# Gregor-Mendel-Institute/SNPmatch

Hardware: NVIDIA B200
Metric: snp_accession_comparisons_per_sec (higher is better)
Workload: dtype f64

## Files before the change

snpmatch_b200/csrc/api.cu:

```cuda
#include "common.cuh"
#include <memory>
#include <new>
#include "pack.cuh"
#include "join.cuh"
#include "score.cuh"
#include "windows.cuh"
#include "f1.cuh"
#include "hardcall.cuh"
#include "gemm_onehot.cuh"
#include "grouped.cuh"
#include "group_sort.cuh"
#include "grouped2.cuh"
#include "pairs.cuh"
#include "cross_geno.cuh"
#include <unordered_map>

namespace snpm {
thread_local std::string g_last_error;

static int grid_for(int64_t items, int threads, int n_sm, int per_sm = 16) {
    int64_t g = ceil_div64(items, threads);
    const int64_t cap = int64_t(n_sm) * per_sm;
    if (g > cap) g = cap;
    if (g < 1) g = 1;
// ... 559 lines not shown
        for (int64_t i = 0; i < n; ++i) gid[size_t(i)] = rank[size_t(gid[size_t(i)])];
    }
    std::vector<int64_t> cnt(static_cast<size_t>(T) + 1);
    for (int64_t s = 0; s < n_samples; ++s) {
        const int64_t b0 = offsets[s], b1 = offsets[s + 1];
        std::fill(cnt.begin(), cnt.end(), 0);
        for (int64_t i = b0; i < b1; ++i) ++cnt[size_t(gid[size_t(i)]) + 1];
        for (int32_t t = 0; t < T; ++t) cnt[size_t(t) + 1] += cnt[size_t(t)];
        for (int64_t i = b0; i < b1; ++i) {
            const int32_t g = gid[size_t(i)];
            const int64_t o = b0 + cnt[size_t(g)]++;
            out_chrom[o] = s_chrom_id[i] < 0 ? uint8_t(255) : uint8_t(s_chrom_id[i]);
            out_pos[o] = s_pos[i];
            out_gid[o] = uint16_t(g);
            if (out_order) out_order[o] = i;
        }
    }
    return SNPM_OK;
}

static int upload_grouped(snpm_batch *b, int64_t n_samples, const int64_t *offsets, const uint8_t *chrom_u8, const int32_t *s_pos,
                          const uint32_t *packed_cp, const uint16_t *gid, const double *table, int32_t n_table,
                          const uint16_t *run_gid = nullptr, const uint32_t *run_end = nullptr, int64_t n_runs = 0) {
    if (!b) return fail(SNPM_E_ARG, "snpm_batch_upload_grouped: NULL batch");
    snpm_db *db = b->db;
    if (n_samples < 1 || !offsets || offsets[0] != 0) return fail(SNPM_E_ARG, "snpm_batch_upload_grouped: need samples and offsets starting at 0");
    for (int64_t s = 0; s < n_samples; ++s)
        if (offsets[s + 1] < offsets[s]) return fail(SNPM_E_ARG, "snpm_batch_upload_grouped: offsets must be non-decreasing");
    const int64_t n = offsets[n_samples];
    if (n >= (int64_t(1) << 31) - 2048) return fail(SNPM_E_ARG, "snpm_batch_upload_grouped: %lld markers exceed the 2^31 limit", (long long)n);
    if (n > 0 && ((!gid && !run_gid) || (!packed_cp && (!chrom_u8 || !s_pos)))) return fail(SNPM_E_ARG, "snpm_batch_upload_grouped: NULL marker arrays");
    if (run_gid && n > 0) {
        if (!run_end || n_runs < 1 || n_runs > n) return fail(SNPM_E_ARG, "snpm_batch_upload_grouped_runs: need 1..n runs");
        if (int64_t(run_end[n_runs - 1]) != n || run_end[0] == 0) return fail(SNPM_E_ARG, "snpm_batch_upload_grouped_runs: the runs must cover markers 0..n");
    }
    if (!table || n_table < 1 || n_table > 65536) return fail(SNPM_E_ARG, "snpm_batch_upload_grouped: weight table must hold 1..65536 triples");
    std::vector<double> t4(size_t(n_table) * 4);
    for (int32_t t = 0; t < n_table; ++t) {
        const double w0 = table[3 * size_t(t)], w1 = table[3 * size_t(t) + 1], w2 = table[3 * size_t(t) + 2];
        if (!(w0 >= 0.0 && w1 >= 0.0 && w2 >= 0.0) || std::isinf(w0) || std::isinf(w1) || std::isinf(w2))
            return fail(SNPM_E_ARG, "snpm_batch_upload_grouped: weights must be finite and non-negative (triple %d)", t);
        t4[4 * size_t(t)] = w0;
        t4[4 * size_t(t) + 1] = w2;
        t4[4 * size_t(t) + 2] = w1;
        t4[4 * size_t(t) + 3] = 0.0;
    }
    SNPM_CUDA(cudaSetDevice(db->device));
    b->S = n_samples;
    b->n = n;
    b->grouped = true;
    b->coded = false;
    b->pending_expand = 0;
    b->n_gtable = n_table;
    b->gchunk = b->gchunk_req;
    b->h_off.assign(offsets, offsets + n_samples + 1);
    int64_t nseg = 0;
    for (int64_t s = 0; s < n_samples; ++s) nseg += ceil_div64(offsets[s + 1] - offsets[s], b->gchunk);
    b->nseg_cap = nseg;
    SNPM_TRY(b->d_off.ensure(size_t(n_samples + 1) * 8));
    SNPM_TRY(b->d_chrom8.ensure(size_t(n)));
    SNPM_TRY(b->d_chrom.ensure(size_t(n) * 4));
    SNPM_TRY(b->d_pos.ensure(size_t(n) * 4));
    SNPM_TRY(b->d_gid.ensure(size_t(n) * 2));
    SNPM_TRY(b->d_gtable.ensure(size_t(n_table) * 32));
    cudaStream_t st = b->copy_stream;
    SNPM_CUDA(cudaStreamWaitEvent(st, b->ev_inputs_free, 0));
    SNPM_CUDA(cudaMemcpyAsync(b->d_off.p, offsets, size_t(n_samples + 1) * 8, cudaMemcpyHostToDevice, st));
    b->h_gtable.assign(t4.begin(), t4.end());
    SNPM_CUDA(cudaMemcpyAsync(b->d_gtable.p, b->h_gtable.data(), size_t(n_table) * 32, cudaMemcpyHostToDevice, st));
    if (n) {
        if (run_gid) {
            const size_t bad_off = (size_t(n_runs) * 6 + 15) & ~size_t(15);
            SNPM_TRY(b->d_runs.ensure(bad_off + 16));
            uint32_t *d_end = b->d_runs.as<uint32_t>();
            uint16_t *d_rg = reinterpret_cast<uint16_t *>(d_end + n_runs);
            b->d_runs_bad = reinterpret_cast<int *>(static_cast<char *>(b->d_runs.p) + bad_off);
            SNPM_CUDA(cudaMemsetAsync(b->d_runs_bad, 0, sizeof(int), st));
            SNPM_CUDA(cudaMemcpyAsync(d_end, run_end, size_t(n_runs) * 4, cudaMemcpyHostToDevice, st));
            SNPM_CUDA(cudaMemcpyAsync(d_rg, run_gid, size_t(n_runs) * 2, cudaMemcpyHostToDevice, st));
            b->pending_expand |= 1;
            b->pending_runs = n_runs;
        } else {
            b->d_runs_bad = nullptr;
            SNPM_CUDA(cudaMemcpyAsync(b->d_gid.p, gid, size_t(n) * 2, cudaMemcpyHostToDevice, st));
        }
        if (packed_cp) {
            SNPM_TRY(b->d_wei_idx.ensure(size_t(n) * 4));
            SNPM_CUDA(cudaMemcpyAsync(b->d_wei_idx.p, packed_cp, size_t(n) * 4, cudaMemcpyHostToDevice, st));
            b->pending_expand |= 2;
        } else {
            SNPM_CUDA(cudaMemcpyAsync(b->d_chrom8.p, chrom_u8, size_t(n), cudaMemcpyHostToDevice, st));
            SNPM_CUDA(cudaMemcpyAsync(b->d_pos.p, s_pos, size_t(n) * 4, cudaMemcpyHostToDevice, st));
            b->pending_expand |= 4;
        }
    }
    SNPM_CUDA(cudaEventRecord(b->ev_uploaded, st));
    b->ran = b->ran_windows = b->epilogue_done = false;
    return SNPM_OK;
}

int snpm_batch_upload_grouped(snpm_batch *b, int64_t n_samples, const int64_t *offsets, const uint8_t *chrom_u8, const int32_t *s_pos,
                              const uint16_t *gid, const double *table, int32_t n_table) {
    return upload_grouped(b, n_samples, offsets, chrom_u8, s_pos, nullptr, gid, table, n_table);
}

int snpm_batch_upload_grouped_packed(snpm_batch *b, int64_t n_samples, const int64_t *offsets, const uint32_t *chrom_pos, const uint16_t *gid,
                                     const double *table, int32_t n_table) {
    return upload_grouped(b, n_samples, offsets, nullptr, nullptr, chrom_pos, gid, table, n_table);
}

int snpm_batch_upload_grouped_runs(snpm_batch *b, int64_t n_samples, const int64_t *offsets, const uint32_t *chrom_pos, const uint16_t *run_gid,
                                   const uint32_t *run_end, int64_t n_runs, const double *table, int32_t n_table) {
    return upload_grouped(b, n_samples, offsets, nullptr, nullptr, chrom_pos, nullptr, table, n_table, run_gid, run_end, n_runs);
}

static int upload_coded(snpm_batch *b, int64_t n_samples, const int64_t *offsets, const uint32_t *chrom_pos, const uint16_t *codes,
                        const uint32_t *codes32, const double *wtable, int32_t n_wtable) {
    if (!b) return fail(SNPM_E_ARG, "snpm_batch_upload_coded: NULL batch");
    if (codes32 && n_wtable > 1024) return fail(SNPM_E_ARG, "snpm_batch_upload_coded32: three codes share one word only up to 1024 weight values (%d given)", n_wtable);
    snpm_db *db = b->db;
    if (n_samples < 1 || !offsets || offsets[0] != 0) return fail(SNPM_E_ARG, "snpm_batch_upload_coded: need samples and offsets starting at 0");
    for (int64_t s = 0; s < n_samples; ++s)
        if (offsets[s + 1] < offsets[s]) return fail(SNPM_E_ARG, "snpm_batch_upload_coded: offsets must be non-decreasing");
    const int64_t n = offsets[n_samples];
    if (n >= (int64_t(1) << 31) - 2048) return fail(SNPM_E_ARG, "snpm_batch_upload_coded: %lld markers exceed the 2^31 limit", (long long)n);
    if (n > 0 && (!chrom_pos || (!codes && !codes32))) return fail(SNPM_E_ARG, "snpm_batch_upload_coded: NULL marker arrays");
    if (!wtable || n_wtable < 1 || n_wtable > 65536) return fail(SNPM_E_ARG, "snpm_batch_upload_coded: the weight table must hold 1..65536 values");
    for (int32_t t = 0; t < n_wtable; ++t)
        if (!(wtable[t] >= 0.0) || std::isinf(wtable[t])) return fail(SNPM_E_ARG, "snpm_batch_upload_coded: weights must be finite and non-negative (entry %d)", t);
    if (!b->gchunk_set) b->gchunk_req = db->stride > G2_WX ? G2_MAX_CHUNK : 320;
    if (b->gchunk_req % GR_BLOCK || b->gchunk_req > G2_MAX_CHUNK)
        return fail(SNPM_E_ARG, "snpm_batch_upload_coded: the group chunk must be a multiple of %d and at most %d rows (it is %d)", GR_BLOCK, G2_MAX_CHUNK, b->gchunk_req);
    SNPM_CUDA(cudaSetDevice(db->device));
    b->S = n_samples;
    b->n = n;
    b->grouped = true;
    b->coded = true;
    b->codes_packed = codes32 != nullptr;
    b->pending_expand = 2;
    b->d_runs_bad = nullptr;
    b->n_wtable = n_wtable;
    int bits = 1;
    while ((1 << bits) < n_wtable) ++bits;
    b->code_bits = bits;
    b->key_bits = 3 * bits + 2;
    b->gchunk = b->gchunk_req;
    b->h_off.assign(offsets, offsets + n_samples + 1);
    int64_t nseg = 0;
    std::vector<int32_t> tile_first(size_t(n_samples) + 1), tile_sample;
    for (int64_t s = 0; s < n_samples; ++s) {
        const int64_t ns = offsets[s + 1] - offsets[s];
        nseg += ceil_div64(ns, b->gchunk);
        tile_first[size_t(s)] = int32_t(tile_sample.size());
        for (int64_t t = 0; t < ceil_div64(ns, RS_TILE); ++t) tile_sample.push_back(int32_t(s));
    }
    tile_first[size_t(n_samples)] = int32_t(tile_sample.size());
    b->nseg_cap = nseg;
    b->n_sort_tiles = int64_t(tile_sample.size());
    const size_t key_bytes = b->key_bits <= 32 ? 4 : 8;
    SNPM_TRY(b->d_off.ensure(size_t(n_samples + 1) * 8));
    SNPM_TRY(b->d_chrom.ensure(size_t(n) * 4));
    SNPM_TRY(b->d_pos.ensure(size_t(n) * 4));
    SNPM_TRY(b->d_wei_idx.ensure(size_t(n) * 4));
    SNPM_TRY(b->d_codes.ensure(size_t(n) * 6));
    SNPM_TRY(b->d_wtable.ensure(size_t(n_wtable) * 8));
    SNPM_TRY(b->d_key_a.ensure(size_t(n) * key_bytes));
    SNPM_TRY(b->d_pair_db_tmp.ensure(size_t(n) * 4));
    SNPM_TRY(b->d_pair_s_tmp.ensure(size_t(n) * 4));
    SNPM_TRY(b->d_tile_sample.ensure(std::max<size_t>(tile_sample.size(), 1) * 4));
    SNPM_TRY(b->d_tile_first.ensure(size_t(n_samples + 1) * 4));
    SNPM_TRY(b->d_tile_hist.ensure(std::max<size_t>(tile_sample.size(), 1) * (size_t(GH_MAX_GROUPS) * 4 + 8)));
    SNPM_TRY(b->d_blk_chg.ensure(size_t(std::max<int64_t>(nseg, 1)) * (size_t(b->gchunk / GR_BLOCK) * 8 + 12) + size_t(SO_BUCKETS) * 4 + 16));
    SNPM_TRY(b->d_seg_order.ensure(size_t(std::max<int64_t>(nseg, 1)) * 16));
    SNPM_TRY(b->d_work_counter.ensure(256));
    SNPM_TRY(b->d_hash.ensure(size_t(n_samples) * GH_SLOTS * 8));
    SNPM_TRY(b->d_slot_gid.ensure(size_t(n_samples) * GH_SLOTS * 2));
    SNPM_TRY(b->d_ngroups.ensure(size_t(n_samples) * 4));
    SNPM_TRY(b->d_group_overflow.ensure(size_t(n_samples) * 4));
    SNPM_TRY(b->d_gkeys.ensure(size_t(n_samples) * GH_MAX_GROUPS * key_bytes));
    SNPM_TRY(b->d_gw.ensure(size_t(n_samples) * GH_MAX_GROUPS * 32));
    SNPM_TRY(b->d_goff.ensure(size_t(n_samples) * (GH_MAX_GROUPS + 1) * 4));
    SNPM_TRY(b->d_gid.ensure(size_t(n) * 2));
    cudaStream_t st = b->copy_stream;
    SNPM_CUDA(cudaStreamWaitEvent(st, b->ev_inputs_free, 0));
    b->h_gtable.assign(wtable, wtable + n_wtable);
    b->h_tiles.assign(tile_first.begin(), tile_first.end());
    b->h_tiles.insert(b->h_tiles.end(), tile_sample.begin(), tile_sample.end());
    SNPM_CUDA(cudaMemcpyAsync(b->d_off.p, offsets, size_t(n_samples + 1) * 8, cudaMemcpyHostToDevice, st));
    SNPM_CUDA(cudaMemcpyAsync(b->d_wtable.p, b->h_gtable.data(), size_t(n_wtable) * 8, cudaMemcpyHostToDevice, st));
    SNPM_CUDA(cudaMemcpyAsync(b->d_tile_first.p, b->h_tiles.data(), size_t(n_samples + 1) * 4, cudaMemcpyHostToDevice, st));
    if (!tile_sample.empty())
        SNPM_CUDA(cudaMemcpyAsync(b->d_tile_sample.p, b->h_tiles.data() + n_samples + 1, tile_sample.size() * 4, cudaMemcpyHostToDevice, st));
    if (n) {
        SNPM_CUDA(cudaMemcpyAsync(b->d_wei_idx.p, chrom_pos, size_t(n) * 4, cudaMemcpyHostToDevice, st));
        if (codes32) SNPM_CUDA(cudaMemcpyAsync(b->d_codes.p, codes32, size_t(n) * 4, cudaMemcpyHostToDevice, st));
        else SNPM_CUDA(cudaMemcpyAsync(b->d_codes.p, codes, size_t(n) * 6, cudaMemcpyHostToDevice, st));
    }
    SNPM_CUDA(cudaEventRecord(b->ev_uploaded, st));
    b->ran = b->ran_windows = b->epilogue_done = false;
    return SNPM_OK;
}

int snpm_batch_upload_coded(snpm_batch *b, int64_t n_samples, const int64_t *offsets, const uint32_t *chrom_pos, const uint16_t *codes,
                            const double *wtable, int32_t n_wtable) {
    return upload_coded(b, n_samples, offsets, chrom_pos, codes, nullptr, wtable, n_wtable);
}

int snpm_batch_upload_coded32(snpm_batch *b, int64_t n_samples, const int64_t *offsets, const uint32_t *chrom_pos, const uint32_t *codes32,
                              const double *wtable, int32_t n_wtable) {
    return upload_coded(b, n_samples, offsets, chrom_pos, nullptr, codes32, wtable, n_wtable);
}

int snpm_batch_coded_timings(snpm_batch *b, float *ms, int n) {
    if (!b || !ms || n < 4) return fail(SNPM_E_ARG, "snpm_batch_coded_timings: need room for 4 floats");
    if (!b->coded || !b->ran) return fail(SNPM_E_STATE, "snpm_batch_coded_timings: run a coded batch first");
    SNPM_CUDA(cudaSetDevice(b->db->device));
    SNPM_CUDA(cudaStreamSynchronize(b->db->stream));
    for (int i = 0; i < n; ++i) ms[i] = 0.f;
    cudaEventElapsedTime(&ms[0], b->ev[SNPM_EV_START], b->ev_joined);
    cudaEventElapsedTime(&ms[1], b->ev_joined, b->ev[SNPM_EV_JOIN]);
    cudaEventElapsedTime(&ms[2], b->ev[SNPM_EV_JOIN], b->ev[SNPM_EV_SCORE]);
    cudaEventElapsedTime(&ms[3], b->ev[SNPM_EV_SCORE], b->ev[SNPM_EV_COMBINE]);
    return SNPM_OK;
}

int snpm_pack_markers(int64_t n, const uint8_t *chrom_u8, const int32_t *pos, uint32_t *out) {
    if (n < 0 || (n > 0 && (!chrom_u8 || !pos || !out))) return fail(SNPM_E_ARG, "snpm_pack_markers: bad arguments");
    for (int64_t i = 0; i < n; ++i) {
        const uint32_t c = chrom_u8[i] == 255 ? 31u : uint32_t(chrom_u8[i]);
        if ((chrom_u8[i] != 255 && c > 30u) || pos[i] < 0 || pos[i] >= (1 << 27))
            return fail(SNPM_E_RANGE, "snpm_pack_markers: marker %lld (chromosome id %u, position %d) does not fit 5 + 27 bits", (long long)i, c, pos[i]);
        out[i] = (c << 27) | uint32_t(pos[i]);
    }
    return SNPM_OK;
}

int snpm_pack_coded(int64_t n, const int32_t *chrom_id, const int32_t *pos, const uint16_t *codes, uint32_t *chrom_pos, uint32_t *codes32) {
    if (n < 0 || (n > 0 && (!chrom_id || !pos || !chrom_pos || (codes32 && !codes)))) return fail(SNPM_E_ARG, "snpm_pack_coded: bad arguments");
    uint32_t bad = 0u;
    for (int64_t i = 0; i < n; ++i) {
        const int32_t c = chrom_id[i], p = pos[i];
        bad |= uint32_t(c > 30) | uint32_t(p < 0) | uint32_t(p >= (1 << 27));
        chrom_pos[i] = ((c < 0 ? 31u : uint32_t(c)) << 27) | (uint32_t(p) & ((1u << 27) - 1u));
    }
    if (codes32)
        for (int64_t i = 0; i < n; ++i) {
            const uint32_t a = codes[3 * i], h = codes[3 * i + 1], t = codes[3 * i + 2];
            bad |= uint32_t((a | h | t) > 1023u);
            codes32[i] = a | (h << 10) | (t << 20);
        }
    if (bad) return fail(SNPM_E_RANGE, "snpm_pack_coded: a chromosome id above 30, a position outside 27 bits or a code above 1023");
    return SNPM_OK;
}

int snpm_batch_guard_counts(snpm_batch *b, int32_t *counts) {
    if (!b || !counts) return fail(SNPM_E_ARG, "snpm_batch_guard_counts: NULL argument");
    if (!b->grouped) { for (int64_t s = 0; s < b->rangen(); ++s) counts[s] = 0; return SNPM_OK; }
    if (!b->epilogue_done) return fail(SNPM_E_STATE, "snpm_batch_guard_counts: run the epilogue first");
    if (b->rangen() == 0) return SNPM_OK;
    SNPM_CUDA(cudaSetDevice(b->db->device));
    SNPM_CUDA(cudaMemcpyAsync(counts, b->d_guard.as<int32_t>() + b->range0(), size_t(b->rangen()) * 4, cudaMemcpyDeviceToHost, b->db->stream));
    SNPM_CUDA(cudaStreamSynchronize(b->db->stream));
    return SNPM_OK;
}

int snpm_batch_set_result_range(snpm_batch *b, int64_t first_sample, int64_t n_samples) {
    if (!b || first_sample < 0 || n_samples < -1) return fail(SNPM_E_ARG, "snpm_batch_set_result_range: bad range");
    b->res0 = first_sample;
    b->resn = n_samples;
    return SNPM_OK;
}

int snpm_batch_set_track_pairs(snpm_batch *b, int on) {
    if (!b) return fail(SNPM_E_ARG, "snpm_batch_set_track_pairs: NULL batch");
    b->track_pairs = on != 0;
    return SNPM_OK;
}

int snpm_batch_set_chunk_rows(snpm_batch *b, int32_t rows) {
    if (!b || rows < 1 || rows > 1000000) return fail(SNPM_E_ARG, "snpm_batch_set_chunk_rows: 1..1000000 rows");
    b->chunk_rows_req = rows;
    return SNPM_OK;
}

int snpm_batch_set_group_chunk(snpm_batch *b, int32_t rows) {
    if (!b || rows < 16 || rows > GR_MAX_CHUNK || rows % 8) return fail(SNPM_E_ARG, "snpm_batch_set_group_chunk: 16..%d rows, a multiple of 8", GR_MAX_CHUNK);
    b->gchunk_req = rows;
    b->gchunk_set = true;
    return SNPM_OK;
}

static void ipc_close_peers(snpm_batch *b);

int snpm_batch_destroy(snpm_batch *b) {
    if (!b) return SNPM_OK;
    cudaSetDevice(b->db->device);
    cudaStreamSynchronize(b->db->stream);
    if (b->copy_stream) { cudaStreamSynchronize(b->copy_stream); cudaStreamDestroy(b->copy_stream); }
    if (b->ev_uploaded) cudaEventDestroy(b->ev_uploaded);
    if (b->ev_inputs_free) cudaEventDestroy(b->ev_inputs_free);
    if (b->ev_joined) cudaEventDestroy(b->ev_joined);
    if (b->ev_fork) cudaEventDestroy(b->ev_fork);
    if (b->ev_join) cudaEventDestroy(b->ev_join);
    DevBuf *bufs[] = {&b->d_off, &b->d_chrom, &b->d_pos, &b->d_wei, &b->d_filter, &b->d_match_row, &b->d_tile_cnt, &b->d_tile_off,
                      &b->d_prefix, &b->d_pair_db, &b->d_pair_s, &b->d_pair_w, &b->d_mstart, &b->d_seg_off, &b->d_part_score,
                      &b->d_part_ninfo, &b->d_red, &b->d_matches, &b->d_ninfo64, &b->d_prob, &b->d_L, &b->d_LR, &b->d_status,
                      &b->d_win_count, &b->d_win_off, &b->d_win_begin, &b->d_win_end, &b->d_kmax, &b->d_win_L, &b->d_win_LR,
                      &b->d_win_ident, &b->d_win_amb, &b->d_win_row_off, &b->d_row_acc, &b->d_row_score, &b->d_row_ninfo, &b->d_row_L, &b->d_row_ident, &b->d_f1_acc, &b->d_f1_part, &b->d_f1_out, &b->d_pair_code, &b->d_wei_idx, &b->d_wei_table,
                      &b->d_chrom8, &b->d_gid, &b->d_gtable, &b->d_pair_gid, &b->d_part_int, &b->d_guard, &b->d_runs,
                      &b->d_codes, &b->d_wtable, &b->d_key_a, &b->d_key_b, &b->d_idx_a, &b->d_idx_b, &b->d_pair_db_tmp, &b->d_pair_s_tmp,
                      &b->d_tile_sample, &b->d_tile_first, &b->d_tile_hist, &b->d_blk_chg, &b->d_seg_order, &b->d_work_counter, &b->d_hash, &b->d_slot_gid, &b->d_ngroups,
                      &b->d_group_overflow, &b->d_gkeys, &b->d_gw, &b->d_goff, &b->d_segsel, &b->d_segsel_off, &b->d_flags, &b->d_flag_counts};
    for (DevBuf *d : bufs) d->release();
    for (int i = 0; i < SNPM_N_EVENTS; ++i)
        if (b->ev[i]) cudaEventDestroy(b->ev[i]);
    if (b->h_status) cudaFreeHost(b->h_status);
    if (b->h_tail) cudaFreeHost(b->h_tail);
    if (b->ev_fetched) cudaEventDestroy(b->ev_fetched);
    if (b->ev_results) cudaEventDestroy(b->ev_results);
    ipc_close_peers(b);
    delete b;
    return SNPM_OK;
}

int snpm_batch_set_row_filter(snpm_batch *b, const int64_t *sorted_rows, int64_t n) {
    if (!b || n < 0) return fail(SNPM_E_ARG, "snpm_batch_set_row_filter: bad arguments");
    for (int64_t i = 1; i < n; ++i)
        if (sorted_rows[i] <= sorted_rows[i - 1]) return fail(SNPM_E_ARG, "snpm_batch_set_row_filter: rows must be strictly ascending");
    SNPM_CUDA(cudaSetDevice(b->db->device));
    b->has_filter = sorted_rows != nullptr;
    b->n_filter = b->has_filter ? n : 0;
    SNPM_TRY(b->d_filter.ensure(size_t(std::max<int64_t>(n, 1)) * 8));
    if (b->has_filter && n) {
        SNPM_CUDA(cudaMemcpyAsync(b->d_filter.p, sorted_rows, size_t(n) * 8, cudaMemcpyHostToDevice, b->db->stream));
        SNPM_CUDA(cudaStreamSynchronize(b->db->stream));
    }
    return SNPM_OK;
}

int snpm_batch_set_segregation_filter(snpm_batch *b, const uint32_t *sel, int64_t S, int32_t words) {
    if (!b) return fail(SNPM_E_ARG, "snpm_batch_set_segregation_filter: NULL batch");
    if (!sel) {
        b->has_seg = false;
        b->seg_S = 0;
        return SNPM_OK;
    }
    snpm_db *db = b->db;
    if (S < 1 || words != db->stride)
        return fail(SNPM_E_ARG, "snpm_batch_set_segregation_filter: need S >= 1 selections of snpm_db_row_words() = %d words (got S = %lld, %d words)",
                    db->stride, (long long)S, words);
    std::vector<int32_t> off(size_t(S) + 1, 0);
    std::vector<uint32_t> pairs;
    for (int64_t s = 0; s < S; ++s) {
        for (int32_t w = 0; w < words; ++w) {
            const uint32_t m = sel[size_t(s) * words + w];
            const int64_t first = int64_t(w) * 32;
            const uint32_t valid = first >= db->n_acc ? 0u : (db->n_acc - first >= 32 ? 0xffffffffu : (1u << (db->n_acc - first)) - 1u);
            if (m & ~valid) return fail(SNPM_E_ARG, "snpm_batch_set_segregation_filter: sample %lld selects accessions beyond the panel's %d", (long long)s, db->n_acc);
            if (m) {
                pairs.push_back(uint32_t(w));
                pairs.push_back(m);
            }
        }
        if (pairs.size() / 2 > size_t(INT32_MAX)) return fail(SNPM_E_ARG, "snpm_batch_set_segregation_filter: selections too large");
        off[size_t(s) + 1] = int32_t(pairs.size() / 2);
    }
    SNPM_CUDA(cudaSetDevice(db->device));
    SNPM_TRY(b->d_segsel.ensure(std::max<size_t>(pairs.size(), 2) * 4));
    SNPM_TRY(b->d_segsel_off.ensure(off.size() * 4));
    if (!pairs.empty()) SNPM_CUDA(cudaMemcpyAsync(b->d_segsel.p, pairs.data(), pairs.size() * 4, cudaMemcpyHostToDevice, db->stream));
    SNPM_CUDA(cudaMemcpyAsync(b->d_segsel_off.p, off.data(), off.size() * 4, cudaMemcpyHostToDevice, db->stream));
    SNPM_CUDA(cudaStreamSynchronize(db->stream));
    b->has_seg = true;
    b->seg_S = S;
    return SNPM_OK;
}

int snpm_batch_count_flagged_pairs(snpm_batch *b, const uint8_t *flags, int64_t *counts) {
    if (!b || !counts || (b->n > 0 && !flags)) return fail(SNPM_E_ARG, "snpm_batch_count_flagged_pairs: bad arguments");
    if (!b->ran) return fail(SNPM_E_STATE, "snpm_batch_count_flagged_pairs: run the batch first");
    snpm_db *db = b->db;
    SNPM_CUDA(cudaSetDevice(db->device));
    cudaStream_t st = db->stream;
    SNPM_TRY(b->d_flag_counts.ensure(size_t(b->S) * 8));
    SNPM_CUDA(cudaMemsetAsync(b->d_flag_counts.p, 0, size_t(b->S) * 8, st));
    if (b->n > 0) {
        SNPM_TRY(b->d_flags.ensure(size_t(b->n)));
        SNPM_CUDA(cudaMemcpyAsync(b->d_flags.p, flags, size_t(b->n), cudaMemcpyHostToDevice, st));
        k_count_flagged_pairs<<<int(ceil_div64(b->n, 256)), 256, 0, st>>>(b->d_match_row.as<int32_t>(), b->d_flags.as<uint8_t>(), b->n,
                                                                          b->d_off.as<int64_t>(), b->S, b->d_flag_counts.as<unsigned long long>());
        SNPM_KERNEL_CHECK();
    }
    SNPM_CUDA(cudaMemcpyAsync(counts, b->d_flag_counts.p, size_t(b->S) * 8, cudaMemcpyDeviceToHost, st));
    SNPM_CUDA(cudaStreamSynchronize(st));
    return SNPM_OK;
}

static int batch_join(snpm_batch *b, int algo) {
    snpm_db *db = b->db;
    cudaStream_t st = db->stream;
    const int64_t n = b->n, S = b->S;
    const int64_t n_tiles = ceil_div64(n, JOIN_TILE);
    SNPM_TRY(b->d_match_row.ensure(size_t(n) * 4));
    SNPM_TRY(b->d_tile_cnt.ensure(size_t(n_tiles) * 4));
    SNPM_TRY(b->d_tile_off.ensure(size_t(n_tiles) * 4));
    SNPM_TRY(b->d_prefix.ensure(size_t(n + 1) * 4));
    SNPM_TRY(b->d_pair_db.ensure(size_t(n) * 4));
    SNPM_TRY(b->d_pair_s.ensure(size_t(n) * 4));
    if (b->coded) {  }
    else if (b->grouped) SNPM_TRY(b->d_pair_gid.ensure(size_t(n) * 2 + 16));
    else SNPM_TRY(b->d_pair_w.ensure(size_t(n) * 32));
    SNPM_TRY(b->d_mstart.ensure(size_t(S + 1) * 4));
    SNPM_TRY(b->d_seg_off.ensure(size_t(S + 1) * 4));
    SNPM_TRY(b->d_status.ensure(8 * sizeof(int)));
    SNPM_CUDA(cudaStreamWaitEvent(st, b->ev_uploaded, 0));
    SNPM_CUDA(cudaMemsetAsync(b->d_status.p, 0, 8 * sizeof(int), st));
    if (b->grouped && b->pending_expand && n > 0) {
        if (b->pending_expand & 1) {
            const uint32_t *d_end = b->d_runs.as<uint32_t>();
            k_expand_runs<<<int(ceil_div64(b->pending_runs * 32, 256)), 256, 0, st>>>(d_end, reinterpret_cast<const uint16_t *>(d_end + b->pending_runs),
                                                                                 int32_t(b->pending_runs), n, b->d_gid.as<uint16_t>(), b->d_runs_bad);
        }
        if (b->pending_expand & 4) k_expand_chrom<<<int(ceil_div64(n, 256)), 256, 0, st>>>(b->d_chrom8.as<uint8_t>(), n, b->d_chrom.as<int32_t>());
        SNPM_KERNEL_CHECK();
        b->pending_expand &= 2;
    }
    if (b->grouped && b->d_runs_bad) SNPM_CUDA(cudaMemcpyAsync(b->d_status.as<int>() + 4, b->d_runs_bad, sizeof(int), cudaMemcpyDeviceToDevice, st));
    if (!b->peer_red.empty() && b->ipc_step > 0 && b->d_red.p == b->ipc_ptr) {
        k_wait_peers_done<<<1, 32, 0, st>>>(reinterpret_cast<const uint32_t *>(static_cast<const char *>(b->d_red.p) + b->ipc_flags_off),
                                            int32_t(b->peer_red.size()), b->ipc_step, b->d_status.as<int>());
        SNPM_KERNEL_CHECK();
    }
    if (algo == 0) algo = (n / S) * 8 >= db->n_rows ? 2 : 1;
    if (b->grouped) algo = 1;
    const int64_t *filter = b->has_filter ? b->d_filter.as<int64_t>() : nullptr;
    if (n_tiles > 0) {
        if (algo == 2)
            k_join_mergepath<<<int(n_tiles), 256, 0, st>>>(b->d_chrom.as<int32_t>(), b->d_pos.as<int32_t>(), n, b->d_off.as<int64_t>(), S,
                                                         db->d_pos, db->d_chr_regions, db->n_chr, filter, b->n_filter, db->row0_global,
                                                         b->d_match_row.as<int32_t>(), b->d_tile_cnt.as<int32_t>(), b->d_status.as<int>());
        else
            k_join_search<<<int(n_tiles), JOIN_TILE, 0, st>>>(b->d_chrom.as<int32_t>(), b->d_pos.as<int32_t>(), n, b->d_off.as<int64_t>(), S,
                                                            db->d_pos, db->d_chr_regions, db->n_chr, db->d_bucket, db->d_bucket_off, db->bucket_shift,
                                                            filter, b->n_filter, db->row0_global,
                                                            b->d_match_row.as<int32_t>(), b->d_tile_cnt.as<int32_t>(), b->d_status.as<int>(), (b->grouped && !b->coded) ? 0 : 1,
                                                            db->d_bitmap, db->d_bm_first_row, db->d_bm_off,
                                                            (b->grouped && (b->pending_expand & 2)) ? b->d_wei_idx.as<uint32_t>() : nullptr);
        SNPM_KERNEL_CHECK();
        if (b->has_seg) {
            static_assert(SEGP_THREADS == JOIN_TILE, "the segregation filter recounts the join's tiles");
            k_segregating_pairs<<<int(n_tiles), SEGP_THREADS, 0, st>>>(db->d_packed, db->stride, b->d_off.as<int64_t>(), S, n, b->d_segsel.as<uint2>(),
                                                                      b->d_segsel_off.as<int32_t>(), b->d_match_row.as<int32_t>(), b->d_tile_cnt.as<int32_t>());
            SNPM_KERNEL_CHECK();
            b->launches += 1;
        }
        k_scan_tiles<<<1, 1024, 0, st>>>(b->d_tile_cnt.as<int32_t>(), n_tiles, b->d_tile_off.as<int32_t>(), b->d_prefix.as<int32_t>() + n);
        SNPM_KERNEL_CHECK();
        if (b->coded) {
            unsigned long long *hash = b->d_hash.as<unsigned long long>();
            SNPM_CUDA(cudaMemsetAsync(b->d_group_overflow.p, 0, size_t(S) * 4, st));
            SNPM_CUDA(cudaMemsetAsync(hash, 0, size_t(S) * GH_SLOTS * 8, st));
            if (b->key_bits <= 32)
                k_scatter_pairs_coded<uint32_t><<<int(n_tiles), SC_THREADS, 0, st>>>(b->d_match_row.as<int32_t>(), n, b->d_tile_off.as<int32_t>(), b->d_codes.as<uint16_t>(),
                        b->d_wtable.as<double>(), b->n_wtable, b->code_bits, b->d_prefix.as<int32_t>(), b->d_pair_db_tmp.as<int32_t>(), b->d_pair_s_tmp.as<int32_t>(),
                        b->d_key_a.as<uint32_t>(), b->d_status.as<int>(), b->d_off.as<int64_t>(), S, hash, b->d_group_overflow.as<int>(),
                        b->codes_packed ? b->d_codes.as<uint32_t>() : nullptr);
            else
                k_scatter_pairs_coded<uint64_t><<<int(n_tiles), SC_THREADS, 0, st>>>(b->d_match_row.as<int32_t>(), n, b->d_tile_off.as<int32_t>(), b->d_codes.as<uint16_t>(),
                        b->d_wtable.as<double>(), b->n_wtable, b->code_bits, b->d_prefix.as<int32_t>(), b->d_pair_db_tmp.as<int32_t>(), b->d_pair_s_tmp.as<int32_t>(),
                        b->d_key_a.as<uint64_t>(), b->d_status.as<int>(), b->d_off.as<int64_t>(), S, hash, b->d_group_overflow.as<int>(),
                        b->codes_packed ? b->d_codes.as<uint32_t>() : nullptr);
        } else if (b->grouped)
            k_scatter_pairs_grouped<<<int(n_tiles), JOIN_TILE, 0, st>>>(b->d_match_row.as<int32_t>(), n, b->d_tile_off.as<int32_t>(),
                                                                      b->d_gid.as<uint16_t>(), b->n_gtable, b->d_prefix.as<int32_t>(), b->d_pair_db.as<int32_t>(),
                                                                      b->d_pair_s.as<int32_t>(), b->d_pair_gid.as<uint16_t>(), b->d_status.as<int>());
        else
            k_scatter_pairs<<<int(n_tiles), JOIN_TILE, 0, st>>>(b->d_match_row.as<int32_t>(), n, b->d_tile_off.as<int32_t>(), b->d_wei.as<double>(),
                                                              b->d_prefix.as<int32_t>(), b->d_pair_db.as<int32_t>(), b->d_pair_s.as<int32_t>(),
                                                              b->d_pair_w.as<double>());
        SNPM_KERNEL_CHECK();
        b->launches += 3;
    } else {
        SNPM_CUDA(cudaMemsetAsync(b->d_prefix.p, 0, 4, st));
    }
    k_sample_ranges<<<1, 1024, 0, st>>>(b->d_prefix.as<int32_t>(), b->d_off.as<int64_t>(), S, b->grouped ? b->gchunk : b->chunk_rows, b->d_mstart.as<int32_t>(),
                                        b->d_seg_off.as<int32_t>());
    SNPM_KERNEL_CHECK();
    b->launches += 1;
    return SNPM_OK;
}

}

template <typename KeyT>
static int batch_group_sort_t(snpm_batch *b) {
    snpm_db *db = b->db;
    cudaStream_t st = db->stream;
    const int tiles = int(b->n_sort_tiles);
    if (tiles == 0 || b->n == 0) return SNPM_OK;
    const int32_t *mstart = b->d_mstart.as<int32_t>(), *tsample = b->d_tile_sample.as<int32_t>(), *tfirst = b->d_tile_first.as<int32_t>();
    uint32_t *hist = b->d_tile_hist.as<uint32_t>();
    int2 *range = reinterpret_cast<int2 *>(hist + (size_t(tiles) << 11));
    static bool gattr = false;
    if (!gattr) {
        SNPM_CUDA(cudaFuncSetAttribute(k_group_place, cudaFuncAttributeMaxDynamicSharedMemorySize, 64 * 1024));
        gattr = true;
    }
    KeyT *gkeys = b->d_gkeys.as<KeyT>();
    k_group_rank<KeyT><<<int(b->S), 1024, 0, st>>>(b->d_hash.as<unsigned long long>(), b->d_wtable.as<double>(), b->code_bits, b->d_slot_gid.as<uint16_t>(),
                                                   b->d_ngroups.as<int32_t>(), gkeys, b->d_gw.as<double4>(), b->d_group_overflow.as<int>());
    int64_t n_max = 0, jcap1 = 1;
    for (int64_t s = 0; s < b->S; ++s) {
        n_max = std::max(n_max, b->h_off[size_t(s) + 1] - b->h_off[size_t(s)]);
        jcap1 = std::max(jcap1, ceil_div64(b->h_off[size_t(s) + 1] - b->h_off[size_t(s)], b->gchunk));
    }
    const char *force = getenv("SNPM_GROUP_KERNEL");
    const bool fits = n_max <= GP_MAX_PAIRS;
    const bool want = force ? !strcmp(force, "sample") : (n_max <= 32768 || b->S >= 128);
    if (fits && want) {
        static bool sattr = false;
        if (!sattr) {
            SNPM_CUDA(cudaFuncSetAttribute(k_group_sample<uint32_t>, cudaFuncAttributeMaxDynamicSharedMemorySize, int(GP_SMEM)));
            SNPM_CUDA(cudaFuncSetAttribute(k_group_sample<uint64_t>, cudaFuncAttributeMaxDynamicSharedMemorySize, int(GP_SMEM)));
            sattr = true;
        }
        const size_t ncap = size_t(std::max<int64_t>(b->nseg_cap, 1));
        int32_t *cost = reinterpret_cast<int32_t *>(b->d_blk_chg.as<unsigned long long>() + ncap * size_t(b->gchunk / GR_BLOCK));
        int32_t *buckets = cost + ncap;
        const size_t zbytes = ncap * (size_t(b->gchunk / GR_BLOCK) * 8 + 4) + size_t(SO_BUCKETS) * 4;
        int2 *br = reinterpret_cast<int2 *>(reinterpret_cast<unsigned char *>(b->d_blk_chg.p) + ((zbytes + 7) & ~size_t(7)));
        SNPM_CUDA(cudaMemsetAsync(b->d_blk_chg.p, 0, zbytes, st));
        k_group_sample<KeyT><<<int(b->S), 32 * GP_WARPS, GP_SMEM, st>>>(
            b->d_key_a.as<KeyT>(), b->d_hash.as<unsigned long long>(), b->d_slot_gid.as<uint16_t>(), b->d_ngroups.as<int32_t>(), b->d_gid.as<uint16_t>(),
            b->d_pair_db_tmp.as<int32_t>(), b->d_pair_s_tmp.as<int32_t>(), b->d_pair_db.as<int32_t>(), b->track_pairs ? b->d_pair_s.as<int32_t>() : nullptr,
            b->d_goff.as<int32_t>(), gkeys, mstart, b->d_seg_off.as<int32_t>(), b->gchunk, b->code_bits, b->d_blk_chg.as<unsigned long long>(), cost,
            int32_t(jcap1), buckets, br, b->d_work_counter.as<unsigned int>());
        k_order_place<<<int(b->S), 256, 0, st>>>(buckets, br, b->d_seg_off.as<int32_t>(), mstart, b->gchunk, b->d_seg_order.as<int4>());
        SNPM_KERNEL_CHECK();
        b->launches += 3;
        return SNPM_OK;
    }
    k_tile_ranges<<<(tiles + 255) / 256, 256, 0, st>>>(mstart, tsample, tfirst, tiles, range);
    k_group_ids<KeyT><<<tiles, RS_THREADS, 0, st>>>(b->d_key_a.as<KeyT>(), range, tsample, b->d_hash.as<unsigned long long>(), b->d_slot_gid.as<uint16_t>(),
                                                    b->d_ngroups.as<int32_t>(), b->d_gid.as<uint16_t>(), hist);
    k_group_scan<<<int(b->S), 1024, 0, st>>>(hist, tfirst, b->d_ngroups.as<int32_t>(), b->d_goff.as<int32_t>());
    const size_t nseg_cap = size_t(std::max<int64_t>(b->nseg_cap, 1));
    int32_t *seg_cost = reinterpret_cast<int32_t *>(b->d_blk_chg.as<unsigned long long>() + nseg_cap * size_t(b->gchunk / GR_BLOCK));
    int32_t *bucket_cnt = seg_cost + nseg_cap;
    const size_t zero_bytes = nseg_cap * (size_t(b->gchunk / GR_BLOCK) * 8 + 4) + size_t(SO_BUCKETS) * 4;
    int2 *seg_br = reinterpret_cast<int2 *>(reinterpret_cast<unsigned char *>(b->d_blk_chg.p) + ((zero_bytes + 7) & ~size_t(7)));
    int64_t jcap = 1;
    for (int64_t s = 0; s < b->S; ++s) jcap = std::max(jcap, ceil_div64(b->h_off[size_t(s) + 1] - b->h_off[size_t(s)], b->gchunk));
    cudaStream_t aux = b->copy_stream;
    if (!b->ev_fork) SNPM_CUDA(cudaEventCreateWithFlags(&b->ev_fork, cudaEventDisableTiming));
    if (!b->ev_join) SNPM_CUDA(cudaEventCreateWithFlags(&b->ev_join, cudaEventDisableTiming));
    SNPM_CUDA(cudaEventRecord(b->ev_fork, st));
    SNPM_CUDA(cudaStreamWaitEvent(aux, b->ev_fork, 0));
    SNPM_CUDA(cudaMemsetAsync(b->d_blk_chg.p, 0, zero_bytes, aux));
    k_group_marks<KeyT><<<int(b->S), 1024, 0, aux>>>(b->d_goff.as<int32_t>(), gkeys, b->d_ngroups.as<int32_t>(), mstart, b->d_seg_off.as<int32_t>(), b->gchunk,
                                                     b->code_bits, b->d_blk_chg.as<unsigned long long>(), seg_cost, int32_t(jcap), bucket_cnt, seg_br);
    k_order_place<<<int(b->S), 256, 0, aux>>>(bucket_cnt, seg_br, b->d_seg_off.as<int32_t>(), mstart, b->gchunk, b->d_seg_order.as<int4>());
    SNPM_CUDA(cudaEventRecord(b->ev_join, aux));
    k_group_place<<<tiles, RS_THREADS, size_t(GH_MAX_GROUPS) * 20, st>>>(b->d_gid.as<uint16_t>(), b->d_pair_db_tmp.as<int32_t>(), b->d_pair_s_tmp.as<int32_t>(),
                                                                        b->d_pair_db.as<int32_t>(), b->track_pairs ? b->d_pair_s.as<int32_t>() : nullptr, mstart, tsample,
                                                                        tfirst, range, hist, b->d_ngroups.as<int32_t>(), b->d_goff.as<int32_t>(), b->d_work_counter.as<unsigned int>());
    SNPM_CUDA(cudaStreamWaitEvent(st, b->ev_join, 0));
    SNPM_KERNEL_CHECK();
    b->launches += 7;
    return SNPM_OK;
}

static int launch_grouped2(snpm_batch *b, bool skip_db_hets) {
    snpm_db *db = b->db;
    cudaStream_t st = db->stream;
    Group2Args g = {};
    g.packed = db->d_packed; g.stride = db->stride; g.pair_db = b->d_pair_db.as<int32_t>();
    g.blk_chg = b->d_blk_chg.as<unsigned long long>(); g.gw = b->d_gw.as<double>();
    g.seg_off = b->d_seg_off.as<int32_t>(); g.mstart = b->d_mstart.as<int32_t>(); g.S = int32_t(b->S); g.chunk = b->gchunk;
    g.part_score = b->d_part_score.as<double>(); g.part_int = b->d_part_int.as<int32_t>(); g.a_pad = db->stride * 32;
    if (db->stride <= G2_WX) { g.n_slices = 1; g.wx = (db->stride + 1) & ~1; }
    else { g.wx = 32; g.n_slices = (db->stride + 31) / 32; }
    g.teams = std::min(G2_THREADS / g.wx, G2_MAX_TEAMS);
    g.order = b->d_seg_order.as<int4>();
    g.work_counter = b->d_work_counter.as<unsigned int>();
    const int64_t n_items = std::max<int64_t>(b->nseg_cap, 1) * g.n_slices;
    if (n_items >= (int64_t(1) << 31) - (int64_t(1) << 20)) return fail(SNPM_E_ARG, "snpm_batch_run: %lld work items exceed the 2^31 limit", (long long)n_items);
    constexpr int ring = 64;
    const size_t smem = size_t(g.teams) * g2_team_smem(g.wx, g.chunk, ring);
    if (smem > 226 * 1024) return fail(SNPM_E_ARG, "snpm_batch_run: group chunk %d needs %zu bytes of shared memory", g.chunk, smem);
    const int grid = int(std::min<int64_t>(db->n_sm, ceil_div64(n_items, g.teams)));
#define G2_LAUNCH(SK, WXV)                                                                                                        \
    do {                                                                                                                          \
        static bool attr_ = false;                                                                                                \
        if (!attr_) {                                                                                                             \
            SNPM_CUDA(cudaFuncSetAttribute(k_score_grouped2<SK, WXV, ring>, cudaFuncAttributeMaxDynamicSharedMemorySize, 226 * 1024)); \
            attr_ = true;                                                                                                         \
        }                                                                                                                         \
        k_score_grouped2<SK, WXV, ring><<<grid, G2_THREADS, smem, st>>>(g);                                                       \
    } while (0)
    if (g.wx == G2_WX) {
        if (skip_db_hets) G2_LAUNCH(true, G2_WX); else G2_LAUNCH(false, G2_WX);
    } else if (g.wx == 32) {
        if (skip_db_hets) G2_LAUNCH(true, 32); else G2_LAUNCH(false, 32);
    } else {
        if (skip_db_hets) G2_LAUNCH(true, 0); else G2_LAUNCH(false, 0);
    }
#undef G2_LAUNCH
    SNPM_KERNEL_CHECK();
    b->launches += 1;
    return SNPM_OK;
}

extern "C" {

static int batch_alloc_outputs(snpm_batch *b, int64_t nseg) {
    snpm_db *db = b->db;
    const int64_t a_pad = int64_t(db->stride) * 32;
    const int64_t SA = b->S * int64_t(db->n_acc);
    SNPM_TRY(b->d_part_score.ensure(size_t(std::max<int64_t>(nseg, 1)) * a_pad * 8));
    SNPM_TRY(b->d_part_ninfo.ensure(size_t(std::max<int64_t>(nseg, 1)) * a_pad * 4));
    SNPM_TRY(b->d_red.ensure(size_t(b->S) * size_t(b->red_pitch()) * 8));
    if (b->grouped) SNPM_TRY(b->d_part_int.ensure(size_t(std::max<int64_t>(nseg, 1)) * a_pad * 4));
    SNPM_TRY(b->d_matches.ensure(size_t(SA) * 8));
    SNPM_TRY(b->d_ninfo64.ensure(size_t(SA) * 8));
    SNPM_TRY(b->d_prob.ensure(size_t(SA) * 8));
    SNPM_TRY(b->d_L.ensure(size_t(SA) * 8));
    SNPM_TRY(b->d_LR.ensure(size_t(SA) * 8));
    return SNPM_OK;
}

static void rec(snpm_batch *b, int which) {
    cudaEventRecord(b->ev[which], b->db->stream);
    b->ev_rec[which] = true;
}

int snpm_batch_run(snpm_batch *b, int skip_db_hets, int mode) {
    if (!b) return fail(SNPM_E_ARG, "snpm_batch_run: NULL batch");
    snpm_db *db = b->db;
    SNPM_CUDA(cudaSetDevice(db->device));
    cudaStream_t st = db->stream;
    const int kernel_mode = mode & 0xff, algo = (mode >> 8) & 0xff;
    if (kernel_mode < 0 || kernel_mode > 2) return fail(SNPM_E_ARG, "snpm_batch_run: unknown kernel mode %d", kernel_mode);
    if ((kernel_mode == 2) != b->grouped)
        return fail(SNPM_E_STATE, "snpm_batch_run: kernel mode 2 scores batches uploaded with snpm_batch_upload_grouped, and only those");
    if (algo > 2) return fail(SNPM_E_ARG, "snpm_batch_run: unknown join algorithm %d", algo);
    if (b->has_seg && kernel_mode == 2)
        return fail(SNPM_E_STATE, "snpm_batch_run: the segregation filter is honoured by kernel modes 0 and 1 only; clear it first");
    if (b->has_seg && b->seg_S != b->S)
        return fail(SNPM_E_ARG, "snpm_batch_run: the segregation filter holds %lld selections for %lld samples", (long long)b->seg_S, (long long)b->S);
    b->launches = 0;
    for (int i = 0; i < SNPM_N_EVENTS; ++i) b->ev_rec[i] = false;
    SNPM_TRY(batch_alloc_outputs(b, b->nseg_cap));
    rec(b, SNPM_EV_START);
    SNPM_TRY(batch_join(b, algo));
    rec(b, SNPM_EV_JOIN);
    ScoreArgs a = {};
    a.packed = db->d_packed;
    a.stride = db->stride;
    a.pair_db = b->d_pair_db.as<int32_t>();
    a.pair_w = b->d_pair_w.as<double>();
    a.seg_off = b->d_seg_off.as<int32_t>();
    a.mstart = b->d_mstart.as<int32_t>();
    a.S = int32_t(b->S);
    a.chunk = b->chunk_rows;
    a.table = 0;
    a.part_score = b->d_part_score.as<double>();
    a.part_ninfo = b->d_part_ninfo.as<int32_t>();
    a.a_pad = db->stride * 32;
    if (kernel_mode == 2 && b->coded) {
        cudaEventRecord(b->ev_joined, st);
        if (b->key_bits <= 32) SNPM_TRY(batch_group_sort_t<uint32_t>(b)); else SNPM_TRY(batch_group_sort_t<uint64_t>(b));
        rec(b, SNPM_EV_JOIN);
        if (b->nseg_cap > 0 && b->n > 0) {
            SNPM_TRY(launch_grouped2(b, skip_db_hets != 0));
        }
        rec(b, SNPM_EV_SCORE);
        dim3 cgrid((a.a_pad + 31) / 32, unsigned(b->S));
        k_combine_grouped<<<cgrid, 32 * CG_PARTS, 0, st>>>(a.part_score, b->d_part_int.as<int32_t>(), a.a_pad, db->stride, db->n_acc, a.seg_off, a.mstart,
                                                 b->d_red.as<double>());
        SNPM_KERNEL_CHECK();
        b->launches += 1;
        rec(b, SNPM_EV_COMBINE);
        SNPM_CUDA(cudaEventRecord(b->ev_inputs_free, st));
        b->ran = true;
        b->ran_windows = false;
        b->epilogue_done = false;
        return SNPM_OK;
    }
    if (kernel_mode == 2) {
        if (b->nseg_cap > 0) {
            GroupArgs g = {};
            g.packed = db->d_packed; g.stride = db->stride; g.pair_db = a.pair_db; g.pair_gid = b->d_pair_gid.as<uint16_t>();
            g.table = b->d_gtable.as<double>(); g.seg_off = a.seg_off; g.mstart = a.mstart; g.S = a.S; g.chunk = b->gchunk;
            g.part_score = a.part_score; g.part_int = b->d_part_int.as<int32_t>(); g.a_pad = a.a_pad;
            const int nsl = (db->stride + GR_MAX_WX - 1) / GR_MAX_WX;
            g.wx = ((db->stride + nsl - 1) / nsl + 1) & ~1;
            g.spc = std::min(GR_THREADS / g.wx, GR_MAX_TEAMS);
            const size_t gsmem = size_t(g.spc) * grouped_team_smem(g.wx, g.chunk);
            static bool gr_attr = false;
            if (!gr_attr) {
                SNPM_CUDA(cudaFuncSetAttribute(k_score_grouped<true, 0>, cudaFuncAttributeMaxDynamicSharedMemorySize, 220 * 1024));
                SNPM_CUDA(cudaFuncSetAttribute(k_score_grouped<false, 0>, cudaFuncAttributeMaxDynamicSharedMemorySize, 220 * 1024));
                SNPM_CUDA(cudaFuncSetAttribute(k_score_grouped<true, GR_MAX_WX>, cudaFuncAttributeMaxDynamicSharedMemorySize, 220 * 1024));
                SNPM_CUDA(cudaFuncSetAttribute(k_score_grouped<false, GR_MAX_WX>, cudaFuncAttributeMaxDynamicSharedMemorySize, 220 * 1024));
                gr_attr = true;
            }
            int64_t jmax = 0;
            for (int64_t smp = 0; smp < b->S; ++smp)
                jmax = std::max(jmax, ceil_div64(b->h_off[size_t(smp) + 1] - b->h_off[size_t(smp)], b->gchunk));
            g.jmax = int32_t(jmax);
            dim3 ggrid(unsigned(ceil_div64(b->S * jmax, g.spc)), unsigned((db->stride + g.wx - 1) / g.wx));
            if (g.wx == GR_MAX_WX) {
                if (skip_db_hets) k_score_grouped<true, GR_MAX_WX><<<ggrid, GR_THREADS, gsmem, st>>>(g);
                else k_score_grouped<false, GR_MAX_WX><<<ggrid, GR_THREADS, gsmem, st>>>(g);
            } else {
                if (skip_db_hets) k_score_grouped<true, 0><<<ggrid, GR_THREADS, gsmem, st>>>(g);
                else k_score_grouped<false, 0><<<ggrid, GR_THREADS, gsmem, st>>>(g);
            }
            SNPM_KERNEL_CHECK();
            b->launches += 1;
        }
        rec(b, SNPM_EV_SCORE);
        dim3 cgrid((a.a_pad + 31) / 32, unsigned(b->S));
        k_combine_grouped<<<cgrid, 32 * CG_PARTS, 0, st>>>(a.part_score, b->d_part_int.as<int32_t>(), a.a_pad, db->stride, db->n_acc, a.seg_off, a.mstart,
                                                 b->d_red.as<double>());
        SNPM_KERNEL_CHECK();
        b->launches += 1;
        rec(b, SNPM_EV_COMBINE);
        SNPM_CUDA(cudaEventRecord(b->ev_inputs_free, st));
        b->ran = true;
        b->ran_windows = false;
        b->epilogue_done = false;
        return SNPM_OK;
    }
    if (kernel_mode == 1 && b->chunk_rows != SNPM_CHUNK_ROWS)
        return fail(SNPM_E_STATE, "snpm_batch_run: the popcount kernel works in %d-row chunks (its sums are exact in any chunking); set the chunk back", SNPM_CHUNK_ROWS);
    if (kernel_mode == 1 && b->nseg_cap > 0) {
        SNPM_TRY(b->d_pair_code.ensure(size_t(std::max<int64_t>(b->n, 1))));
        k_pair_codes<<<int(ceil_div64(b->n, 256)), 256, 0, st>>>(a.pair_w, b->d_prefix.as<int32_t>() + b->n, b->d_pair_code.as<uint8_t>());
        SNPM_KERNEL_CHECK();
        HardArgs h = {};
        h.packed = a.packed; h.stride = a.stride; h.pair_db = a.pair_db; h.pair_code = b->d_pair_code.as<uint8_t>();
        h.seg_off = a.seg_off; h.mstart = a.mstart; h.S = a.S; h.chunk = a.chunk;
        h.part_score = a.part_score; h.part_ninfo = a.part_ninfo; h.a_pad = a.a_pad; h.status = b->d_status.as<int>();
        const int wx = std::min<int>(db->stride, HC_THREADS), spc = std::min(HC_THREADS / wx, HC_MAX_SEGS);
        h.wx = wx;
        h.spc = spc;
        dim3 hgrid(unsigned(ceil_div64(b->nseg_cap, spc)), unsigned((db->stride + wx - 1) / wx));
        const size_t hsmem = size_t(spc) * SNPM_CHUNK_ROWS * 5;
        static bool hc_attr = false;
        if (!hc_attr) {
            SNPM_CUDA(cudaFuncSetAttribute(k_score_hard<true>, cudaFuncAttributeMaxDynamicSharedMemorySize, 64 * 1024));
            SNPM_CUDA(cudaFuncSetAttribute(k_score_hard<false>, cudaFuncAttributeMaxDynamicSharedMemorySize, 64 * 1024));
            hc_attr = true;
        }
        if (skip_db_hets) k_score_hard<true><<<hgrid, HC_THREADS, hsmem, st>>>(h);
        else k_score_hard<false><<<hgrid, HC_THREADS, hsmem, st>>>(h);
        SNPM_KERNEL_CHECK();
        b->launches += 2;
    } else {
        SNPM_TRY(launch_score(st, a, int(b->nseg_cap), skip_db_hets != 0));
        if (b->nseg_cap > 0) b->launches += 1;
    }
    rec(b, SNPM_EV_SCORE);
    dim3 cgrid((db->n_acc + 31) / 32, unsigned(b->S));
    k_combine<<<cgrid, 32, 0, st>>>(a.part_score, a.part_ninfo, a.a_pad, db->n_acc, a.seg_off, a.mstart, 0, nullptr, nullptr, b->d_red.as<double>());
    SNPM_KERNEL_CHECK();
    b->launches += 1;
    rec(b, SNPM_EV_COMBINE);
    SNPM_CUDA(cudaEventRecord(b->ev_inputs_free, st));
    b->ran = true;
    b->ran_windows = false;
    b->epilogue_done = false;
    return SNPM_OK;
}

int snpm_batch_epilogue(snpm_batch *b) {
    if (!b) return fail(SNPM_E_ARG, "snpm_batch_epilogue: NULL batch");
    if (!b->ran) return fail(SNPM_E_STATE, "snpm_batch_epilogue: run the batch first");
    snpm_db *db = b->db;
    SNPM_CUDA(cudaSetDevice(db->device));
    const int64_t r0 = b->range0(), rn = b->rangen();
    if (r0 < 0 || rn < 0 || r0 + rn > b->S) return fail(SNPM_E_ARG, "snpm_batch_epilogue: result range [%lld, %lld) outside the %lld samples", (long long)r0, (long long)(r0 + rn), (long long)b->S);
    rec(b, SNPM_EV_EPI_START);
    const int64_t pitch = b->red_pitch(), A = db->n_acc;
    if (rn > 0) {
        if (b->grouped) {
            SNPM_TRY(b->d_guard.ensure(size_t(b->S) * 4));
            SNPM_CUDA(cudaMemsetAsync(b->d_guard.as<int32_t>() + r0, 0, size_t(rn) * 4, db->stream));
            dim3 fgrid((db->n_acc + 255) / 256, unsigned(rn));
            k_grouped_finalize<<<fgrid, 256, 0, db->stream>>>(b->d_red.as<double>() + r0 * pitch, db->n_acc, b->d_guard.as<int32_t>() + r0,
                                                              b->coded ? b->d_group_overflow.as<int>() + r0 : nullptr);
            SNPM_KERNEL_CHECK();
            b->launches += 1;
        }
        SNPM_CUDA(launch_epilogue(db->stream, rn, b->d_red.as<double>() + r0 * pitch, pitch, db->n_acc, 1, 0, 0.0,
                                  b->d_matches.as<int64_t>() + r0 * A, b->d_ninfo64.as<int64_t>() + r0 * A,
                                  b->d_prob.as<double>() + r0 * A, b->d_L.as<double>() + r0 * A, b->d_LR.as<double>() + r0 * A));
    }
    SNPM_KERNEL_CHECK();
    b->launches += 1;
    rec(b, SNPM_EV_EPI_END);
    b->epilogue_done = true;
    return SNPM_OK;
}

int snpm_batch_wait(snpm_batch *b, float *ms_device) {
    if (!b) return fail(SNPM_E_ARG, "snpm_batch_wait: NULL batch");
    snpm_db *db = b->db;
    SNPM_CUDA(cudaSetDevice(db->device));
    if (b->d_status.p) SNPM_CUDA(cudaMemcpyAsync(b->h_status, b->d_status.p, 8 * sizeof(int), cudaMemcpyDeviceToHost, db->stream));
    else memset(b->h_status, 0, 8 * sizeof(int));
    SNPM_CUDA(cudaStreamSynchronize(db->stream));
    if (ms_device) {
        *ms_device = 0.f;
        if (b->ev_rec[SNPM_EV_START] && b->ev_rec[SNPM_EV_COMBINE]) {
            float t = 0.f;
            cudaEventElapsedTime(&t, b->ev[SNPM_EV_START], b->ev[SNPM_EV_COMBINE]);
            *ms_device += t;
        }
        if (b->ev_rec[SNPM_EV_EPI_START] && b->ev_rec[SNPM_EV_EPI_END]) {
            float t = 0.f;
            cudaEventElapsedTime(&t, b->ev[SNPM_EV_EPI_START], b->ev[SNPM_EV_EPI_END]);
            *ms_device += t;
        }
    }
    if (b->h_status[0] > 0)
        return fail(SNPM_E_ARG, "sample markers are not sorted by (database chromosome order, position) or repeat a position (%d places)", b->h_status[0]);
    if (b->h_status[1] > 0)
        return fail(SNPM_E_ASSERT, "provided y is greater than n (%d window cells; likeliTest, snpmatch.py:43)", b->h_status[1]);
    if (b->h_status[2] > 0)
        return fail(SNPM_E_ARG, "identity table too short for %d window cells", b->h_status[2]);
    if (b->h_status[3] > 0)
        return fail(SNPM_E_ARG, "kernel mode 1 needs one-hot weights (called genotypes); %d matched markers are not", b->h_status[3]);
    if (b->h_status[4] > 0)
        return fail(SNPM_E_ARG, "%d matched markers carry a weight-triple id outside the table (or run-length coded ids do not ascend)", b->h_status[4]);
    if (b->h_status[5] > 0)
        return fail(SNPM_E_STATE, "peer reduce: a rank did not arrive within thirty seconds (every rank must run and reduce the same batches in the same order)");
    return SNPM_OK;
}

int snpm_batch_timings(snpm_batch *b, float *ms, int n) {
    if (!b || !ms || n < 6) return fail(SNPM_E_ARG, "snpm_batch_timings: need room for 6 floats");
    SNPM_CUDA(cudaSetDevice(b->db->device));
    SNPM_CUDA(cudaStreamSynchronize(b->db->stream));
    for (int i = 0; i < n; ++i) ms[i] = 0.f;
    auto el = [&](int a, int c) {
        float t = 0.f;
        if (b->ev_rec[a] && b->ev_rec[c]) cudaEventElapsedTime(&t, b->ev[a], b->ev[c]);
        return t;
    };
    ms[0] = el(SNPM_EV_START, SNPM_EV_JOIN);
    ms[1] = el(SNPM_EV_JOIN, SNPM_EV_SCORE);
    ms[2] = el(SNPM_EV_SCORE, SNPM_EV_COMBINE);
    ms[3] = el(SNPM_EV_EPI_START, SNPM_EV_EPI_END);
    ms[4] = el(SNPM_EV_START, SNPM_EV_COMBINE) + ms[3];
    ms[5] = float(b->launches);
    if (n >= 8) {
        ms[6] = el(SNPM_EV_RED_START, SNPM_EV_RED_END);
        int wait_ns = 0;
        if (b->ev_rec[SNPM_EV_RED_END] && b->d_status.p) cudaMemcpy(&wait_ns, b->d_status.as<int>() + 7, sizeof(int), cudaMemcpyDeviceToHost);
        ms[7] = float(wait_ns) * 1e-6f;
    }
    return SNPM_OK;
}

int snpm_batch_reduce_buffer(snpm_batch *b, void **dev_ptr, int64_t *n_doubles) {
    if (!b || !dev_ptr) return fail(SNPM_E_ARG, "snpm_batch_reduce_buffer: NULL argument");
    SNPM_CUDA(cudaSetDevice(b->db->device));
    SNPM_TRY(b->d_red.ensure(size_t(b->S) * size_t(b->red_pitch()) * 8));
    *dev_ptr = b->d_red.p;
    if (n_doubles) *n_doubles = b->S * b->red_pitch();
    return SNPM_OK;
}

static void ipc_close_peers(snpm_batch *b) {
    for (size_t r = 0; r < b->peer_red.size(); ++r)
        if (int32_t(r) != b->ipc_rank && b->peer_red[r]) cudaIpcCloseMemHandle(b->peer_red[r]);
    b->peer_red.clear();
    b->ipc_rank = -1;
}

int snpm_batch_ipc_export(snpm_batch *b, void *handle64, int64_t *n_doubles) {
    static_assert(sizeof(cudaIpcMemHandle_t) == 64, "CUDA IPC handles are 64 bytes");
    if (!b || !handle64) return fail(SNPM_E_ARG, "snpm_batch_ipc_export: NULL argument");
    SNPM_CUDA(cudaSetDevice(b->db->device));
    const size_t bytes = size_t(b->S) * size_t(b->red_pitch()) * 8;
    const size_t cap = std::max<size_t>(((bytes + 255) & ~size_t(255)) + PR_FLAG_BYTES, size_t(4) << 20);
    SNPM_CUDA(cudaStreamSynchronize(b->db->stream));
    if (b->d_red.cap != cap) {
        b->d_red.release();
        SNPM_TRY(b->d_red.ensure(cap));
    }
    b->ipc_flags_off = cap - PR_FLAG_BYTES;
    b->ipc_step = 0;
    SNPM_CUDA(cudaMemset(static_cast<char *>(b->d_red.p) + b->ipc_flags_off, 0, PR_FLAG_BYTES));
    SNPM_CUDA(cudaIpcGetMemHandle(reinterpret_cast<cudaIpcMemHandle_t *>(handle64), b->d_red.p));
    b->ipc_ptr = b->d_red.p;
    if (n_doubles) *n_doubles = b->S * b->red_pitch();
    return SNPM_OK;
}

int snpm_batch_ipc_open(snpm_batch *b, const void *handles, int32_t world, int32_t rank) {
    if (!b || !handles || world < 1 || world > PR_MAX_WORLD || rank < 0 || rank >= world) return fail(SNPM_E_ARG, "snpm_batch_ipc_open: bad arguments (at most %d ranks)", PR_MAX_WORLD);
    if (!b->ipc_ptr || b->ipc_ptr != b->d_red.p) return fail(SNPM_E_STATE, "snpm_batch_ipc_open: export this batch's buffer first (snpm_batch_ipc_export)");
    SNPM_CUDA(cudaSetDevice(b->db->device));
    ipc_close_peers(b);
    b->peer_red.assign(size_t(world), nullptr);
    b->ipc_rank = rank;
    const cudaIpcMemHandle_t *h = reinterpret_cast<const cudaIpcMemHandle_t *>(handles);
    for (int32_t r = 0; r < world; ++r) {
        if (r == rank) { b->peer_red[size_t(r)] = b->d_red.p; continue; }
        cudaError_t e = cudaIpcOpenMemHandle(&b->peer_red[size_t(r)], h[r], cudaIpcMemLazyEnablePeerAccess);
        if (e != cudaSuccess) {
            b->peer_red[size_t(r)] = nullptr;
            ipc_close_peers(b);
            return fail(SNPM_E_CUDA, "snpm_batch_ipc_open: rank %d's buffer: %s", r, cudaGetErrorString(e));
        }
    }
    return SNPM_OK;
}

int snpm_batch_ipc_close(snpm_batch *b) {
    if (!b) return SNPM_OK;
    cudaSetDevice(b->db->device);
    cudaStreamSynchronize(b->db->stream);
    ipc_close_peers(b);
    b->ipc_ptr = nullptr;
    return SNPM_OK;
}

int snpm_batch_reduce_peers(snpm_batch *b) {
    if (!b) return fail(SNPM_E_ARG, "snpm_batch_reduce_peers: NULL batch");
    if (!b->ran) return fail(SNPM_E_STATE, "snpm_batch_reduce_peers: run the batch first");
    const int32_t world = int32_t(b->peer_red.size());
    if (world < 1 || b->ipc_rank < 0) return fail(SNPM_E_STATE, "snpm_batch_reduce_peers: open the peers' buffers first (snpm_batch_ipc_open)");
    if (b->d_red.p != b->ipc_ptr) return fail(SNPM_E_STATE, "snpm_batch_reduce_peers: the reduce buffer moved since it was exported (batch grew): export and open again");
    const int64_t r0 = b->res0, rn = b->resn < 0 ? b->S - b->res0 : b->resn;
    if (r0 + rn > b->S) return fail(SNPM_E_ARG, "snpm_batch_reduce_peers: result range outside the batch");
    const int64_t pitch = b->red_pitch();
    int64_t first = r0 * pitch, count = rn * pitch;
    SNPM_CUDA(cudaSetDevice(b->db->device));
    PeerPtrs pp;
    for (int32_t r = 0; r < PR_MAX_WORLD; ++r) {
        pp.p[r] = r < world ? static_cast<const double *>(b->peer_red[size_t(r)]) : nullptr;
        pp.flags[r] = r < world ? reinterpret_cast<uint32_t *>(static_cast<char *>(b->peer_red[size_t(r)]) + b->ipc_flags_off) : nullptr;
    }
    b->ipc_step += 1;
    rec(b, SNPM_EV_RED_START);
    const bool vec = ((first | count) & 1) == 0;
    const int grid = int(std::max<int64_t>(1, std::min<int64_t>(ceil_div64(vec ? count / 2 : count, 256), int64_t(b->db->n_sm) * 4)));
    if (vec) k_reduce_peers<double2><<<grid, 256, 0, b->db->stream>>>(pp, world, b->ipc_rank, b->ipc_step, first, count, b->d_red.as<double>(), b->d_status.as<int>());
    else k_reduce_peers<double><<<grid, 256, 0, b->db->stream>>>(pp, world, b->ipc_rank, b->ipc_step, first, count, b->d_red.as<double>(), b->d_status.as<int>());
    rec(b, SNPM_EV_RED_END);
    SNPM_KERNEL_CHECK();
    b->launches += 1;
    return SNPM_OK;
}

int snpm_batch_fetch(snpm_batch *b, double *score, int64_t *matches, int64_t *ninfo, int64_t *m, double *prob, double *L, double *LR) {
    if (!b) return fail(SNPM_E_ARG, "snpm_batch_fetch: NULL batch");
    if (!b->ran) return fail(SNPM_E_STATE, "snpm_batch_fetch: run the batch first");
    if ((matches || ninfo || prob || L || LR) && !b->epilogue_done) return fail(SNPM_E_STATE, "snpm_batch_fetch: run the epilogue first");
    snpm_db *db = b->db;
    SNPM_CUDA(cudaSetDevice(db->device));
    cudaStream_t st = db->stream;
    const size_t A = size_t(db->n_acc), S = size_t(b->rangen()), R0 = size_t(b->range0()), pitch = size_t(b->red_pitch()) * 8;
    if (R0 + S > size_t(b->S)) return fail(SNPM_E_ARG, "snpm_batch_fetch: result range outside the batch");
    if (b->grouped && score && !b->epilogue_done) return fail(SNPM_E_STATE, "snpm_batch_fetch: grouped batches finalise their scores in the epilogue; run it first");
    const double *red = b->d_red.as<double>() + R0 * size_t(b->red_pitch());
    std::vector<double> tail(2 * S + 2);
    if (S > 0) {
        if (score) SNPM_CUDA(cudaMemcpy2DAsync(score, A * 8, red, pitch, A * 8, S, cudaMemcpyDeviceToHost, st));
        SNPM_CUDA(cudaMemcpy2DAsync(tail.data(), 16, red + 2 * A, pitch, 16, S, cudaMemcpyDeviceToHost, st));
        if (matches) SNPM_CUDA(cudaMemcpyAsync(matches, b->d_matches.as<int64_t>() + R0 * A, S * A * 8, cudaMemcpyDeviceToHost, st));
        if (ninfo) SNPM_CUDA(cudaMemcpyAsync(ninfo, b->d_ninfo64.as<int64_t>() + R0 * A, S * A * 8, cudaMemcpyDeviceToHost, st));
        if (prob) SNPM_CUDA(cudaMemcpyAsync(prob, b->d_prob.as<double>() + R0 * A, S * A * 8, cudaMemcpyDeviceToHost, st));
        if (L) SNPM_CUDA(cudaMemcpyAsync(L, b->d_L.as<double>() + R0 * A, S * A * 8, cudaMemcpyDeviceToHost, st));
        if (LR) SNPM_CUDA(cudaMemcpyAsync(LR, b->d_LR.as<double>() + R0 * A, S * A * 8, cudaMemcpyDeviceToHost, st));
    }
    SNPM_TRY(snpm_batch_wait(b, nullptr));
    long long viol = 0;
// ... 766 lines not shown
```

snpmatch_b200/csrc/common.cuh:

```cuda
#pragma once
#include <cuda_runtime.h>
#include <stdint.h>
#include <stdarg.h>
#include <stdio.h>
#include <stdlib.h>
#include <string.h>
#include <string>
#include <vector>
#include <algorithm>
#include <cmath>

#include "../../include/snpmatch_b200.h"

namespace snpm {

extern thread_local std::string g_last_error;

inline int fail(int code, const char *fmt, ...) __attribute__((format(printf, 2, 3)));
inline int fail(int code, const char *fmt, ...) {
    char buf[512];
    va_list ap;
    va_start(ap, fmt);
    vsnprintf(buf, sizeof(buf), fmt, ap);
    va_end(ap);
    g_last_error = buf;
    return code;
}

#define SNPM_CUDA(call)                                                                          \
    do {                                                                                         \
        cudaError_t e__ = (call);                                                                \
        if (e__ != cudaSuccess)                                                                  \
            return snpm::fail(SNPM_E_CUDA, "%s:%d %s -> %s", __FILE__, __LINE__, #call,          \
                              cudaGetErrorString(e__));                                          \
    } while (0)

#define SNPM_TRY(call)                 \
    do {                               \
        int rc__ = (call);             \
        if (rc__ != SNPM_OK) return rc__; \
    } while (0)

static inline bool snpm_sync_debug() {
    static int v = -1;
    if (v < 0) v = getenv("SNPM_SYNC_DEBUG") ? 1 : 0;
    return v == 1;
}
#define SNPM_KERNEL_CHECK()                                              \
    do {                                                                 \
        SNPM_CUDA(cudaGetLastError());                                   \
        if (snpm_sync_debug()) SNPM_CUDA(cudaDeviceSynchronize());       \
    } while (0)

struct DevBuf {
    void *p = nullptr;
    size_t cap = 0;
    int ensure(size_t bytes) {
        if (bytes <= cap && p) return SNPM_OK;
        if (p) { cudaFree(p); p = nullptr; cap = 0; }
        size_t want = bytes < 256 ? 256 : bytes;
        cudaError_t e = cudaMalloc(&p, want);
        if (e != cudaSuccess) {
            p = nullptr;
            return fail(SNPM_E_NOMEM, "cudaMalloc(%zu bytes) failed: %s", want, cudaGetErrorString(e));
        }
        cap = want;
        return SNPM_OK;
    }
    void release() {
        if (p) cudaFree(p);
        p = nullptr;
        cap = 0;
    }
    template <typename T> T *as() const { return reinterpret_cast<T *>(p); }
};

static inline int64_t ceil_div64(int64_t a, int64_t b) { return (a + b - 1) / b; }

}

struct snpm_db {
    int device = 0;
    int64_t n_rows = 0;
    int32_t n_acc = 0;
    int32_t n_words = 0;
    int32_t stride = 0;
    int64_t row0_global = 0;
    int32_t n_chr = 0;
    int n_sm = 148;
    uint64_t *d_packed = nullptr;
    int32_t *d_pos = nullptr;
    int64_t *d_chr_regions = nullptr;
    int32_t *d_bucket = nullptr;
    int32_t *d_bucket_off = nullptr;
    int bucket_shift = 0;
    unsigned long long *d_bitmap = nullptr;
    int32_t *d_bm_first_row = nullptr;
    int64_t *d_bm_off = nullptr;
    std::vector<int64_t> h_chr_regions;
    cudaStream_t stream = nullptr;
    bool own_stream = false;
    snpm::DevBuf scratch;
    struct snpm_batch *scratch_batch_ = nullptr;
};

enum { SNPM_EV_START = 0, SNPM_EV_JOIN, SNPM_EV_SCORE, SNPM_EV_COMBINE, SNPM_EV_EPI_START, SNPM_EV_EPI_END, SNPM_EV_RED_START, SNPM_EV_RED_END, SNPM_N_EVENTS };

struct snpm_batch {
    snpm_db *db = nullptr;
    int64_t S = 0;
    int64_t n = 0;
    int64_t nseg_cap = 0;
    std::vector<int64_t> h_off;
    snpm::DevBuf d_off, d_chrom, d_pos, d_wei, d_filter;
    int64_t n_filter = 0;
    bool has_filter = false;
    snpm::DevBuf d_segsel, d_segsel_off;
    int64_t seg_S = 0;
    bool has_seg = false;
    snpm::DevBuf d_flags, d_flag_counts;
    snpm::DevBuf d_match_row, d_tile_cnt, d_tile_off, d_prefix, d_pair_db, d_pair_s, d_pair_w;
    snpm::DevBuf d_mstart, d_seg_off;
    snpm::DevBuf d_part_score, d_part_ninfo, d_red, d_matches, d_ninfo64, d_prob, d_L, d_LR, d_status;
    int32_t n_windows = 0;
    int64_t bin_len = 0;
    double lr_thres = 3.841;
    snpm::DevBuf d_win_count, d_win_off, d_win_begin, d_win_end, d_kmax, d_win_L, d_win_LR, d_win_ident, d_win_amb;
    snpm::DevBuf d_win_nrows, d_win_zero, d_win_red;
    int64_t kmax_len = 0;
    bool win_pending = false;
    bool win_reduced = false;
    snpm::DevBuf d_win_row_off, d_row_acc, d_row_score, d_row_ninfo, d_row_L, d_row_ident;
    snpm::DevBuf d_f1_acc, d_f1_part, d_f1_out;
    snpm::DevBuf d_pair_code;
    snpm::DevBuf d_wei_idx, d_wei_table;
    bool grouped = false;
    int32_t n_gtable = 0;
    int32_t chunk_rows = SNPM_CHUNK_ROWS, chunk_rows_req = SNPM_CHUNK_ROWS;
    int32_t gchunk = 320;
    int32_t gchunk_req = 320;
    bool gchunk_set = false;
    bool coded = false;
    bool codes_packed = false;
    int32_t n_wtable = 0, code_bits = 0, key_bits = 0;
    int64_t n_sort_tiles = 0;
    snpm::DevBuf d_codes, d_wtable, d_key_a, d_key_b, d_idx_a, d_idx_b, d_pair_db_tmp, d_pair_s_tmp, d_tile_sample, d_tile_first,
                 d_tile_hist, d_blk_chg, d_seg_order, d_work_counter, d_hash, d_slot_gid, d_ngroups, d_group_overflow, d_gkeys, d_gw, d_goff;
    bool track_pairs = true;
    cudaEvent_t ev_fork = nullptr, ev_join = nullptr;
    cudaEvent_t ev_joined = nullptr;
    snpm::DevBuf d_chrom8, d_gid, d_gtable, d_pair_gid, d_part_int, d_guard, d_runs;
    std::vector<double> h_gtable;
    std::vector<int32_t> h_tiles;
    int pending_expand = 0;
    int64_t pending_runs = 0;
    int *d_runs_bad = nullptr;
    int64_t red_pitch() const { return (grouped ? 3 : 2) * int64_t(db->n_acc) + 2; }
    bool ran = false, ran_windows = false, epilogue_done = false;
    int launches = 0;
    cudaStream_t copy_stream = nullptr;
    cudaEvent_t ev_uploaded = nullptr, ev_inputs_free = nullptr;
    cudaEvent_t ev[SNPM_N_EVENTS] = {};
    bool ev_rec[SNPM_N_EVENTS] = {};
    int *h_status = nullptr;
    cudaEvent_t ev_fetched = nullptr, ev_results = nullptr;
    double *h_tail = nullptr;
    int64_t h_tail_cap = 0;
    int64_t *pend_m = nullptr;
    bool fetch_pending = false;
    int64_t res0 = 0, resn = -1;
    void *ipc_ptr = nullptr;
    std::vector<void *> peer_red;
    int32_t ipc_rank = -1;
    size_t ipc_flags_off = 0;
    uint32_t ipc_step = 0;
    int64_t range0() const { return resn < 0 ? 0 : res0; }
    int64_t rangen() const { return resn < 0 ? S : resn; }
};
```

snpmatch_b200/csrc/group_sort.cuh:

```cuda
#pragma once
#include "common.cuh"
#include "join.cuh"

namespace snpm {

constexpr int RS_THREADS = 256;
constexpr int RS_PER_THREAD = 8;
constexpr int RS_TILE = RS_THREADS * RS_PER_THREAD;

__host__ __device__ __forceinline__ int gs_slow_class(int c) { return c == 2 ? 0 : 2; }
__host__ __device__ __forceinline__ int gs_fast_class(int c) { return c == 1 ? 0 : 1; }
__host__ __device__ __forceinline__ int gs_field_shift(int c, int which, int b) {
    return which == c ? 2 * b : (which == gs_slow_class(c) ? b : 0);
}
template <typename KeyT>
__host__ __device__ __forceinline__ uint32_t gs_code(KeyT key, int which, int b) {
    const int c = int(key >> (3 * b)) & 3;
    return uint32_t(key >> gs_field_shift(c, which, b)) & ((1u << b) - 1u);
}

constexpr int GH_SLOTS = 4096;
constexpr int GH_MAX_GROUPS = 2048;

__device__ __forceinline__ uint32_t gh_hash(unsigned long long key) { return uint32_t((key * 0x9E3779B97F4A7C15ull) >> 52); }
__device__ __forceinline__ void gh_insert(unsigned long long *__restrict__ table, unsigned long long key, int *overflow) {
    const unsigned long long want = key + 1ull;
    uint32_t h = gh_hash(key);
    for (int probe = 0; probe < GH_SLOTS; ++probe) {
        unsigned long long cur = __ldcg(table + h);
        if (cur == 0ull) cur = atomicCAS(table + h, 0ull, want);
        if (cur == 0ull || cur == want) return;
        h = (h + 1u) & uint32_t(GH_SLOTS - 1);
    }
    atomicExch(overflow, 1);
}
__device__ __forceinline__ uint32_t gh_find(const unsigned long long *__restrict__ table, unsigned long long key) {
    const unsigned long long want = key + 1ull;
    uint32_t h = gh_hash(key);
    for (int probe = 0; probe < GH_SLOTS; ++probe) {
        const unsigned long long cur = __ldg(table + h);
        if (cur == want || cur == 0ull) break;
        h = (h + 1u) & uint32_t(GH_SLOTS - 1);
    }
    return h;
}

constexpr int SC_THREADS = 256;
constexpr int SC_PER = JOIN_TILE / SC_THREADS;
constexpr int SC_SLOTS = 1024;
template <typename KeyT>
__global__ void __launch_bounds__(SC_THREADS) k_scatter_pairs_coded(
        const int32_t *__restrict__ match_row, int64_t n, const int32_t *__restrict__ tile_off, const uint16_t *__restrict__ codes,
        const double *__restrict__ wtable, int32_t n_table, int32_t code_bits, int32_t *__restrict__ prefix,
        int32_t *__restrict__ pair_db, int32_t *__restrict__ pair_s, KeyT *__restrict__ key, int *status,
        const int64_t *__restrict__ off, int64_t S, unsigned long long *__restrict__ hash, int *__restrict__ overflow,
        const uint32_t *__restrict__ codes32) {
    constexpr int NW = SC_THREADS / 32;
    __shared__ int s_cnt[SC_PER][NW];
    __shared__ int64_t s_first_sm, s_first_end;
    __shared__ unsigned long long s_seen[SC_SLOTS];
    const int lane = threadIdx.x & 31, warp = threadIdx.x >> 5;
    const int64_t i0 = int64_t(blockIdx.x) * JOIN_TILE;
    int32_t row[SC_PER];
    uint32_t cw[SC_PER];
#pragma unroll
    for (int j = 0; j < SC_PER; ++j) {
        const int64_t i = i0 + j * SC_THREADS + threadIdx.x;
        row[j] = i < n ? match_row[i] : -1;
    }
#pragma unroll
    for (int j = 0; j < SC_PER; ++j) {
        const int64_t i = i0 + j * SC_THREADS + threadIdx.x;
        cw[j] = (codes32 != nullptr && i < n) ? codes32[i] : 0u;
    }
    const int32_t base0 = tile_off[blockIdx.x];
#pragma unroll
    for (int j = 0; j < SC_SLOTS / SC_THREADS; ++j) s_seen[j * SC_THREADS + threadIdx.x] = 0ull;
    uint32_t bal[SC_PER];
#pragma unroll
    for (int j = 0; j < SC_PER; ++j) {
        bal[j] = __ballot_sync(0xffffffffu, row[j] >= 0);
        if (lane == 0) s_cnt[j][warp] = __popc(bal[j]);
    }
    if (threadIdx.x == 0) {
        int64_t lo = 0, hi = S;
        while (hi - lo > 1) {
            const int64_t mid = (lo + hi) >> 1;
            if (off[mid] <= i0) lo = mid; else hi = mid;
        }
        s_first_sm = lo;
        s_first_end = off[lo + 1];
    }
    __syncthreads();
    const int64_t s_first = s_first_sm, first_end = s_first_end;
    int32_t base = base0;
#pragma unroll
    for (int j = 0; j < SC_PER; ++j) {
        const int64_t i = i0 + j * SC_THREADS + threadIdx.x;
        int before = 0, total = 0;
#pragma unroll
        for (int w = 0; w < NW; ++w) {
            const int c = s_cnt[j][w];
            before += w < warp ? c : 0;
            total += c;
        }
        const int32_t p = base + before + __popc(bal[j] & ((1u << lane) - 1u));
        base += total;
        unsigned long long ins = ~0ull, fold = 0ull;
        bool solo = false;
        int64_t smp = 0;
        if (i < n) {
            prefix[i] = p;
            if (row[j] >= 0) {
                pair_db[p] = row[j];
                pair_s[p] = int32_t(i);
                uint32_t cd[3];
                if (codes32 != nullptr) {
                    const uint32_t v = cw[j];
                    cd[0] = v & 1023u; cd[2] = (v >> 10) & 1023u; cd[1] = (v >> 20) & 1023u;
                } else {
                    cd[0] = codes[3 * i]; cd[2] = codes[3 * i + 1]; cd[1] = codes[3 * i + 2];
                }
                bool bad = false;
#pragma unroll
                for (int k = 0; k < 3; ++k)
                    if (int32_t(cd[k]) >= n_table) { bad = true; cd[k] = 0; }
                if (bad) atomicAdd(status + 4, 1);
                const double w0 = __ldg(wtable + cd[0]), w1 = __ldg(wtable + cd[1]), w2 = __ldg(wtable + cd[2]);
                int c;
                if (w0 == 1.0) c = 0; else if (w1 == 1.0) c = 1; else if (w2 == 1.0) c = 2;
                else { c = 0; if (w1 > w0) c = 1; if (w2 > (c ? w1 : w0)) c = 2; }
                const int b = code_bits;
                const KeyT kk = (KeyT(c) << (3 * b)) | (KeyT(cd[c]) << (2 * b)) | (KeyT(cd[gs_slow_class(c)]) << b) | KeyT(cd[gs_fast_class(c)]);
                key[p] = kk;
                int64_t lo = s_first;
                if (i >= first_end) {
                    ++lo;
                    while (lo + 1 < S && off[lo + 1] <= i) ++lo;
                }
                smp = lo;
                ins = (unsigned long long)(kk);
                if (lo - s_first < 8192) fold = (unsigned long long)(lo - s_first) << 50;
                else solo = true;
            }
        }
        const uint32_t peers = __match_any_sync(0xffffffffu, solo ? (0xffffull << 48 | (unsigned long long)(threadIdx.x)) : (ins | fold));
        if (ins != ~0ull && (solo || lane == __ffs(peers) - 1)) {
            bool fresh = true;
            if (!solo) {
                const unsigned long long want = (ins | fold) + 1ull;
                uint32_t h = uint32_t((want * 0x9E3779B97F4A7C15ull) >> 54);
                for (int probe = 0; probe < 16; ++probe) {
                    const unsigned long long cur = atomicCAS(s_seen + h, 0ull, want);
                    if (cur == 0ull) break;
                    if (cur == want) { fresh = false; break; }
                    h = (h + 1u) & uint32_t(SC_SLOTS - 1);
                }
            }
            if (fresh) gh_insert(hash + size_t(smp) * GH_SLOTS, ins, overflow + smp);
        }
    }
}

__global__ void __launch_bounds__(256) k_tile_ranges(const int32_t *__restrict__ mstart, const int32_t *__restrict__ tile_sample,
                                                     const int32_t *__restrict__ tile_first, int32_t n_tiles, int2 *__restrict__ range) {
    const int t = blockIdx.x * blockDim.x + threadIdx.x;
    if (t >= n_tiles) return;
    const int s = tile_sample[t];
    const int lt = t - tile_first[s];
    const int b0 = mstart[s], b1 = mstart[s + 1];
    const int begin = min(b1, b0 + lt * RS_TILE);
    range[t] = make_int2(begin, min(b1, begin + RS_TILE));
}


template <typename KeyT>
__global__ void __launch_bounds__(1024) k_group_rank(const unsigned long long *__restrict__ hash, const double *__restrict__ wtable, int32_t code_bits,
                                                     uint16_t *__restrict__ slot_gid, int32_t *__restrict__ ngroups, KeyT *__restrict__ gkeys,
                                                     double4 *__restrict__ gw, int *__restrict__ overflow) {
    __shared__ unsigned long long sm[GH_SLOTS];
    __shared__ int s_warp[33];
    const int s = blockIdx.x;
    const unsigned long long *tab = hash + size_t(s) * GH_SLOTS;
    unsigned long long v[4];
    int cnt = 0;
#pragma unroll
    for (int j = 0; j < 4; ++j) {
        v[j] = tab[4 * threadIdx.x + j];
        cnt += v[j] != 0ull;
    }
    int n;
    int at = block_excl_scan(cnt, &n, s_warp);
    int P = 1;
    while (P < n) P <<= 1;
    for (int j = threadIdx.x; j < P; j += blockDim.x) sm[j] = ~0ull;
    __syncthreads();
#pragma unroll
    for (int j = 0; j < 4; ++j)
        if (v[j] != 0ull) sm[at++] = ((v[j] - 1ull) << 12) | (unsigned long long)(4 * threadIdx.x + j);
    __syncthreads();
    for (int k = 2; k <= P; k <<= 1) {
        for (int j = k >> 1; j > 0; j >>= 1) {
            for (int i = threadIdx.x; i < P; i += blockDim.x) {
                const int x = i ^ j;
                if (x > i) {
                    const unsigned long long a = sm[i], c = sm[x];
                    const bool up = (i & k) == 0;
                    if ((a > c) == up) { sm[i] = c; sm[x] = a; }
                }
            }
            __syncthreads();
        }
    }
    const int ng = min(n, GH_MAX_GROUPS);
    uint16_t *out = slot_gid + size_t(s) * GH_SLOTS;
    for (int p = threadIdx.x; p < n; p += blockDim.x) {
        const unsigned long long e = sm[p];
        out[e & 4095ull] = uint16_t(min(p, GH_MAX_GROUPS - 1));
        if (p < ng) {
            const KeyT key = KeyT(e >> 12);
            gkeys[size_t(s) * GH_MAX_GROUPS + p] = key;
            double4 w;
            w.x = __ldg(wtable + gs_code(key, 0, code_bits));
            w.y = __ldg(wtable + gs_code(key, 1, code_bits));
            w.z = __ldg(wtable + gs_code(key, 2, code_bits));
            w.w = 0.0;
            gw[size_t(s) * GH_MAX_GROUPS + p] = w;
        }
    }
    if (threadIdx.x == 0) {
        ngroups[s] = ng;
        if (n > GH_MAX_GROUPS) overflow[s] = 1;
    }
}

template <typename KeyT>
__global__ void __launch_bounds__(RS_THREADS) k_group_ids(const KeyT *__restrict__ key, const int2 *__restrict__ range,
                                                         const int32_t *__restrict__ tile_sample, const unsigned long long *__restrict__ hash,
                                                         const uint16_t *__restrict__ slot_gid, const int32_t *__restrict__ ngroups,
                                                         uint16_t *__restrict__ gid, uint32_t *__restrict__ tile_hist) {
    __shared__ uint32_t h[GH_MAX_GROUPS];
    const int t = blockIdx.x;
    const int2 rg = range[t];
    const int begin = rg.x, end = rg.y;
    const int s = tile_sample[t];
    const int ng = ngroups[s];
    if (begin >= end) {
        for (int d = threadIdx.x; d < ng; d += RS_THREADS) tile_hist[size_t(t) * GH_MAX_GROUPS + d] = 0u;
        return;
    }
    for (int d = threadIdx.x; d < ng; d += RS_THREADS) h[d] = 0u;
    const int lane = threadIdx.x & 31, warp = threadIdx.x >> 5;
    const unsigned long long *tab = hash + size_t(s) * GH_SLOTS;
    const uint16_t *sg = slot_gid + size_t(s) * GH_SLOTS;
    KeyT k[RS_PER_THREAD];
#pragma unroll
    for (int e = 0; e < RS_PER_THREAD; ++e) {
        const int i = begin + warp * (32 * RS_PER_THREAD) + e * 32 + lane;
        k[e] = i < end ? key[i] : KeyT(0);
    }
    __syncthreads();
#pragma unroll
    for (int e = 0; e < RS_PER_THREAD; ++e) {
        const int i = begin + warp * (32 * RS_PER_THREAD) + e * 32 + lane;
        if (i < end) {
            const uint32_t g = min(uint32_t(__ldg(sg + gh_find(tab, (unsigned long long)(k[e])))), uint32_t(max(ng, 1) - 1));
            gid[i] = uint16_t(g);
            atomicAdd(h + g, 1u);
        }
    }
    __syncthreads();
    uint32_t *out = tile_hist + size_t(t) * GH_MAX_GROUPS;
    for (int d = threadIdx.x; d < ng; d += RS_THREADS) out[d] = h[d];
}

__global__ void __launch_bounds__(1024) k_group_scan(uint32_t *__restrict__ tile_hist, const int32_t *__restrict__ tile_first,
                                                     const int32_t *__restrict__ ngroups, int32_t *__restrict__ goff) {
    __shared__ int s_warp[33];
    const int s = blockIdx.x;
    const int ng = ngroups[s];
    const int t0 = tile_first[s], t1 = tile_first[s + 1];
    constexpr int PITCH = GH_MAX_GROUPS, U = 8;
    uint32_t tot[2] = {0u, 0u};
    const int d0 = 2 * threadIdx.x;
#pragma unroll
    for (int j = 0; j < 2; ++j) {
        if (d0 + j < ng) {
            uint32_t run = 0u;
            for (int t = t0; t < t1; t += U) {
                uint32_t c[U];
#pragma unroll
                for (int u = 0; u < U; ++u) c[u] = t + u < t1 ? tile_hist[size_t(t + u) * PITCH + d0 + j] : 0u;
#pragma unroll
                for (int u = 0; u < U; ++u) {
                    if (t + u < t1) tile_hist[size_t(t + u) * PITCH + d0 + j] = run;
                    run += c[u];
                }
            }
            tot[j] = run;
        }
    }
    int all;
    const int ex = block_excl_scan(int(tot[0] + tot[1]), &all, s_warp);
    int32_t *out = goff + size_t(s) * (GH_MAX_GROUPS + 1);
    if (d0 < ng) out[d0] = ex;
    if (d0 + 1 < ng) out[d0 + 1] = ex + int(tot[0]);
    if (threadIdx.x == 0) out[ng] = all;
}

__global__ void __launch_bounds__(RS_THREADS, 3) k_group_place(const uint16_t *__restrict__ gid_in,
                                                              const int32_t *__restrict__ pair_db_in, const int32_t *__restrict__ pair_s_in,
                                                              int32_t *__restrict__ pair_db_out, int32_t *__restrict__ pair_s_out,
                                                              const int32_t *__restrict__ mstart, const int32_t *__restrict__ tile_sample,
                                                              const int32_t *__restrict__ tile_first, const int2 *__restrict__ range,
                                                              const uint32_t *__restrict__ tile_hist, const int32_t *__restrict__ ngroups,
                                                              const int32_t *__restrict__ goff, unsigned int *__restrict__ work_counter) {
    extern __shared__ uint32_t rs_sm[];
    if (blockIdx.x == 0 && threadIdx.x == 0) *work_counter = 0u;
    constexpr int NW = RS_THREADS / 32;
    constexpr int PITCH = GH_MAX_GROUPS;
    uint16_t *whist = reinterpret_cast<uint16_t *>(rs_sm);
    uint32_t *off = rs_sm + NW * PITCH / 2;
    const int t = blockIdx.x;
    const int2 rg = range[t];
    const int begin = rg.x, end = rg.y;
    const int s = tile_sample[t];
    if (begin >= end) return;
    const int lane = threadIdx.x & 31, warp = threadIdx.x >> 5;
    uint32_t d[RS_PER_THREAD];
    int32_t pdb[RS_PER_THREAD], ps[RS_PER_THREAD];
#pragma unroll
    for (int e = 0; e < RS_PER_THREAD; ++e) {
        const int i = begin + warp * (32 * RS_PER_THREAD) + e * 32 + lane;
        const bool on = i < end;
        d[e] = on ? uint32_t(gid_in[i]) : 0xffffffffu;
        pdb[e] = on ? pair_db_in[i] : 0;
        ps[e] = on && pair_s_out ? pair_s_in[i] : 0;
    }
    const int ng = ngroups[s];
    const int base = mstart[s];
    for (int j = threadIdx.x; j < NW * PITCH / 2; j += RS_THREADS) rs_sm[j] = 0u;
    for (int g = threadIdx.x; g < ng; g += RS_THREADS)
        off[g] = uint32_t(__ldg(goff + size_t(s) * (GH_MAX_GROUPS + 1) + g)) + __ldg(tile_hist + size_t(t) * PITCH + g);
    __syncthreads();
    const uint32_t lt_mask = (1u << lane) - 1u;
    uint16_t *mine_h = whist + size_t(warp) * PITCH;
    uint32_t rank[RS_PER_THREAD];
#pragma unroll
    for (int e = 0; e < RS_PER_THREAD; ++e) {
        const bool on = d[e] != 0xffffffffu;
        const uint32_t peers = __match_any_sync(0xffffffffu, d[e]);
        uint32_t prior = 0u;
        if (on) prior = mine_h[d[e]];
        __syncwarp();
        if (on && lane == __ffs(peers) - 1) mine_h[d[e]] = uint16_t(prior + __popc(peers));
        __syncwarp();
        rank[e] = prior + uint32_t(__popc(peers & lt_mask));
    }
    __syncthreads();
    for (int g = threadIdx.x; g < ng; g += RS_THREADS) {
        uint32_t run = 0u;
#pragma unroll
        for (int w = 0; w < NW; ++w) {
            const uint32_t c = whist[size_t(w) * PITCH + g];
            whist[size_t(w) * PITCH + g] = uint16_t(run);
            run += c;
        }
    }
    __syncthreads();
#pragma unroll
    for (int e = 0; e < RS_PER_THREAD; ++e) {
        if (d[e] != 0xffffffffu) {
            const int o = base + int(off[d[e]]) + int(mine_h[d[e]]) + int(rank[e]);
            pair_db_out[o] = pdb[e];
            if (pair_s_out) pair_s_out[o] = ps[e];
        }
    }
}

constexpr int SEG_CLASSES = 16;
constexpr int SO_LEVELS = 128;
constexpr int SO_BUCKETS = SEG_CLASSES * SO_LEVELS;
__device__ __forceinline__ int seg_cost_class(int cost, int base) {
    const int r = (cost * 16) / max(base, 1);
    const int lim[SEG_CLASSES - 1] = {384, 256, 192, 160, 128, 96, 80, 64, 48, 40, 32, 28, 24, 20, 18};
    int c = 0;
#pragma unroll
    for (int k = 0; k < SEG_CLASSES - 1; ++k) c += r < lim[k] ? 1 : 0;
    return c;
}

constexpr int SEG_COST_BLOCK = 8;
constexpr int SEG_COST_CHANGE = 8;
template <typename KeyT>
__device__ __forceinline__ void group_marks_body(int s, const int32_t *s_off, int ng, const KeyT *__restrict__ gkeys,
                                                 const int32_t *__restrict__ mstart, const int32_t *__restrict__ seg_off, int32_t chunk,
                                                 int32_t code_bits, unsigned long long *__restrict__ blk_chg, int32_t *__restrict__ seg_cost,
                                                 int32_t jcap, int32_t *__restrict__ bucket_cnt, int2 *__restrict__ seg_br) {
    const int m = mstart[s + 1] - mstart[s];
    const int seg0 = seg_off[s];
    const int nseg_s = seg_off[s + 1] - seg0;
    for (int j = threadIdx.x; j < nseg_s; j += blockDim.x) {
        const int rows = min(chunk, m - j * chunk);
        atomicAdd(seg_cost + seg0 + j, SEG_COST_BLOCK * ((rows + 15) / 16));
    }
    if (m > 0 && ng > 0) {
        unsigned long long *out = blk_chg + size_t(seg0) * size_t(chunk / 16);
        const KeyT *gk = gkeys + size_t(s) * GH_MAX_GROUPS;
        const int b = code_bits;
        for (int g = 1 + threadIdx.x; g < ng; g += blockDim.x) {
            const int r = s_off[g];
            if (r >= m || s_off[g + 1] == r) continue;
            const KeyT k1 = gk[g], k0 = gk[g - 1];
            const int c1 = int(k1 >> (3 * b)) & 3, c0 = int(k0 >> (3 * b)) & 3;
            unsigned long long bits = 0ull;
            if (c1 != c0) {
                bits = 1ull | (1ull << 16) | (1ull << 32);
            } else {
                const KeyT dd = k1 ^ k0;
                const uint32_t fm = (1u << b) - 1u;
#pragma unroll
                for (int w = 0; w < 3; ++w)
                    if ((uint32_t(dd >> gs_field_shift(c1, w, b)) & fm) != 0u) bits |= 1ull << (16 * w);
            }
            atomicOr(out + (r >> 4), bits << (r & 15));
            atomicAdd(seg_cost + seg0 + r / chunk, SEG_COST_CHANGE * __popcll(bits));
        }
        const int nb = (m + 15) / 16;
        for (int blk = threadIdx.x; blk < nb; blk += blockDim.x) {
            int lo = 0, hi = ng;
            const int r = 16 * blk;
            while (hi - lo > 1) {
                const int mid = (lo + hi) >> 1;
                if (s_off[mid] <= r) lo = mid; else hi = mid;
            }
            atomicOr(out + blk, (unsigned long long)(lo) << 48);
        }
    }
    __threadfence();
    __syncthreads();
    const int base = SEG_COST_BLOCK * (chunk / 16);
    const int jdiv = (jcap + SO_LEVELS - 1) / SO_LEVELS;
    for (int j = threadIdx.x; j < nseg_s; j += blockDim.x) {
        const int bkt = seg_cost_class(__ldcg(seg_cost + seg0 + j), base) * SO_LEVELS + min(SO_LEVELS - 1, j / jdiv);
        seg_br[seg0 + j] = make_int2(bkt, atomicAdd(bucket_cnt + bkt, 1));
    }
}

template <typename KeyT>
__global__ void __launch_bounds__(1024) k_group_marks(const int32_t *__restrict__ goff, const KeyT *__restrict__ gkeys, const int32_t *__restrict__ ngroups,
                                                      const int32_t *__restrict__ mstart, const int32_t *__restrict__ seg_off, int32_t chunk,
                                                      int32_t code_bits, unsigned long long *__restrict__ blk_chg, int32_t *__restrict__ seg_cost,
                                                      int32_t jcap, int32_t *__restrict__ bucket_cnt, int2 *__restrict__ seg_br) {
    __shared__ int32_t s_off[GH_MAX_GROUPS + 1];
    const int s = blockIdx.x;
    const int ng = ngroups[s];
    for (int g = threadIdx.x; g <= ng; g += blockDim.x) s_off[g] = goff[size_t(s) * (GH_MAX_GROUPS + 1) + g];
    __syncthreads();
    group_marks_body<KeyT>(s, s_off, ng, gkeys, mstart, seg_off, chunk, code_bits, blk_chg, seg_cost, jcap, bucket_cnt, seg_br);
}

constexpr int GP_WARPS = 32;
constexpr int GP_MAX_PAIRS = 65535;
constexpr size_t GP_SMEM = size_t(GP_WARPS) * GH_MAX_GROUPS * 2 + size_t(GH_MAX_GROUPS + 4) * 4;
template <typename KeyT>
__global__ void __launch_bounds__(32 * GP_WARPS) k_group_sample(
        const KeyT *__restrict__ key, const unsigned long long *__restrict__ hash, const uint16_t *__restrict__ slot_gid,
        const int32_t *__restrict__ ngroups, uint16_t *__restrict__ gid, const int32_t *__restrict__ pair_db_in,
        const int32_t *__restrict__ pair_s_in, int32_t *__restrict__ pair_db_out, int32_t *__restrict__ pair_s_out,
        int32_t *__restrict__ goff, const KeyT *__restrict__ gkeys, const int32_t *__restrict__ mstart,
        const int32_t *__restrict__ seg_off, int32_t chunk, int32_t code_bits, unsigned long long *__restrict__ blk_chg,
        int32_t *__restrict__ seg_cost, int32_t jcap, int32_t *__restrict__ bucket_cnt, int2 *__restrict__ seg_br,
        unsigned int *__restrict__ work_counter) {
    extern __shared__ __align__(16) unsigned char gp_smem[];
    __shared__ int s_warp[33];
    uint16_t *whist = reinterpret_cast<uint16_t *>(gp_smem);
    uint32_t *whist32 = reinterpret_cast<uint32_t *>(gp_smem);
    int32_t *s_off = reinterpret_cast<int32_t *>(gp_smem + size_t(GP_WARPS) * GH_MAX_GROUPS * 2);
    if (blockIdx.x == 0 && threadIdx.x == 0) *work_counter = 0u;
    const int s = blockIdx.x;
    const int ng = ngroups[s];
    const int b0 = mstart[s], m = min(mstart[s + 1] - b0, GP_MAX_PAIRS);
    const int lane = threadIdx.x & 31, warp = threadIdx.x >> 5;
    const int used_words = (ng + 1) / 2;
    for (int j = threadIdx.x; j < GP_WARPS * used_words; j += blockDim.x) whist32[size_t(j / used_words) * (GH_MAX_GROUPS / 2) + j % used_words] = 0u;
    __syncthreads();
    const int per = ((m + GP_WARPS - 1) / GP_WARPS + 31) & ~31;
    const int r0 = min(m, warp * per), r1 = min(m, r0 + per);
    uint16_t *mine = whist + size_t(warp) * GH_MAX_GROUPS;
    const unsigned long long *tab = hash + size_t(s) * GH_SLOTS;
    const uint16_t *sg = slot_gid + size_t(s) * GH_SLOTS;
    const uint32_t last_id = uint32_t(max(ng, 1) - 1);
    constexpr int U = 8;
    for (int base = r0; base < r1; base += 32 * U) {
        unsigned long long want[U], cur[U];
        uint32_t h[U];
#pragma unroll
        for (int u = 0; u < U; ++u) {
            const int i = base + 32 * u + lane;
            want[u] = i < r1 ? (unsigned long long)(key[b0 + i]) + 1ull : 0ull;
            h[u] = gh_hash(want[u] - 1ull);
        }
#pragma unroll
        for (int u = 0; u < U; ++u) cur[u] = want[u] ? __ldg(tab + h[u]) : 0ull;
#pragma unroll
        for (int u = 0; u < U; ++u) {
            for (int probe = 1; probe < GH_SLOTS && cur[u] != want[u] && cur[u] != 0ull; ++probe) {
                h[u] = (h[u] + 1u) & uint32_t(GH_SLOTS - 1);
                cur[u] = __ldg(tab + h[u]);
            }
        }
        uint32_t g[U];
#pragma unroll
        for (int u = 0; u < U; ++u) g[u] = want[u] ? min(uint32_t(__ldg(sg + h[u])), last_id) : 0xffffffffu;
#pragma unroll
        for (int u = 0; u < U; ++u) {
            if (base + 32 * u >= r1) break;
            const int i = base + 32 * u + lane;
            const bool on = i < r1;
            if (on) gid[b0 + i] = uint16_t(g[u]);
            const uint32_t peers = __match_any_sync(0xffffffffu, g[u]);
            if (on && lane == __ffs(peers) - 1) mine[g[u]] = uint16_t(mine[g[u]] + __popc(peers));
            __syncwarp();
        }
    }
    __syncthreads();
    uint32_t tot0 = 0u, tot1 = 0u;
    if (2 * int(threadIdx.x) < ng) {
#pragma unroll 8
        for (int w = 0; w < GP_WARPS; ++w) {
            const uint32_t c = whist32[size_t(w) * (GH_MAX_GROUPS / 2) + threadIdx.x];
            whist32[size_t(w) * (GH_MAX_GROUPS / 2) + threadIdx.x] = tot0 | (tot1 << 16);
            tot0 += c & 0xffffu;
            tot1 += c >> 16;
        }
    }
    int all;
    const int ex = block_excl_scan(int(tot0 + tot1), &all, s_warp);
    int32_t *out = goff + size_t(s) * (GH_MAX_GROUPS + 1);
    const int d0 = 2 * int(threadIdx.x);
    if (d0 < ng) { s_off[d0] = ex; out[d0] = ex; }
    if (d0 + 1 < ng) { s_off[d0 + 1] = ex + int(tot0); out[d0 + 1] = ex + int(tot0); }
    if (threadIdx.x == 0) { s_off[ng] = all; out[ng] = all; }
    __syncthreads();
    const uint32_t lt_mask = (1u << lane) - 1u;
    for (int base = r0; base < r1; base += 32 * U) {
        uint32_t g[U];
        int32_t pdb[U], ps[U];
#pragma unroll
        for (int u = 0; u < U; ++u) {
            const int i = base + 32 * u + lane;
            const bool on = i < r1;
            g[u] = on ? uint32_t(gid[b0 + i]) : 0xffffffffu;
            pdb[u] = on ? pair_db_in[b0 + i] : 0;
            ps[u] = on && pair_s_out ? pair_s_in[b0 + i] : 0;
        }
#pragma unroll
        for (int u = 0; u < U; ++u) {
            if (base + 32 * u >= r1) break;
            const bool on = g[u] != 0xffffffffu;
            const uint32_t peers = __match_any_sync(0xffffffffu, g[u]);
            uint32_t prior = 0u;
            if (on) prior = mine[g[u]];
            __syncwarp();
            if (on && lane == __ffs(peers) - 1) mine[g[u]] = uint16_t(prior + __popc(peers));
            __syncwarp();
            if (on) {
                const int o = b0 + s_off[g[u]] + int(prior) + __popc(peers & lt_mask);
                pair_db_out[o] = pdb[u];
                if (pair_s_out) pair_s_out[o] = ps[u];
            }
        }
    }
    __syncthreads();
    group_marks_body<KeyT>(s, s_off, ng, gkeys, mstart, seg_off, chunk, code_bits, blk_chg, seg_cost, jcap, bucket_cnt, seg_br);
}

__global__ void __launch_bounds__(256) k_order_place(const int32_t *__restrict__ bucket_cnt, const int2 *__restrict__ seg_br, const int32_t *__restrict__ seg_off,
                                                    const int32_t *__restrict__ mstart, int32_t chunk, int4 *__restrict__ order) {
    __shared__ int scan[SO_BUCKETS];
    __shared__ int warp_sum[8];
    const int s = blockIdx.x, t = threadIdx.x;
    const int seg0 = seg_off[s], nseg_s = seg_off[s + 1] - seg0;
    if (nseg_s <= 0) return;
    constexpr int PT = SO_BUCKETS / 256;
    int v[PT], sum = 0;
#pragma unroll
    for (int k = 0; k < PT; ++k) { v[k] = __ldcg(bucket_cnt + PT * t + k); sum += v[k]; }
    int incl = sum;
#pragma unroll
    for (int d = 1; d < 32; d <<= 1) {
        const int u = __shfl_up_sync(0xffffffffu, incl, d);
        if ((t & 31) >= d) incl += u;
    }
    if ((t & 31) == 31) warp_sum[t >> 5] = incl;
    __syncthreads();
    int run = incl - sum;
    for (int w = 0; w < (t >> 5); ++w) run += warp_sum[w];
#pragma unroll
    for (int k = 0; k < PT; ++k) { scan[PT * t + k] = run; run += v[k]; }
    __syncthreads();
    const int m0 = mstart[s], m1 = mstart[s + 1];
    for (int j = t; j < nseg_s; j += blockDim.x) {
        const int2 br = seg_br[seg0 + j];
        const int begin = m0 + j * chunk;
        order[scan[br.x] + br.y] = make_int4(seg0 + j, begin, min(m1, begin + chunk) - begin, s);
    }
}

}
```

snpmatch_b200/csrc/grouped.cuh:

```cuda
#pragma once
#include "common.cuh"
#include "hardcall.cuh"

namespace snpm {

constexpr int GR_THREADS = 128;
constexpr int GR_MAX_WX = 36;
constexpr int GR_MAX_TEAMS = 3;
constexpr int GR_BLOCK = 16;
constexpr int GR_RING = 64;
constexpr int GR_INFLIGHT = GR_RING / GR_BLOCK;
constexpr int GR_LP = 10;
constexpr int GR_MAX_CHUNK = 1008;

struct GroupArgs {
    const uint64_t *packed;
    int32_t stride;
    const int32_t *pair_db;
    const uint16_t *pair_gid;
    const double *table;
    const int32_t *seg_off;
    const int32_t *mstart;
    int32_t S;
    int32_t chunk;
// ... 94 lines not shown

__device__ __forceinline__ void fold_counts(const BitCounter<GR_LP> &c, double w, double (&F)[32]) {
    uint32_t t[8];
#pragma unroll
    for (int k = 0; k < 8; ++k) t[k] = c.p[k];
    transpose_planes8(t);
    if ((c.p[8] | c.p[9]) == 0u) {
#pragma unroll
        for (int i = 0; i < 8; ++i) {
#pragma unroll
            for (int j = 0; j < 4; ++j) {
                const int cnt = int((t[i] >> (8 * j)) & 0xffu);
                F[8 * j + i] = fma(w, double(cnt), F[8 * j + i]);
            }
        }
    } else {
#pragma unroll
        for (int i = 0; i < 8; ++i) {
#pragma unroll
            for (int j = 0; j < 4; ++j) {
                const int b = 8 * j + i;
                const int cnt = int((t[i] >> (8 * j)) & 0xffu) | int(((c.p[8] >> b) & 1u) << 8) | int(((c.p[9] >> b) & 1u) << 9);
                F[b] = fma(w, double(cnt), F[b]);
            }
        }
    }
}

__device__ __forceinline__ void counter_values(const BitCounter<GR_LP> &c, int32_t (&v)[32]) {
    uint32_t t[8];
#pragma unroll
    for (int k = 0; k < 8; ++k) t[k] = c.p[k];
    transpose_planes8(t);
#pragma unroll
    for (int i = 0; i < 8; ++i) {
#pragma unroll
        for (int j = 0; j < 4; ++j) {
            const int b = 8 * j + i;
            v[b] = int32_t((t[i] >> (8 * j)) & 0xffu) | int32_t(((c.p[8] >> b) & 1u) << 8) | int32_t(((c.p[9] >> b) & 1u) << 9);
        }
    }
}

__host__ __device__ __forceinline__ size_t grouped_team_smem(int wx, int chunk) {
    const size_t n_blocks = size_t(chunk + GR_BLOCK - 1) / GR_BLOCK;
    return size_t(GR_RING) * wx * 8 + size_t(chunk) * 4 + ((size_t(chunk) * 2 + 15) & ~size_t(15)) + ((n_blocks * 8 + 15) & ~size_t(15));
}

template <bool SKIP_HETS, int WX>
__global__ void __launch_bounds__(GR_THREADS, 2) k_score_grouped(const GroupArgs a) {
    extern __shared__ __align__(16) unsigned char gr_smem[];
    const int wx = WX ? WX : a.wx;
    const int spc = a.spc;
    const int q = threadIdx.x / wx, w = threadIdx.x - q * wx;
    const int slot = blockIdx.x * spc + q;
    const int word = blockIdx.y * wx + w;
    int seg = 0, begin = 0, end = 0;
    bool team_ok = false;
    if (q < spc) {
        const int j = a.jmax - 1 - slot / a.S, smp = slot % a.S;
        if (j >= 0 && j < a.seg_off[smp + 1] - a.seg_off[smp]) {
            team_ok = true;
            seg = a.seg_off[smp] + j;
            begin = a.mstart[smp] + j * a.chunk;
            end = min(a.mstart[smp + 1], begin + a.chunk);
        }
    }
    const int n_rows = end - begin;
    const int n_blocks = (n_rows + GR_BLOCK - 1) / GR_BLOCK;
    unsigned char *team = gr_smem + size_t(q < spc ? q : 0) * grouped_team_smem(wx, a.chunk);
    uint64_t *ring = reinterpret_cast<uint64_t *>(team);
    int32_t *s_row = reinterpret_cast<int32_t *>(team + size_t(GR_RING) * wx * 8);
    uint16_t *s_gid = reinterpret_cast<uint16_t *>(team + size_t(GR_RING) * wx * 8 + size_t(a.chunk) * 4);
    unsigned long long *s_chg = reinterpret_cast<unsigned long long *>(team + size_t(GR_RING) * wx * 8 + size_t(a.chunk) * 4 +
                                                                       ((size_t(a.chunk) * 2 + 15) & ~size_t(15)));
    if (team_ok) {
        for (int b = w; b < n_blocks; b += wx) s_chg[b] = 0ull;
#pragma unroll 4
        for (int r = w; r < n_rows; r += wx) {
            s_row[r] = __ldg(a.pair_db + begin + r);
            s_gid[r] = __ldg(a.pair_gid + begin + r);
        }
    }
    __syncthreads();
    if (team_ok) {
        for (int r = w + 1; r < n_rows; r += wx) {
            const int g1 = s_gid[r], g0 = s_gid[r - 1];
            if (g1 != g0) {
                const double4 t1 = reinterpret_cast<const double4 *>(a.table)[g1];
                const double4 t0 = reinterpret_cast<const double4 *>(a.table)[g0];
                unsigned long long f = 0ull;
                if (t1.x != t0.x) f |= 1ull << (r & 15);
                if (t1.y != t0.y) f |= 1ull << (16 + (r & 15));
                if (t1.z != t0.z) f |= 1ull << (32 + (r & 15));
                if (f) atomicOr(s_chg + (r >> 4), f);
            }
        }
    }
    __syncthreads();
    if (!team_ok || word >= a.stride) return;

    const uint32_t my_ring = smem_u32(ring + w);
    const uint32_t ring_pitch = uint32_t(wx) * 8u;
    const int64_t stride = a.stride;
    const int n_full = n_rows / GR_BLOCK;
    const int odd = w & 1;
    const uint32_t pair_ring = smem_u32(ring + (w & ~1));
    const unsigned char *pair_col = reinterpret_cast<const unsigned char *>(a.packed + (word & ~1));
    const uint32_t stride_b = uint32_t(a.stride) * 8u;
    constexpr unsigned pair_mask = 0xffffffffu;
    auto issue = [&](int b) {
        const int r0 = b * GR_BLOCK + 8 * odd;
        const uint32_t slot0 = pair_ring + uint32_t(r0 % GR_RING) * ring_pitch;
        if (b < n_full) {
#pragma unroll
            for (int k4 = 0; k4 < GR_BLOCK / 2; k4 += 4) {
                const int4 rr = *reinterpret_cast<const int4 *>(s_row + r0 + k4);
                cp_async16(slot0 + uint32_t(k4 + 0) * ring_pitch, pair_col + (unsigned long long)(uint32_t(rr.x)) * stride_b);
                cp_async16(slot0 + uint32_t(k4 + 1) * ring_pitch, pair_col + (unsigned long long)(uint32_t(rr.y)) * stride_b);
                cp_async16(slot0 + uint32_t(k4 + 2) * ring_pitch, pair_col + (unsigned long long)(uint32_t(rr.z)) * stride_b);
                cp_async16(slot0 + uint32_t(k4 + 3) * ring_pitch, pair_col + (unsigned long long)(uint32_t(rr.w)) * stride_b);
            }
        } else if (b < n_blocks) {
            for (int k = 0; k < GR_BLOCK / 2 && r0 + k < n_rows; ++k) cp_async16(slot0 + uint32_t(k) * ring_pitch, pair_col + (unsigned long long)(uint32_t(s_row[r0 + k])) * stride_b);
        }
        cp_async_commit();
    };
#pragma unroll
    for (int b = 0; b < GR_INFLIGHT; ++b) issue(b);

    double F[32];
#pragma unroll
    for (int b = 0; b < 32; ++b) F[b] = 0.0;
    BitCounter<GR_LP> c_int, c_ninfo, c_ref, c_alt, c_het;
    c_int.clear();
    c_ninfo.clear();
    c_ref.clear();
    c_alt.clear();
    c_het.clear();
    double w_ref, w_alt, w_het;
    {
        const double4 t = *reinterpret_cast<const double4 *>(a.table + 4 * size_t(s_gid[0]));
        w_ref = t.x;
        w_alt = t.y;
        w_het = t.z;
    }
    auto flush_class = [&](BitCounter<GR_LP> &c, double wt) {
        if (c.any()) {
            c_ninfo.add_counter(c);
            if (wt == 1.0) c_int.add_counter(c);
            else if (wt != 0.0) fold_counts(c, wt, F);
            c.clear();
        }
    };
    auto add_class = [&](BitCounter<GR_LP> &c, double &wt, const uint32_t (&pl)[GR_BLOCK], uint32_t mask, int which, int r0) {
        if (mask == 0u) {
            c.add16(pl);
            return;
        }
        int k0 = 0;
        while (true) {
            const int k1 = mask ? __ffs(mask) - 1 : GR_BLOCK;
            if (k1 > k0) {
                const uint32_t rm = ((1u << k1) - 1u) & ~((1u << k0) - 1u);
                uint32_t m[GR_BLOCK];
#pragma unroll
                for (int k = 0; k < GR_BLOCK; ++k) m[k] = pl[k] & uint32_t(int32_t(rm << (31 - k)) >> 31);
                c.add16(m);
            }
            if (k1 >= GR_BLOCK) break;
            flush_class(c, wt);
            wt = a.table[4 * size_t(s_gid[r0 + k1]) + which];
            mask &= mask - 1u;
            k0 = k1;
        }
    };
    auto score_block = [&](const uint32_t (&lo)[GR_BLOCK], const uint32_t (&hi)[GR_BLOCK], int b) {
        const unsigned long long chg = s_chg[b];
        uint32_t pl[GR_BLOCK];
#pragma unroll
        for (int k = 0; k < GR_BLOCK; ++k) pl[k] = ~(lo[k] | hi[k]);
        add_class(c_ref, w_ref, pl, uint32_t(chg) & 0xffffu, 0, b * GR_BLOCK);
#pragma unroll
        for (int k = 0; k < GR_BLOCK; ++k) pl[k] = lo[k] & ~hi[k];
        add_class(c_alt, w_alt, pl, uint32_t(chg >> 16) & 0xffffu, 1, b * GR_BLOCK);
        if (!SKIP_HETS) {
#pragma unroll
            for (int k = 0; k < GR_BLOCK; ++k) pl[k] = hi[k] & ~lo[k];
            add_class(c_het, w_het, pl, uint32_t(chg >> 32) & 0xffffu, 2, b * GR_BLOCK);
        }
    };

    for (int b = 0; b < n_full; ++b) {
        cp_async_wait<GR_INFLIGHT - 1>();
        __syncwarp(pair_mask);
        const uint64_t *slot = ring + size_t((b * GR_BLOCK) % GR_RING) * wx + w;
        uint32_t lo[GR_BLOCK], hi[GR_BLOCK];
#pragma unroll
        for (int k = 0; k < GR_BLOCK; ++k) {
            const uint64_t v = slot[size_t(k) * wx];
            lo[k] = uint32_t(v);
            hi[k] = uint32_t(v >> 32);
        }
        score_block(lo, hi, b);
        __syncwarp(pair_mask);
        issue(b + GR_INFLIGHT);
    }
    if (n_full < n_blocks) {
        cp_async_wait<0>();
        __syncwarp(pair_mask);
        const int r0 = n_full * GR_BLOCK;
        const uint64_t *slot = ring + size_t(r0 % GR_RING) * wx + w;
        uint32_t lo[GR_BLOCK], hi[GR_BLOCK];
#pragma unroll
        for (int k = 0; k < GR_BLOCK; ++k) {
            uint64_t v = ~0ull;
            if (r0 + k < n_rows) v = slot[size_t(k) * wx];
            lo[k] = uint32_t(v);
            hi[k] = uint32_t(v >> 32);
        }
        score_block(lo, hi, n_full);
    }
    flush_class(c_ref, w_ref);
    flush_class(c_alt, w_alt);
    if (!SKIP_HETS) flush_class(c_het, w_het);

    int32_t vi[32], vn[32];
    counter_values(c_int, vi);
    counter_values(c_ninfo, vn);
    const int64_t o = int64_t(seg) * a.a_pad + word;
    const int64_t lane_pitch = a.stride;
#pragma unroll
    for (int b = 0; b < 32; ++b) {
        a.part_score[o + b * lane_pitch] = F[b];
        a.part_int[o + b * lane_pitch] = vi[b] | (vn[b] << 16);
    }
}

__global__ void __launch_bounds__(JOIN_TILE) k_scatter_pairs_grouped(
        const int32_t *__restrict__ match_row, int64_t n, const int32_t *__restrict__ tile_off, const uint16_t *__restrict__ gid,
        int32_t n_table, int32_t *__restrict__ prefix, int32_t *__restrict__ pair_db, int32_t *__restrict__ pair_s,
        uint16_t *__restrict__ pair_gid, int *status) {
    __shared__ int s_warp[33];
    const int64_t i = int64_t(blockIdx.x) * JOIN_TILE + threadIdx.x;
    const int32_t row = i < n ? match_row[i] : -1;
    const int flag = row >= 0;
    int total;
    const int ex = block_excl_scan(flag, &total, s_warp);
    if (i < n) {
        const int32_t p = tile_off[blockIdx.x] + ex;
        prefix[i] = p;
        if (flag) {
            pair_db[p] = row;
            pair_s[p] = int32_t(i);
            uint16_t g = gid[i];
            if (int32_t(g) >= n_table) {
                atomicAdd(status + 4, 1);
                g = 0;
            }
            pair_gid[p] = g;
        }
    }
}

__global__ void __launch_bounds__(256) k_expand_chrom(const uint8_t *__restrict__ c8, int64_t n, int32_t *__restrict__ c32) {
    const int64_t i = int64_t(blockIdx.x) * blockDim.x + threadIdx.x;
    if (i < n) c32[i] = c8[i] == 255 ? -1 : int32_t(c8[i]);
}

__global__ void __launch_bounds__(256) k_expand_packed(const uint32_t *__restrict__ cp, int64_t n, int32_t *__restrict__ c32, int32_t *__restrict__ pos) {
    const int64_t i = int64_t(blockIdx.x) * blockDim.x + threadIdx.x;
    if (i < n) {
        const uint32_t v = cp[i];
        const uint32_t c = v >> 27;
        c32[i] = c == 31u ? -1 : int32_t(c);
        pos[i] = int32_t(v & 0x7ffffffu);
    }
}

__global__ void __launch_bounds__(256) k_expand_runs(const uint32_t *__restrict__ run_end, const uint16_t *__restrict__ run_gid, int32_t n_runs,
                                                     int64_t n, uint16_t *__restrict__ gid, int *__restrict__ status_bad) {
    const int lane = threadIdx.x & 31;
    const int64_t r = (int64_t(blockIdx.x) * blockDim.x + threadIdx.x) >> 5;
    if (r >= n_runs) return;
    const int64_t begin = r ? int64_t(__ldg(run_end + r - 1)) : 0, end = int64_t(__ldg(run_end + r));
    if (end <= begin || end > n) {
        if (lane == 0) atomicAdd(status_bad, 1);
        return;
    }
    const uint16_t g = __ldg(run_gid + r);
    for (int64_t i = begin + lane; i < end; i += 32) gid[i] = g;
}

constexpr int CG_PARTS = 8;
__global__ void __launch_bounds__(32 * CG_PARTS) k_combine_grouped(const double *__restrict__ part_score, const int32_t *__restrict__ part_int,
                                                                   int32_t a_pad, int32_t stride, int32_t n_acc,
                                                                   const int32_t *__restrict__ seg_off, const int32_t *__restrict__ mstart,
                                                                   double *__restrict__ red) {
    __shared__ double s_f[CG_PARTS][32];
    __shared__ long long s_i[CG_PARTS][32], s_n[CG_PARTS][32];
    const int s = blockIdx.y;
    const int x = threadIdx.x & 31, y = threadIdx.x >> 5;
    const int p = blockIdx.x * 32 + x;
    const int j0 = seg_off[s], j1 = seg_off[s + 1];
    const int per = (j1 - j0 + CG_PARTS - 1) / CG_PARTS;
    const int ja = min(j1, j0 + y * per), jb = min(j1, ja + per);
    double f = 0.0;
    long long ii = 0, ni = 0;
    if (p < a_pad) {
        constexpr int CB = 8;
        int j = ja;
        for (; j + CB <= jb; j += CB) {
            double v[CB];
            int32_t ci[CB];
#pragma unroll
            for (int k = 0; k < CB; ++k) {
                v[k] = __ldg(part_score + int64_t(j + k) * a_pad + p);
                ci[k] = __ldg(part_int + int64_t(j + k) * a_pad + p);
            }
#pragma unroll
            for (int k = 0; k < CB; ++k) {
                f += v[k];
                ii += ci[k] & 0xffff;
                ni += ci[k] >> 16;
            }
        }
        for (; j < jb; ++j) {
            f += part_score[int64_t(j) * a_pad + p];
            const int32_t c = part_int[int64_t(j) * a_pad + p];
            ii += c & 0xffff;
            ni += c >> 16;
        }
    }
    s_f[y][x] = f;
    s_i[y][x] = ii;
    s_n[y][x] = ni;
    __syncthreads();
    double *row = red + int64_t(s) * (3 * int64_t(n_acc) + 2);
    if (y == 0) {
        const int b = p / stride, w = p - b * stride;
        const int acc = 32 * w + b;
        if (p < a_pad && acc < n_acc) {
#pragma unroll
            for (int k = 1; k < CG_PARTS; ++k) {
                f += s_f[k][x];
                ii += s_i[k][x];
                ni += s_n[k][x];
            }
            row[acc] = f;
            row[n_acc + acc] = double(ni);
            row[2 * n_acc + 2 + acc] = double(ii);
        }
        if (p == 0) {
            row[2 * n_acc] = double(mstart[s + 1] - mstart[s]);
            row[2 * n_acc + 1] = 0.0;
        }
    }
}

constexpr int PR_MAX_WORLD = 16;
constexpr int PR_FLAG_BYTES = 4096;
constexpr int PR_DONE_OFF = 64;
struct PeerPtrs {
    const double *p[PR_MAX_WORLD];
    uint32_t *flags[PR_MAX_WORLD];
};
__device__ __forceinline__ uint32_t ld_acquire_sys_u32(const uint32_t *p) {
    uint32_t v;
    asm volatile("ld.acquire.sys.global.u32 %0, [%1];" : "=r"(v) : "l"(p) : "memory");
    return v;
}
__device__ __forceinline__ void st_release_sys_u32(uint32_t *p, uint32_t v) {
    asm volatile("st.release.sys.global.u32 [%0], %1;" ::"l"(p), "r"(v) : "memory");
}
__device__ __forceinline__ unsigned long long global_timer_ns() {
    unsigned long long t;
    asm volatile("mov.u64 %0, %%globaltimer;" : "=l"(t));
    return t;
}
__device__ __forceinline__ bool spin_until(const uint32_t *f, uint32_t want) {
    const unsigned long long t0 = global_timer_ns();
    while (int32_t(ld_acquire_sys_u32(f) - want) < 0) {
        __nanosleep(40);
        if (global_timer_ns() - t0 > 30000000000ull) return false;
    }
    return true;
}
template <typename V>
__device__ __forceinline__ V ld_peer(const double *p);
template <>
__device__ __forceinline__ double ld_peer<double>(const double *p) {
    double v;
    asm volatile("ld.volatile.global.f64 %0, [%1];" : "=d"(v) : "l"(p) : "memory");
    return v;
}
template <>
__device__ __forceinline__ double2 ld_peer<double2>(const double *p) {
    double2 v;
    asm volatile("ld.volatile.global.v2.f64 {%0, %1}, [%2];" : "=d"(v.x), "=d"(v.y) : "l"(p) : "memory");
    return v;
}

template <typename V>
__global__ void __launch_bounds__(256) k_reduce_peers(const PeerPtrs peers, int32_t world, int32_t rank, uint32_t step, int64_t first, int64_t count,
                                                      double *__restrict__ own, int *status) {
    constexpr int W = int(sizeof(V) / sizeof(double));
    __shared__ int s_last;
    if (blockIdx.x == 0 && threadIdx.x < world) {
        __threadfence_system();
        st_release_sys_u32(peers.flags[threadIdx.x] + rank, step);
    }
    const unsigned long long t_wait = global_timer_ns();
    if (threadIdx.x < world && !spin_until(peers.flags[rank] + threadIdx.x, step)) atomicExch(status + 5, 1);
    __syncthreads();
    if (blockIdx.x == 0 && threadIdx.x == 0) status[7] = int(global_timer_ns() - t_wait);
    const int64_t nv = count / W;
    for (int64_t i = int64_t(blockIdx.x) * blockDim.x + threadIdx.x; i < nv; i += int64_t(gridDim.x) * blockDim.x) {
        const int64_t o = first + W * i;
        double acc[W];
#pragma unroll
        for (int k = 0; k < W; ++k) acc[k] = 0.0;
#pragma unroll 4
        for (int r = 0; r < world; ++r) {
            const V v = ld_peer<V>(peers.p[r] + o);
            const double *e = reinterpret_cast<const double *>(&v);
#pragma unroll
            for (int k = 0; k < W; ++k) acc[k] += e[k];
        }
#pragma unroll
        for (int k = 0; k < W; ++k) own[o + k] = acc[k];
    }
    __syncthreads();
    if (threadIdx.x == 0) {
        __threadfence();
        const int prev = atomicAdd(status + 6, 1);
        s_last = prev == int(gridDim.x) - 1;
        if (s_last) status[6] = 0;
    }
    __syncthreads();
    if (s_last && threadIdx.x < world) st_release_sys_u32(peers.flags[threadIdx.x] + PR_DONE_OFF + rank, step);
}

__global__ void __launch_bounds__(32) k_wait_peers_done(const uint32_t *own_flags, int32_t world, uint32_t want, int *status) {
    if (threadIdx.x < world && !spin_until(own_flags + PR_DONE_OFF + threadIdx.x, want)) atomicExch(status + 5, 1);
}

__global__ void __launch_bounds__(256) k_grouped_finalize(double *__restrict__ red, int32_t n_acc, int32_t *__restrict__ guard,
                                                          const int *__restrict__ overflow = nullptr) {
    const int s = blockIdx.y;
    const int acc = blockIdx.x * blockDim.x + threadIdx.x;
    if (acc >= n_acc) return;
    if (acc == 0 && overflow != nullptr && overflow[s]) atomicAdd(guard + s, 1);
    double *row = red + int64_t(s) * (3 * int64_t(n_acc) + 2);
    const double f = row[acc], ii = row[2 * n_acc + 2 + acc], m = row[2 * n_acc];
    const double depth = 1010.0 + m * (1.0 / 500.0);
    const double g = 4.0 * depth * 1.1102230246251565e-16 * (ii + f + 1.0);
    const double k = rint(f);
    if (k >= 1.0 && fabs(f - k) <= g) atomicAdd(guard + s, 1);
    const double want = ii + floor(f);
    double v = ii + f;
    if (floor(v) != want) v = __longlong_as_double(__double_as_longlong(want + 1.0) - 1);
    row[acc] = v;
}

}
```

snpmatch_b200/csrc/grouped2.cuh:

```cuda
#pragma once
#include "common.cuh"
#include "grouped.cuh"
#include "group_sort.cuh"

namespace snpm {

constexpr int G2_WX = 36;
constexpr int G2_MAX_TEAMS = 8;
constexpr int G2_THREADS = 256;
constexpr int G2_MAX_CHUNK = 496;
constexpr int G2_CP = 9;
constexpr int G2_TP = 9;

struct Group2Args {
    const uint64_t *packed;
    int32_t stride;
    const int32_t *pair_db;
    const unsigned long long *blk_chg;
    const double *gw;
    const int32_t *seg_off;
    const int32_t *mstart;
    int32_t S;
    int32_t chunk;
    double *part_score;
    int32_t *part_int;
    int32_t a_pad;
    int32_t wx;
    int32_t teams;
    int32_t n_slices;
    const int4 *order;
    unsigned int *work_counter;
};

__device__ __forceinline__ void cp_async4(uint32_t dst_smem, const void *src_gmem) {
    asm volatile("cp.async.ca.shared.global [%0], [%1], 4;" ::"r"(dst_smem), "l"(src_gmem) : "memory");
}

struct G2Item {
    int32_t seg;
    int32_t begin;
    int32_t n_rows;
    int32_t slice;
    int32_t smp;
};

__host__ __device__ __forceinline__ size_t g2_stage_bytes(int chunk) {
    return (size_t(chunk) * 4 + size_t(chunk / 16 + 1) * 8 + 15) & ~size_t(15);
}
__host__ __device__ __forceinline__ size_t g2_team_smem(int wx, int chunk, int ring) {
    return size_t(ring) * wx * 8 + 2 * g2_stage_bytes(chunk);
}

__device__ __forceinline__ void bytes_to_f64(uint32_t t, double &d0, double &d1, double &d2, double &d3) {
    asm("{\n\t.reg .b8 b0, b1, b2, b3;\n\tmov.b32 {b0, b1, b2, b3}, %4;\n\tcvt.rn.f64.u8 %0, b0;\n\tcvt.rn.f64.u8 %1, b1;\n\t"
        "cvt.rn.f64.u8 %2, b2;\n\tcvt.rn.f64.u8 %3, b3;\n\t}"
        : "=d"(d0), "=d"(d1), "=d"(d2), "=d"(d3)
        : "r"(t));
}

template <int K>
__device__ __forceinline__ uint32_t row_if_bit(uint32_t pl, uint32_t rm) {
    uint32_t r;
    asm("{\n\t.reg .pred p;\n\t.reg .b32 t;\n\tand.b32 t, %2, %3;\n\tsetp.ne.u32 p, t, 0;\n\tselp.b32 %0, %1, 0, p;\n\t}"
        : "=r"(r)
        : "r"(pl), "r"(rm), "n"(1u << K));
    return r;
}
template <int K>
struct MaskRows {
    static __device__ __forceinline__ void go(uint32_t (&m)[GR_BLOCK], const uint32_t (&pl)[GR_BLOCK], uint32_t rm) {
        m[K] = row_if_bit<K>(pl[K], rm);
        MaskRows<K - 1>::go(m, pl, rm);
    }
};
template <>
struct MaskRows<-1> {
    static __device__ __forceinline__ void go(uint32_t (&)[GR_BLOCK], const uint32_t (&)[GR_BLOCK], uint32_t) {}
};

__device__ __forceinline__ void fold_counts9(const BitCounter<G2_CP> &c, double w, double (&F)[32]) {
    uint32_t t[8];
#pragma unroll
    for (int k = 0; k < 8; ++k) t[k] = c.p[k];
    transpose_planes8(t);
    if (c.p[8] == 0u) {
#pragma unroll
        for (int i = 0; i < 8; ++i) {
            double d0, d1, d2, d3;
            bytes_to_f64(t[i], d0, d1, d2, d3);
            F[i] = fma(w, d0, F[i]);
            F[8 + i] = fma(w, d1, F[8 + i]);
            F[16 + i] = fma(w, d2, F[16 + i]);
            F[24 + i] = fma(w, d3, F[24 + i]);
        }
    } else {
#pragma unroll
        for (int i = 0; i < 8; ++i) {
#pragma unroll
            for (int j = 0; j < 4; ++j) {
                const int b = 8 * j + i;
                const int cnt = int((t[i] >> (8 * j)) & 0xffu) | int(((c.p[8] >> b) & 1u) << 8);
                F[b] = fma(w, double(cnt), F[b]);
            }
        }
    }
}

__device__ __forceinline__ void counter_values9(const BitCounter<G2_TP> &c, int32_t (&v)[32]) {
    uint32_t t[8];
#pragma unroll
    for (int k = 0; k < 8; ++k) t[k] = c.p[k];
    transpose_planes8(t);
#pragma unroll
    for (int i = 0; i < 8; ++i) {
#pragma unroll
        for (int j = 0; j < 4; ++j) {
            const int b = 8 * j + i;
            v[b] = int32_t((t[i] >> (8 * j)) & 0xffu) | int32_t(((c.p[8] >> b) & 1u) << 8);
        }
    }
}

template <bool SKIP_HETS, int WX, int RING>
__global__ void __launch_bounds__(G2_THREADS, 1) k_score_grouped2(const Group2Args a) {
    constexpr int INFLIGHT = RING / GR_BLOCK;
    extern __shared__ __align__(16) unsigned char g2_smem[];
    __shared__ int s_base[2];
    const int wx = WX ? WX : a.wx;
    const int q = threadIdx.x / wx, w = threadIdx.x - q * wx;
    const bool in_team = q < a.teams;
    const size_t team_bytes = g2_team_smem(wx, a.chunk, RING);
    const size_t stage_bytes = g2_stage_bytes(a.chunk);
    unsigned char *team = g2_smem + size_t(in_team ? q : 0) * team_bytes;
    uint64_t *ring = reinterpret_cast<uint64_t *>(team);
    unsigned char *stage0 = team + size_t(RING) * wx * 8;
    const int n_items = __ldg(a.seg_off + a.S) * a.n_slices;
    auto decode = [&](int i) {
        G2Item it;
        it.seg = -1; it.begin = 0; it.n_rows = 0; it.slice = 0; it.smp = 0;
        if (in_team && i < n_items) {
            const int rank = i / a.n_slices;
            const int4 o = __ldg(a.order + rank);
            it.seg = o.x;
            it.begin = o.y;
            it.n_rows = o.z;
            it.slice = i - rank * a.n_slices;
            it.smp = o.w;
        }
        return it;
    };
    auto prefetch = [&](const G2Item &it, int buf) {
        if (it.seg >= 0) {
            unsigned char *st = stage0 + size_t(buf) * stage_bytes;
            const uint32_t s_row = smem_u32(st), s_chg = s_row + uint32_t(a.chunk) * 4u;
            for (int r = w; r < it.n_rows; r += wx) cp_async4(s_row + uint32_t(r) * 4u, a.pair_db + it.begin + r);
            const int nb = (it.n_rows + GR_BLOCK - 1) / GR_BLOCK;
            const unsigned long long *src = a.blk_chg + size_t(it.seg) * size_t(a.chunk / GR_BLOCK);
            for (int b = w; b < nb; b += wx) cp_async8(s_chg + uint32_t(b) * 8u, src + b);
        }
        cp_async_commit();
    };

    const int G = int(gridDim.x), T = a.teams;
    const int R = (n_items + T - 1) / T;
    const int dyn_end = max(G, R - 2 * G);
    const int second = R - 1 - int(blockIdx.x), third = R - 1 - G - int(blockIdx.x);
    if (threadIdx.x == 0) {
        s_base[0] = int(blockIdx.x) * T;
        s_base[1] = second >= max(G, R - G) ? second * T : n_items;
    }
    __syncthreads();
    if (s_base[0] >= n_items) return;
    G2Item cur = decode(s_base[0] + q);
    prefetch(cur, 0);
    cp_async_wait<0>();
    __syncthreads();
    int buf = 0;
    bool first_round = true;

    const int64_t stride = a.stride;
    const int odd = w & 1;
    const uint32_t ring_pitch = uint32_t(wx) * 8u;
    const uint32_t stride_b = uint32_t(a.stride) * 8u;
    const int nb_round = a.chunk / GR_BLOCK;

    while (true) {
        const int next_base = s_base[buf ^ 1];
        int ticket = 0;
        if (threadIdx.x == 0 && next_base < n_items) {
            if (first_round) {
                ticket = third >= dyn_end && third < R - G ? third * T : n_items;
            } else {
                const int r = G + int(atomicAdd(a.work_counter, 1u));
                ticket = r < dyn_end ? r * T : n_items;
            }
        }
        first_round = false;
        const G2Item nxt = decode(next_base + q);
        prefetch(nxt, buf ^ 1);
        const unsigned char *st = stage0 + size_t(buf) * stage_bytes;
        const int32_t *s_row = reinterpret_cast<const int32_t *>(st);
        const unsigned long long *s_chg = reinterpret_cast<const unsigned long long *>(st + size_t(a.chunk) * 4);
        const double *gwp = a.gw + size_t(cur.smp) * (4 * GH_MAX_GROUPS);
        const int n_rows = cur.n_rows;
        const int n_blocks = (n_rows + GR_BLOCK - 1) / GR_BLOCK;
        const int n_full = n_rows / GR_BLOCK;
        const int word = cur.slice * wx + w;
        const bool live = in_team && n_rows > 0 && word < a.stride;
        const unsigned char *col = reinterpret_cast<const unsigned char *>(a.packed + (word & ~1));
        const uint32_t my_ring = smem_u32(ring + (w & ~1));
        auto issue = [&](int b) {
            if (live) {
                const int r0 = b * GR_BLOCK + 8 * odd;
                const uint32_t slot0 = my_ring + uint32_t(r0 % RING) * ring_pitch;
                if (b < n_full) {
#pragma unroll
                    for (int k4 = 0; k4 < GR_BLOCK / 2; k4 += 4) {
                        const int4 rr = *reinterpret_cast<const int4 *>(s_row + r0 + k4);
                        cp_async16(slot0 + uint32_t(k4 + 0) * ring_pitch, col + (unsigned long long)(uint32_t(rr.x)) * stride_b);
                        cp_async16(slot0 + uint32_t(k4 + 1) * ring_pitch, col + (unsigned long long)(uint32_t(rr.y)) * stride_b);
                        cp_async16(slot0 + uint32_t(k4 + 2) * ring_pitch, col + (unsigned long long)(uint32_t(rr.z)) * stride_b);
                        cp_async16(slot0 + uint32_t(k4 + 3) * ring_pitch, col + (unsigned long long)(uint32_t(rr.w)) * stride_b);
                    }
                } else if (b < n_blocks) {
                    for (int k = 0; k < GR_BLOCK / 2 && r0 + k < n_rows; ++k)
                        cp_async16(slot0 + uint32_t(k) * ring_pitch, col + (unsigned long long)(uint32_t(s_row[r0 + k])) * stride_b);
                }
            }
            cp_async_commit();
        };
#pragma unroll
        for (int b = 0; b < INFLIGHT; ++b) issue(b);

        double F[32];
#pragma unroll
        for (int b = 0; b < 32; ++b) F[b] = 0.0;
        BitCounter<G2_TP> c_int, c_ninfo;
        BitCounter<G2_CP> c_ref, c_alt, c_het;
        c_int.clear();
        c_ninfo.clear();
        c_ref.clear();
        c_alt.clear();
        c_het.clear();
        double w_ref = 0.0, w_alt = 0.0, w_het = 0.0;
        if (n_rows > 0) {
            const double *w0 = gwp + 4 * int(s_chg[0] >> 48);
            w_ref = __ldg(w0);
            w_alt = __ldg(w0 + 1);
            w_het = __ldg(w0 + 2);
        }
        auto flush_class = [&](BitCounter<G2_CP> &c, double wt) {
            if (c.any()) {
                c_ninfo.add_counter(c);
                if (wt == 1.0) c_int.add_counter(c);
                else if (wt != 0.0) fold_counts9(c, wt, F);
                c.clear();
            }
        };
        auto add_class = [&](BitCounter<G2_CP> &c, double &wt, const uint32_t (&pl)[GR_BLOCK], uint32_t mask, int which, unsigned long long chg) {
            if (mask == 0u) {
                c.add16(pl);
                return;
            }
            int k0 = 0;
            while (true) {
                const int k1 = mask ? __ffs(mask) - 1 : GR_BLOCK;
                if (k1 > k0) {
                    const uint32_t rm = ((1u << k1) - 1u) & ~((1u << k0) - 1u);
                    uint32_t m[GR_BLOCK];
                    if (WX != 32) {
                        MaskRows<GR_BLOCK - 1>::go(m, pl, rm);
                    } else {
#pragma unroll
                        for (int k = 0; k < GR_BLOCK; ++k) m[k] = pl[k] & uint32_t(int32_t(rm << (31 - k)) >> 31);
                    }
                    c.add16(m);
                }
                if (k1 >= GR_BLOCK) break;
                flush_class(c, wt);
                const uint32_t starts = uint32_t(chg | (chg >> 16) | (chg >> 32)) & 0xffffu;
                const int g = int(chg >> 48) + __popc(starts & ((2u << k1) - 2u));
                wt = __ldg(gwp + 4 * g + which);
                mask &= mask - 1u;
                k0 = k1;
            }
        };
        auto score_block = [&](const uint32_t (&lo)[GR_BLOCK], const uint32_t (&hi)[GR_BLOCK], int b) {
            const unsigned long long chg = s_chg[b];
            uint32_t pl[GR_BLOCK];
#pragma unroll
            for (int k = 0; k < GR_BLOCK; ++k) pl[k] = ~(lo[k] | hi[k]);
            add_class(c_ref, w_ref, pl, uint32_t(chg) & 0xffffu, 0, chg);
#pragma unroll
            for (int k = 0; k < GR_BLOCK; ++k) pl[k] = lo[k] & ~hi[k];
            add_class(c_alt, w_alt, pl, uint32_t(chg >> 16) & 0xffffu, 1, chg);
            if (!SKIP_HETS) {
#pragma unroll
                for (int k = 0; k < GR_BLOCK; ++k) pl[k] = hi[k] & ~lo[k];
                add_class(c_het, w_het, pl, uint32_t(chg >> 32) & 0xffffu, 2, chg);
            }
        };

        for (int b = 0; b < nb_round; ++b) {
            cp_async_wait<INFLIGHT - 2>();
            __syncwarp();
            if (b > 0) issue(b + INFLIGHT - 1);
            if (b < n_full) {
                const uint64_t *slot = ring + size_t((b * GR_BLOCK) % RING) * wx + w;
                uint32_t lo[GR_BLOCK], hi[GR_BLOCK];
#pragma unroll
                for (int k = 0; k < GR_BLOCK; ++k) {
                    const uint64_t v = slot[size_t(k) * wx];
                    lo[k] = uint32_t(v);
                    hi[k] = uint32_t(v >> 32);
                }
                score_block(lo, hi, b);
            } else if (b < n_blocks) {
                const int r0 = b * GR_BLOCK;
                const uint64_t *slot = ring + size_t(r0 % RING) * wx + w;
                uint32_t lo[GR_BLOCK], hi[GR_BLOCK];
#pragma unroll
                for (int k = 0; k < GR_BLOCK; ++k) {
                    uint64_t v = ~0ull;
                    if (r0 + k < n_rows) v = slot[size_t(k) * wx];
                    lo[k] = uint32_t(v);
                    hi[k] = uint32_t(v >> 32);
                }
                score_block(lo, hi, b);
            }
        }
        flush_class(c_ref, w_ref);
        flush_class(c_alt, w_alt);
        if (!SKIP_HETS) flush_class(c_het, w_het);
        if (live) {
            int32_t vi[32], vn[32];
            counter_values9(c_int, vi);
            counter_values9(c_ninfo, vn);
            const int64_t o = int64_t(cur.seg) * a.a_pad + word;
#pragma unroll
            for (int b = 0; b < 32; ++b) {
                a.part_score[o + b * stride] = F[b];
                a.part_int[o + b * stride] = vi[b] | (vn[b] << 16);
            }
        }
        cp_async_wait<0>();
        if (next_base >= n_items) break;
        if (threadIdx.x == 0) s_base[buf] = ticket;
        __syncthreads();
        cur = nxt;
        buf ^= 1;
    }
}

}
```

snpmatch_b200/csrc/join.cuh:

```cuda
#pragma once
#include "common.cuh"

namespace snpm {

constexpr int JOIN_TILE = 1024;

__device__ __forceinline__ int64_t lower_bound_i32(const int32_t *__restrict__ a, int64_t lo, int64_t hi, int32_t key) {
    while (lo < hi) {
        const int64_t mid = (lo + hi) >> 1;
        if (__ldg(a + mid) < key) lo = mid + 1; else hi = mid;
    }
    return lo;
}

__device__ __forceinline__ bool contains_i64(const int64_t *__restrict__ a, int64_t n, int64_t key) {
    int64_t lo = 0, hi = n;
    while (lo < hi) {
        const int64_t mid = (lo + hi) >> 1;
        if (__ldg(a + mid) < key) lo = mid + 1; else hi = mid;
    }
    return lo < n && __ldg(a + lo) == key;
}

__device__ __forceinline__ void check_order(const int32_t *__restrict__ chrom, const int32_t *__restrict__ pos,
                                            const int64_t *__restrict__ off, int64_t S, int64_t i, int *status) {
    if (i == 0) return;
    const int32_t c1 = chrom[i], c0 = chrom[i - 1];
    if (c1 < 0 || c0 < 0) return;
    const bool bad = (c1 < c0) || (c1 == c0 && pos[i] <= pos[i - 1]);
    if (!bad) return;
    int64_t lo = 0, hi = S + 1;
    while (lo < hi) {
        const int64_t mid = (lo + hi) >> 1;
        if (off[mid] < i) lo = mid + 1; else hi = mid;
    }
    if (lo <= S && off[lo] == i) return;
    atomicAdd(status, 1);
}

__global__ void __launch_bounds__(256) k_build_buckets(const int32_t *__restrict__ db_pos, const int64_t *__restrict__ chr_regions,
                                                       int32_t n_chr, const int32_t *__restrict__ bucket_off, int shift,
                                                       int32_t *__restrict__ bucket) {
    const int64_t i = int64_t(blockIdx.x) * blockDim.x + threadIdx.x;
    if (i >= bucket_off[n_chr]) return;
    int c = 0;
    while (c + 1 < n_chr && bucket_off[c + 1] <= i) ++c;
    const int64_t b = i - bucket_off[c];
    const int64_t rs = chr_regions[2 * c], re = chr_regions[2 * c + 1];
    const int64_t key = b << shift;
    bucket[i] = key > 0x7fffffffll ? int32_t(re) : int32_t(lower_bound_i32(db_pos, rs, re, int32_t(key)));
}

__global__ void __launch_bounds__(256) k_bitmap_set(const int32_t *__restrict__ db_pos, const int64_t *__restrict__ chr_regions, int32_t n_chr,
                                                    const int64_t *__restrict__ bm_off, int64_t n_rows, unsigned long long *__restrict__ bitmap) {
    const int64_t r = int64_t(blockIdx.x) * blockDim.x + threadIdx.x;
    if (r >= n_rows) return;
    int c = 0;
    while (c + 1 < n_chr && !(r >= chr_regions[2 * c] && r < chr_regions[2 * c + 1])) ++c;
    if (!(r >= chr_regions[2 * c] && r < chr_regions[2 * c + 1])) return;
    const int32_t p = db_pos[r];
    if (p < 0) return;
    const int64_t bit = bm_off[c] + p;
    atomicOr(bitmap + (bit >> 6), 1ull << (bit & 63));
}
__global__ void __launch_bounds__(256) k_bitmap_rows(const int32_t *__restrict__ db_pos, const int64_t *__restrict__ chr_regions, int32_t n_chr,
                                                     const int64_t *__restrict__ bm_off, int64_t n_words, int32_t *__restrict__ first_row) {
    const int64_t w = int64_t(blockIdx.x) * blockDim.x + threadIdx.x;
    if (w >= n_words) return;
    int c = 0;
    while (c + 1 < n_chr && bm_off[c + 1] <= w * 64) ++c;
    const int64_t rs = chr_regions[2 * c], re = chr_regions[2 * c + 1];
    const int64_t p0 = w * 64 - bm_off[c];
    first_row[w] = p0 > 0x7fffffffll ? int32_t(re) : int32_t(lower_bound_i32(db_pos, rs, re, int32_t(p0)));
}

__global__ void __launch_bounds__(JOIN_TILE) k_join_search(
        const int32_t *__restrict__ chrom, const int32_t *__restrict__ pos, int64_t n,
        const int64_t *__restrict__ off, int64_t S,
        const int32_t *__restrict__ db_pos, const int64_t *__restrict__ chr_regions, int32_t n_chr,
        const int32_t *__restrict__ bucket, const int32_t *__restrict__ bucket_off, int shift,
        const int64_t *__restrict__ filter, int64_t n_filter, int64_t row0_global,
        int32_t *__restrict__ match_row, int32_t *__restrict__ tile_cnt, int *status, int check,
        const unsigned long long *__restrict__ bitmap, const int32_t *__restrict__ first_row, const int64_t *__restrict__ bm_off,
        const uint32_t *__restrict__ packed_cp) {
    const int64_t i = int64_t(blockIdx.x) * JOIN_TILE + threadIdx.x;
    int32_t row = -1;
    if (i < n) {
        int32_t c, p;
        if (packed_cp != nullptr) {
            const uint32_t v = packed_cp[i];
            c = (v >> 27) == 31u ? -1 : int32_t(v >> 27);
            p = int32_t(v & 0x7ffffffu);
            if (check && i > 0 && c >= 0) {
                const uint32_t v0 = packed_cp[i - 1];
                if ((v0 >> 27) != 31u && v <= v0) {
                    int64_t lo = 0, hi = S + 1;
                    while (lo < hi) {
                        const int64_t mid = (lo + hi) >> 1;
                        if (off[mid] < i) lo = mid + 1; else hi = mid;
                    }
                    if (!(lo <= S && off[lo] == i)) atomicAdd(status, 1);
                }
            }
        } else {
            if (check) check_order(chrom, pos, off, S, i, status);
            c = chrom[i];
            p = pos[i];
        }
        if (c >= 0 && c < n_chr) {
            const int32_t b0 = bucket_off[c], nb = bucket_off[c + 1] - b0 - 1;
            const int32_t b = p >> shift;
            if (bitmap != nullptr) {
                const int64_t bit = bm_off[c] + p;
                if (p >= 0 && bit < bm_off[c + 1]) {
                    const int64_t w = bit >> 6;
                    const unsigned long long word = __ldg(bitmap + w);
                    const int32_t base = __ldg(first_row + w);
                    const unsigned long long m = 1ull << (bit & 63);
                    if (word & m) {
                        row = base + __popcll(word & (m - 1ull));
                        if (filter && !contains_i64(filter, n_filter, int64_t(row) + row0_global)) row = -1;
                    }
                }
            } else if (p >= 0 && b < nb) {
                const int64_t rs = __ldg(bucket + b0 + b), re = __ldg(bucket + b0 + b + 1);
                const int64_t j = lower_bound_i32(db_pos, rs, re, p);
                if (j < re && __ldg(db_pos + j) == p) {
                    row = int32_t(j);
                    if (filter && !contains_i64(filter, n_filter, j + row0_global)) row = -1;
                }
            }
        }
        match_row[i] = row;
    }
    const int cnt = __syncthreads_count(row >= 0);
    if (threadIdx.x == 0) tile_cnt[blockIdx.x] = cnt;
}

constexpr int MP_TILE = 1024;
constexpr int MP_DB_CHUNK = 4096;

__global__ void __launch_bounds__(256) k_join_mergepath(
        const int32_t *__restrict__ chrom, const int32_t *__restrict__ pos, int64_t n,
        const int64_t *__restrict__ off, int64_t S,
        const int32_t *__restrict__ db_pos, const int64_t *__restrict__ chr_regions, int32_t n_chr,
        const int64_t *__restrict__ filter, int64_t n_filter, int64_t row0_global,
        int32_t *__restrict__ match_row, int32_t *__restrict__ tile_cnt, int *status) {
    __shared__ int32_t s_pos[MP_TILE];
    __shared__ int32_t s_chr[MP_TILE];
    __shared__ int32_t s_db[MP_DB_CHUNK];
    __shared__ int32_t s_cnt;
    __shared__ int32_t s_next;
    __shared__ uint8_t s_brk[MP_TILE];
    const int64_t base = int64_t(blockIdx.x) * MP_TILE;
    const int tile_n = int((n - base) < int64_t(MP_TILE) ? (n - base) : int64_t(MP_TILE));
    if (threadIdx.x == 0) s_cnt = 0;
    for (int t = threadIdx.x; t < tile_n; t += blockDim.x) {
        check_order(chrom, pos, off, S, base + t, status);
        s_pos[t] = pos[base + t];
        s_chr[t] = chrom[base + t];
    }
    __syncthreads();
    for (int t = threadIdx.x; t < tile_n; t += blockDim.x)
        s_brk[t] = t == 0 || s_chr[t] != s_chr[t - 1] || s_pos[t] <= s_pos[t - 1];
    int local_cnt = 0;
    int run_start = 0;
    while (run_start < tile_n) {
        const int32_t c = s_chr[run_start];
        __syncthreads();
        if (threadIdx.x == 0) s_next = tile_n;
        __syncthreads();
        for (int t = threadIdx.x; t < tile_n; t += blockDim.x)
            if (s_brk[t] && t > run_start) atomicMin(&s_next, t);
        __syncthreads();
        const int run_end = s_next;
        if (c < 0 || c >= n_chr) {
            for (int t = run_start + threadIdx.x; t < run_end; t += blockDim.x) match_row[base + t] = -1;
            run_start = run_end;
            continue;
        }
        const int64_t rs = chr_regions[2 * c], re = chr_regions[2 * c + 1];
        const int32_t p_first = s_pos[run_start], p_last = s_pos[run_end - 1];
        const int64_t d0 = lower_bound_i32(db_pos, rs, re, p_first);
        const int64_t d1 = lower_bound_i32(db_pos, d0, re, p_last + 1);
        for (int t = run_start + threadIdx.x; t < run_end; t += blockDim.x) match_row[base + t] = -1;
        for (int64_t dc = d0; dc < d1; dc += MP_DB_CHUNK) {
            const int chunk_n = int((d1 - dc) < int64_t(MP_DB_CHUNK) ? (d1 - dc) : int64_t(MP_DB_CHUNK));
            __syncthreads();
            for (int t = threadIdx.x; t < chunk_n; t += blockDim.x) s_db[t] = __ldg(db_pos + dc + t);
            __syncthreads();
            const int32_t lo_key = s_db[0], hi_key = s_db[chunk_n - 1];
            int m0 = run_start, m1 = run_end;
            {
                int lo = run_start, hi = run_end;
                while (lo < hi) { const int mid = (lo + hi) >> 1; if (s_pos[mid] < lo_key) lo = mid + 1; else hi = mid; }
                m0 = lo;
                hi = run_end;
                while (lo < hi) { const int mid = (lo + hi) >> 1; if (s_pos[mid] <= hi_key) lo = mid + 1; else hi = mid; }
                m1 = lo;
            }
            const int na = m1 - m0, nb = chunk_n;
            const int total = na + nb;
            const int per = (total + blockDim.x - 1) / blockDim.x;
            const int diag0 = min(total, int(threadIdx.x) * per);
            const int diag1 = min(total, diag0 + per);
            int lo = max(0, diag0 - nb), hi = min(diag0, na);
            while (lo < hi) {
                const int mid = (lo + hi) >> 1;
                if (s_pos[m0 + mid] < s_db[diag0 - 1 - mid]) lo = mid + 1; else hi = mid;
            }
            int i = lo, j = diag0 - lo;
            for (int d = diag0; d < diag1; ++d) {
                const bool take_b = (j < nb) && (i >= na || s_db[j] <= s_pos[m0 + i]);
                if (take_b) {
                    ++j;
                } else {
                    if (j > 0 && s_db[j - 1] == s_pos[m0 + i]) {
                        int32_t row = int32_t(dc + j - 1);
                        if (filter && !contains_i64(filter, n_filter, int64_t(row) + row0_global)) row = -1;
                        match_row[base + m0 + i] = row;
                        if (row >= 0) ++local_cnt;
                    }
                    ++i;
                }
            }
        }
        __syncthreads();
        run_start = run_end;
    }
    atomicAdd(&s_cnt, local_cnt);
    __syncthreads();
    if (threadIdx.x == 0) tile_cnt[blockIdx.x] = s_cnt;
}

__device__ __forceinline__ int block_excl_scan(int v, int *total, int *s_warp ) {
    const int lane = threadIdx.x & 31, warp = threadIdx.x >> 5, nwarp = blockDim.x >> 5;
    int x = v;
#pragma unroll
    for (int d = 1; d < 32; d <<= 1) {
        const int y = __shfl_up_sync(0xffffffffu, x, d);
        if (lane >= d) x += y;
    }
    if (lane == 31) s_warp[warp] = x;
    __syncthreads();
    if (warp == 0) {
        int w = lane < nwarp ? s_warp[lane] : 0;
        int xs = w;
#pragma unroll
        for (int d = 1; d < 32; d <<= 1) {
            const int y = __shfl_up_sync(0xffffffffu, xs, d);
            if (lane >= d) xs += y;
        }
        if (lane < nwarp) s_warp[lane] = xs - w;
        if (lane == 31) s_warp[32] = xs;
    }
    __syncthreads();
    const int res = s_warp[warp] + x - v;
    *total = s_warp[32];
    __syncthreads();
    return res;
}

__global__ void __launch_bounds__(1024) k_scan_tiles(const int32_t *__restrict__ tile_cnt, int64_t n_tiles,
                                                     int32_t *__restrict__ tile_off, int32_t *__restrict__ prefix_last) {
    __shared__ int s_warp[33];
    int carry = 0;
    for (int64_t base = 0; base < n_tiles; base += blockDim.x) {
        const int64_t t = base + threadIdx.x;
        const int v = t < n_tiles ? tile_cnt[t] : 0;
        int total;
        const int ex = block_excl_scan(v, &total, s_warp);
        if (t < n_tiles) tile_off[t] = carry + ex;
        carry += total;
    }
    if (threadIdx.x == 0) *prefix_last = carry;
}

__global__ void __launch_bounds__(JOIN_TILE) k_scatter_pairs(
        const int32_t *__restrict__ match_row, int64_t n, const int32_t *__restrict__ tile_off,
        const double *__restrict__ wei, int32_t *__restrict__ prefix, int32_t *__restrict__ pair_db,
        int32_t *__restrict__ pair_s, double *__restrict__ pair_w) {
    __shared__ int s_warp[33];
    const int64_t i = int64_t(blockIdx.x) * JOIN_TILE + threadIdx.x;
    const int32_t row = i < n ? match_row[i] : -1;
    const int flag = row >= 0;
    int total;
    const int ex = block_excl_scan(flag, &total, s_warp);
    if (i < n) {
        const int32_t p = tile_off[blockIdx.x] + ex;
        prefix[i] = p;
        if (flag) {
            pair_db[p] = row;
            pair_s[p] = int32_t(i);
            double4 w4;
            w4.x = wei[3 * i + 0];
            w4.y = wei[3 * i + 2];
            w4.z = wei[3 * i + 1];
            w4.w = 0.0;
            reinterpret_cast<double4 *>(pair_w)[p] = w4;
        }
    }
}

__global__ void __launch_bounds__(256) k_expand_weights(const uint16_t *__restrict__ idx, const double *__restrict__ table,
                                                        int64_t n3, double *__restrict__ wei) {
    const int64_t i = int64_t(blockIdx.x) * blockDim.x + threadIdx.x;
    if (i < n3) wei[i] = __ldg(table + idx[i]);
}

__global__ void __launch_bounds__(1024) k_sample_ranges(const int32_t *__restrict__ prefix, const int64_t *__restrict__ off,
                                                        int64_t S, int32_t chunk, int32_t *__restrict__ mstart,
                                                        int32_t *__restrict__ seg_off) {
    __shared__ int s_warp[33];
    for (int64_t s = threadIdx.x; s <= S; s += blockDim.x) mstart[s] = prefix[off[s]];
    __syncthreads();
    int carry = 0;
    for (int64_t base = 0; base < S; base += blockDim.x) {
        const int64_t s = base + threadIdx.x;
        int v = 0;
        if (s < S) v = (mstart[s + 1] - mstart[s] + chunk - 1) / chunk;
        int total;
        const int ex = block_excl_scan(v, &total, s_warp);
        if (s < S) seg_off[s] = carry + ex;
        carry += total;
    }
    if (threadIdx.x == 0) seg_off[S] = carry;
}

}
```

Measured before the change: 6246 billion.

## Fuse coded join, tile scan and pair scatter; add programmatic dependent launch

For coded batches, the separate join-search, tile-scan and scatter kernels become one k_join_scatter_coded kernel that carries prefix offsets across tiles through a decoupled-lookback tile state array. The buffer memsets move up front. The grouping pipeline folds k_tile_ranges into k_group_rank and launches the rank, sample, place, score and combine kernels with programmatic dependent launch so each launch can overlap the previous kernel's tail. The aim is fewer launches and less inter-kernel idle time, at the cost of a cross-block lookback dependency and more complex synchronization.

```diff
diff --git a/snpmatch_b200/csrc/api.cu b/snpmatch_b200/csrc/api.cu
--- a/snpmatch_b200/csrc/api.cu
+++ b/snpmatch_b200/csrc/api.cu
@@ -885,7 +885,7 @@
     if (b->ev_joined) cudaEventDestroy(b->ev_joined);
     if (b->ev_fork) cudaEventDestroy(b->ev_fork);
     if (b->ev_join) cudaEventDestroy(b->ev_join);
-    DevBuf *bufs[] = {&b->d_off, &b->d_chrom, &b->d_pos, &b->d_wei, &b->d_filter, &b->d_match_row, &b->d_tile_cnt, &b->d_tile_off,
+    DevBuf *bufs[] = {&b->d_off, &b->d_chrom, &b->d_pos, &b->d_wei, &b->d_filter, &b->d_match_row, &b->d_tile_cnt, &b->d_tile_off, &b->d_tile_state,
                       &b->d_prefix, &b->d_pair_db, &b->d_pair_s, &b->d_pair_w, &b->d_mstart, &b->d_seg_off, &b->d_part_score,
                       &b->d_part_ninfo, &b->d_red, &b->d_matches, &b->d_ninfo64, &b->d_prob, &b->d_L, &b->d_LR, &b->d_status,
                       &b->d_win_count, &b->d_win_off, &b->d_win_begin, &b->d_win_end, &b->d_kmax, &b->d_win_L, &b->d_win_LR,
@@ -979,14 +979,21 @@
     return SNPM_OK;
 }
 
+static size_t coded_zero_bytes(const snpm_batch *b) {
+    return size_t(std::max<int64_t>(b->nseg_cap, 1)) * (size_t(b->gchunk / GR_BLOCK) * 8 + 4) + size_t(SO_BUCKETS) * 4;
+}
+
 static int batch_join(snpm_batch *b, int algo) {
     snpm_db *db = b->db;
     cudaStream_t st = db->stream;
     const int64_t n = b->n, S = b->S;
     const int64_t n_tiles = ceil_div64(n, JOIN_TILE);
     SNPM_TRY(b->d_match_row.ensure(size_t(n) * 4));
-    SNPM_TRY(b->d_tile_cnt.ensure(size_t(n_tiles) * 4));
-    SNPM_TRY(b->d_tile_off.ensure(size_t(n_tiles) * 4));
+    if (b->coded) SNPM_TRY(b->d_tile_state.ensure(size_t(n_tiles + 2) * 8));
+    else {
+        SNPM_TRY(b->d_tile_cnt.ensure(size_t(n_tiles) * 4));
+        SNPM_TRY(b->d_tile_off.ensure(size_t(n_tiles) * 4));
+    }
     SNPM_TRY(b->d_prefix.ensure(size_t(n + 1) * 4));
     SNPM_TRY(b->d_pair_db.ensure(size_t(n) * 4));
     SNPM_TRY(b->d_pair_s.ensure(size_t(n) * 4));
@@ -1017,17 +1024,40 @@
     if (algo == 0) algo = (n / S) * 8 >= db->n_rows ? 2 : 1;
     if (b->grouped) algo = 1;
     const int64_t *filter = b->has_filter ? b->d_filter.as<int64_t>() : nullptr;
+    const JoinIndex jx = {db->d_pos, db->n_chr, db->d_bucket, db->d_bucket_off, db->bucket_shift, filter, b->n_filter, db->row0_global,
+                          db->d_bitmap, db->d_bm_first_row, db->d_bm_off};
+    if (b->coded && n_tiles > 0) {
+        unsigned long long *hash = b->d_hash.as<unsigned long long>();
+        SNPM_CUDA(cudaMemsetAsync(b->d_tile_state.p, 0, size_t(n_tiles + 2) * 8, st));
+        SNPM_CUDA(cudaMemsetAsync(b->d_group_overflow.p, 0, size_t(S) * 4, st));
+        SNPM_CUDA(cudaMemsetAsync(hash, 0, size_t(S) * GH_SLOTS * 8, st));
+        SNPM_CUDA(cudaMemsetAsync(b->d_blk_chg.p, 0, coded_zero_bytes(b), st));
+        const uint32_t *packed_cp = b->d_wei_idx.as<uint32_t>();
+        const uint32_t *codes32 = b->codes_packed ? b->d_codes.as<uint32_t>() : nullptr;
+        if (b->key_bits <= 32)
+            k_join_scatter_coded<uint32_t><<<int(n_tiles), SC_THREADS, 0, st>>>(
+                packed_cp, n, b->d_off.as<int64_t>(), S, jx, b->d_codes.as<uint16_t>(), codes32, b->d_wtable.as<double>(), b->n_wtable, b->code_bits,
+                b->d_match_row.as<int32_t>(), b->d_prefix.as<int32_t>(), b->d_pair_db_tmp.as<int32_t>(), b->d_pair_s_tmp.as<int32_t>(),
+                b->d_key_a.as<uint32_t>(), hash, b->d_group_overflow.as<int>(), b->d_status.as<int>(), b->d_tile_state.as<unsigned long long>(),
+                b->gchunk, b->d_mstart.as<int32_t>(), b->d_seg_off.as<int32_t>());
+        else
+            k_join_scatter_coded<uint64_t><<<int(n_tiles), SC_THREADS, 0, st>>>(
+                packed_cp, n, b->d_off.as<int64_t>(), S, jx, b->d_codes.as<uint16_t>(), codes32, b->d_wtable.as<double>(), b->n_wtable, b->code_bits,
+                b->d_match_row.as<int32_t>(), b->d_prefix.as<int32_t>(), b->d_pair_db_tmp.as<int32_t>(), b->d_pair_s_tmp.as<int32_t>(),
+                b->d_key_a.as<uint64_t>(), hash, b->d_group_overflow.as<int>(), b->d_status.as<int>(), b->d_tile_state.as<unsigned long long>(),
+                b->gchunk, b->d_mstart.as<int32_t>(), b->d_seg_off.as<int32_t>());
+        SNPM_KERNEL_CHECK();
+        b->launches += 1;
+        return SNPM_OK;
+    }
     if (n_tiles > 0) {
         if (algo == 2)
             k_join_mergepath<<<int(n_tiles), 256, 0, st>>>(b->d_chrom.as<int32_t>(), b->d_pos.as<int32_t>(), n, b->d_off.as<int64_t>(), S,
                                                          db->d_pos, db->d_chr_regions, db->n_chr, filter, b->n_filter, db->row0_global,
                                                          b->d_match_row.as<int32_t>(), b->d_tile_cnt.as<int32_t>(), b->d_status.as<int>());
         else
-            k_join_search<<<int(n_tiles), JOIN_TILE, 0, st>>>(b->d_chrom.as<int32_t>(), b->d_pos.as<int32_t>(), n, b->d_off.as<int64_t>(), S,
-                                                            db->d_pos, db->d_chr_regions, db->n_chr, db->d_bucket, db->d_bucket_off, db->bucket_shift,
-                                                            filter, b->n_filter, db->row0_global,
-                                                            b->d_match_row.as<int32_t>(), b->d_tile_cnt.as<int32_t>(), b->d_status.as<int>(), (b->grouped && !b->coded) ? 0 : 1,
-                                                            db->d_bitmap, db->d_bm_first_row, db->d_bm_off,
+            k_join_search<<<int(n_tiles), JOIN_TILE, 0, st>>>(b->d_chrom.as<int32_t>(), b->d_pos.as<int32_t>(), n, b->d_off.as<int64_t>(), S, jx,
+                                                            b->d_match_row.as<int32_t>(), b->d_tile_cnt.as<int32_t>(), b->d_status.as<int>(), b->grouped ? 0 : 1,
                                                             (b->grouped && (b->pending_expand & 2)) ? b->d_wei_idx.as<uint32_t>() : nullptr);
         SNPM_KERNEL_CHECK();
         if (b->has_seg) {
@@ -1039,21 +1069,7 @@
         }
         k_scan_tiles<<<1, 1024, 0, st>>>(b->d_tile_cnt.as<int32_t>(), n_tiles, b->d_tile_off.as<int32_t>(), b->d_prefix.as<int32_t>() + n);
         SNPM_KERNEL_CHECK();
-        if (b->coded) {
-            unsigned long long *hash = b->d_hash.as<unsigned long long>();
-            SNPM_CUDA(cudaMemsetAsync(b->d_group_overflow.p, 0, size_t(S) * 4, st));
-            SNPM_CUDA(cudaMemsetAsync(hash, 0, size_t(S) * GH_SLOTS * 8, st));
-            if (b->key_bits <= 32)
-                k_scatter_pairs_coded<uint32_t><<<int(n_tiles), SC_THREADS, 0, st>>>(b->d_match_row.as<int32_t>(), n, b->d_tile_off.as<int32_t>(), b->d_codes.as<uint16_t>(),
-                        b->d_wtable.as<double>(), b->n_wtable, b->code_bits, b->d_prefix.as<int32_t>(), b->d_pair_db_tmp.as<int32_t>(), b->d_pair_s_tmp.as<int32_t>(),
-                        b->d_key_a.as<uint32_t>(), b->d_status.as<int>(), b->d_off.as<int64_t>(), S, hash, b->d_group_overflow.as<int>(),
-                        b->codes_packed ? b->d_codes.as<uint32_t>() : nullptr);
-            else
-                k_scatter_pairs_coded<uint64_t><<<int(n_tiles), SC_THREADS, 0, st>>>(b->d_match_row.as<int32_t>(), n, b->d_tile_off.as<int32_t>(), b->d_codes.as<uint16_t>(),
-                        b->d_wtable.as<double>(), b->n_wtable, b->code_bits, b->d_prefix.as<int32_t>(), b->d_pair_db_tmp.as<int32_t>(), b->d_pair_s_tmp.as<int32_t>(),
-                        b->d_key_a.as<uint64_t>(), b->d_status.as<int>(), b->d_off.as<int64_t>(), S, hash, b->d_group_overflow.as<int>(),
-                        b->codes_packed ? b->d_codes.as<uint32_t>() : nullptr);
-        } else if (b->grouped)
+        if (b->grouped)
             k_scatter_pairs_grouped<<<int(n_tiles), JOIN_TILE, 0, st>>>(b->d_match_row.as<int32_t>(), n, b->d_tile_off.as<int32_t>(),
                                                                       b->d_gid.as<uint16_t>(), b->n_gtable, b->d_prefix.as<int32_t>(), b->d_pair_db.as<int32_t>(),
                                                                       b->d_pair_s.as<int32_t>(), b->d_pair_gid.as<uint16_t>(), b->d_status.as<int>());
@@ -1090,66 +1106,58 @@
         gattr = true;
     }
     KeyT *gkeys = b->d_gkeys.as<KeyT>();
-    k_group_rank<KeyT><<<int(b->S), 1024, 0, st>>>(b->d_hash.as<unsigned long long>(), b->d_wtable.as<double>(), b->code_bits, b->d_slot_gid.as<uint16_t>(),
-                                                   b->d_ngroups.as<int32_t>(), gkeys, b->d_gw.as<double4>(), b->d_group_overflow.as<int>());
-    int64_t n_max = 0, jcap1 = 1;
+    int64_t n_max = 0, jcap = 1;
     for (int64_t s = 0; s < b->S; ++s) {
         n_max = std::max(n_max, b->h_off[size_t(s) + 1] - b->h_off[size_t(s)]);
-        jcap1 = std::max(jcap1, ceil_div64(b->h_off[size_t(s) + 1] - b->h_off[size_t(s)], b->gchunk));
+        jcap = std::max(jcap, ceil_div64(b->h_off[size_t(s) + 1] - b->h_off[size_t(s)], b->gchunk));
     }
     const char *force = getenv("SNPM_GROUP_KERNEL");
     const bool fits = n_max <= GP_MAX_PAIRS;
-    const bool want = force ? !strcmp(force, "sample") : (n_max <= 32768 || b->S >= 128);
-    if (fits && want) {
+    const bool by_sample = fits && (force ? !strcmp(force, "sample") : (n_max <= 32768 || b->S >= 128));
+    SNPM_CUDA(launch_pdl(k_group_rank<KeyT>, dim3(unsigned(b->S)), dim3(1024), 0, st, b->d_hash.as<unsigned long long>(), b->d_wtable.as<double>(),
+                         b->code_bits, b->d_slot_gid.as<uint16_t>(), b->d_ngroups.as<int32_t>(), gkeys, b->d_gw.as<double4>(),
+                         b->d_group_overflow.as<int>(), mstart, tfirst, by_sample ? nullptr : range));
+    const size_t ncap = size_t(std::max<int64_t>(b->nseg_cap, 1));
+    int32_t *seg_cost = reinterpret_cast<int32_t *>(b->d_blk_chg.as<unsigned long long>() + ncap * size_t(b->gchunk / GR_BLOCK));
+    int32_t *bucket_cnt = seg_cost + ncap;
+    int2 *seg_br = reinterpret_cast<int2 *>(reinterpret_cast<unsigned char *>(b->d_blk_chg.p) + ((coded_zero_bytes(b) + 7) & ~size_t(7)));
+    if (by_sample) {
         static bool sattr = false;
         if (!sattr) {
             SNPM_CUDA(cudaFuncSetAttribute(k_group_sample<uint32_t>, cudaFuncAttributeMaxDynamicSharedMemorySize, int(GP_SMEM)));
             SNPM_CUDA(cudaFuncSetAttribute(k_group_sample<uint64_t>, cudaFuncAttributeMaxDynamicSharedMemorySize, int(GP_SMEM)));
             sattr = true;
         }
-        const size_t ncap = size_t(std::max<int64_t>(b->nseg_cap, 1));
-        int32_t *cost = reinterpret_cast<int32_t *>(b->d_blk_chg.as<unsigned long long>() + ncap * size_t(b->gchunk / GR_BLOCK));
-        int32_t *buckets = cost + ncap;
-        const size_t zbytes = ncap * (size_t(b->gchunk / GR_BLOCK) * 8 + 4) + size_t(SO_BUCKETS) * 4;
-        int2 *br = reinterpret_cast<int2 *>(reinterpret_cast<unsigned char *>(b->d_blk_chg.p) + ((zbytes + 7) & ~size_t(7)));
-        SNPM_CUDA(cudaMemsetAsync(b->d_blk_chg.p, 0, zbytes, st));
-        k_group_sample<KeyT><<<int(b->S), 32 * GP_WARPS, GP_SMEM, st>>>(
+        SNPM_CUDA(launch_pdl(k_group_sample<KeyT>, dim3(unsigned(b->S)), dim3(32 * GP_WARPS), GP_SMEM, st,
             b->d_key_a.as<KeyT>(), b->d_hash.as<unsigned long long>(), b->d_slot_gid.as<uint16_t>(), b->d_ngroups.as<int32_t>(), b->d_gid.as<uint16_t>(),
             b->d_pair_db_tmp.as<int32_t>(), b->d_pair_s_tmp.as<int32_t>(), b->d_pair_db.as<int32_t>(), b->track_pairs ? b->d_pair_s.as<int32_t>() : nullptr,
-            b->d_goff.as<int32_t>(), gkeys, mstart, b->d_seg_off.as<int32_t>(), b->gchunk, b->code_bits, b->d_blk_chg.as<unsigned long long>(), cost,
-            int32_t(jcap1), buckets, br, b->d_work_counter.as<unsigned int>());
-        k_order_place<<<int(b->S), 256, 0, st>>>(buckets, br, b->d_seg_off.as<int32_t>(), mstart, b->gchunk, b->d_seg_order.as<int4>());
+            b->d_goff.as<int32_t>(), (const KeyT *)gkeys, mstart, b->d_seg_off.as<int32_t>(), b->gchunk, b->code_bits, b->d_blk_chg.as<unsigned long long>(),
+            seg_cost, int32_t(jcap), bucket_cnt, seg_br, b->d_work_counter.as<unsigned int>()));
+        SNPM_CUDA(launch_pdl(k_order_place, dim3(unsigned(b->S)), dim3(256), 0, st, (const int32_t *)bucket_cnt, (const int2 *)seg_br,
+                             b->d_seg_off.as<int32_t>(), mstart, b->gchunk, b->d_seg_order.as<int4>()));
         SNPM_KERNEL_CHECK();
         b->launches += 3;
         return SNPM_OK;
     }
-    k_tile_ranges<<<(tiles + 255) / 256, 256, 0, st>>>(mstart, tsample, tfirst, tiles, range);
-    k_group_ids<KeyT><<<tiles, RS_THREADS, 0, st>>>(b->d_key_a.as<KeyT>(), range, tsample, b->d_hash.as<unsigned long long>(), b->d_slot_gid.as<uint16_t>(),
-                                                    b->d_ngroups.as<int32_t>(), b->d_gid.as<uint16_t>(), hist);
-    k_group_scan<<<int(b->S), 1024, 0, st>>>(hist, tfirst, b->d_ngroups.as<int32_t>(), b->d_goff.as<int32_t>());
-    const size_t nseg_cap = size_t(std::max<int64_t>(b->nseg_cap, 1));
-    int32_t *seg_cost = reinterpret_cast<int32_t *>(b->d_blk_chg.as<unsigned long long>() + nseg_cap * size_t(b->gchunk / GR_BLOCK));
-    int32_t *bucket_cnt = seg_cost + nseg_cap;
-    const size_t zero_bytes = nseg_cap * (size_t(b->gchunk / GR_BLOCK) * 8 + 4) + size_t(SO_BUCKETS) * 4;
-    int2 *seg_br = reinterpret_cast<int2 *>(reinterpret_cast<unsigned char *>(b->d_blk_chg.p) + ((zero_bytes + 7) & ~size_t(7)));
-    int64_t jcap = 1;
-    for (int64_t s = 0; s < b->S; ++s) jcap = std::max(jcap, ceil_div64(b->h_off[size_t(s) + 1] - b->h_off[size_t(s)], b->gchunk));
+    SNPM_CUDA(launch_pdl(k_group_ids<KeyT>, dim3(unsigned(tiles)), dim3(RS_THREADS), 0, st, b->d_key_a.as<KeyT>(), (const int2 *)range, tsample,
+                         b->d_hash.as<unsigned long long>(), b->d_slot_gid.as<uint16_t>(), b->d_ngroups.as<int32_t>(), b->d_gid.as<uint16_t>(), hist));
+    SNPM_CUDA(launch_pdl(k_group_scan, dim3(unsigned(b->S)), dim3(1024), 0, st, hist, tfirst, b->d_ngroups.as<int32_t>(), b->d_goff.as<int32_t>()));
     cudaStream_t aux = b->copy_stream;
     if (!b->ev_fork) SNPM_CUDA(cudaEventCreateWithFlags(&b->ev_fork, cudaEventDisableTiming));
     if (!b->ev_join) SNPM_CUDA(cudaEventCreateWithFlags(&b->ev_join, cudaEventDisableTiming));
     SNPM_CUDA(cudaEventRecord(b->ev_fork, st));
     SNPM_CUDA(cudaStreamWaitEvent(aux, b->ev_fork, 0));
-    SNPM_CUDA(cudaMemsetAsync(b->d_blk_chg.p, 0, zero_bytes, aux));
     k_group_marks<KeyT><<<int(b->S), 1024, 0, aux>>>(b->d_goff.as<int32_t>(), gkeys, b->d_ngroups.as<int32_t>(), mstart, b->d_seg_off.as<int32_t>(), b->gchunk,
                                                      b->code_bits, b->d_blk_chg.as<unsigned long long>(), seg_cost, int32_t(jcap), bucket_cnt, seg_br);
     k_order_place<<<int(b->S), 256, 0, aux>>>(bucket_cnt, seg_br, b->d_seg_off.as<int32_t>(), mstart, b->gchunk, b->d_seg_order.as<int4>());
     SNPM_CUDA(cudaEventRecord(b->ev_join, aux));
-    k_group_place<<<tiles, RS_THREADS, size_t(GH_MAX_GROUPS) * 20, st>>>(b->d_gid.as<uint16_t>(), b->d_pair_db_tmp.as<int32_t>(), b->d_pair_s_tmp.as<int32_t>(),
-                                                                        b->d_pair_db.as<int32_t>(), b->track_pairs ? b->d_pair_s.as<int32_t>() : nullptr, mstart, tsample,
-                                                                        tfirst, range, hist, b->d_ngroups.as<int32_t>(), b->d_goff.as<int32_t>(), b->d_work_counter.as<unsigned int>());
+    SNPM_CUDA(launch_pdl(k_group_place, dim3(unsigned(tiles)), dim3(RS_THREADS), size_t(GH_MAX_GROUPS) * 20, st, b->d_gid.as<uint16_t>(),
+                         b->d_pair_db_tmp.as<int32_t>(), b->d_pair_s_tmp.as<int32_t>(), b->d_pair_db.as<int32_t>(),
+                         b->track_pairs ? b->d_pair_s.as<int32_t>() : nullptr, mstart, tsample, tfirst, (const int2 *)range, (const uint32_t *)hist,
+                         b->d_ngroups.as<int32_t>(), b->d_goff.as<int32_t>(), b->d_work_counter.as<unsigned int>()));
     SNPM_CUDA(cudaStreamWaitEvent(st, b->ev_join, 0));
     SNPM_KERNEL_CHECK();
-    b->launches += 7;
+    b->launches += 6;
     return SNPM_OK;
 }
 
@@ -1179,7 +1187,7 @@
             SNPM_CUDA(cudaFuncSetAttribute(k_score_grouped2<SK, WXV, ring>, cudaFuncAttributeMaxDynamicSharedMemorySize, 226 * 1024)); \
             attr_ = true;                                                                                                         \
         }                                                                                                                         \
-        k_score_grouped2<SK, WXV, ring><<<grid, G2_THREADS, smem, st>>>(g);                                                       \
+        SNPM_CUDA(launch_pdl(k_score_grouped2<SK, WXV, ring>, dim3(grid), dim3(G2_THREADS), smem, st, g));                         \
     } while (0)
     if (g.wx == G2_WX) {
         if (skip_db_hets) G2_LAUNCH(true, G2_WX); else G2_LAUNCH(false, G2_WX);
@@ -1259,8 +1267,8 @@
         }
         rec(b, SNPM_EV_SCORE);
         dim3 cgrid((a.a_pad + 31) / 32, unsigned(b->S));
-        k_combine_grouped<<<cgrid, 32 * CG_PARTS, 0, st>>>(a.part_score, b->d_part_int.as<int32_t>(), a.a_pad, db->stride, db->n_acc, a.seg_off, a.mstart,
-                                                 b->d_red.as<double>());
+        SNPM_CUDA(launch_pdl(k_combine_grouped, cgrid, dim3(32 * CG_PARTS), 0, st, (const double *)a.part_score, (const int32_t *)b->d_part_int.as<int32_t>(),
+                             a.a_pad, db->stride, db->n_acc, (const int32_t *)a.seg_off, (const int32_t *)a.mstart, b->d_red.as<double>()));
         SNPM_KERNEL_CHECK();
         b->launches += 1;
         rec(b, SNPM_EV_COMBINE);
diff --git a/snpmatch_b200/csrc/common.cuh b/snpmatch_b200/csrc/common.cuh
--- a/snpmatch_b200/csrc/common.cuh
+++ b/snpmatch_b200/csrc/common.cuh
@@ -9,6 +9,7 @@
 #include <vector>
 #include <algorithm>
 #include <cmath>
+#include <utility>
 
 #include "../../include/snpmatch_b200.h"
 
@@ -51,6 +52,24 @@
         SNPM_CUDA(cudaGetLastError());                                   \
         if (snpm_sync_debug()) SNPM_CUDA(cudaDeviceSynchronize());       \
     } while (0)
+
+__device__ __forceinline__ void pdl_wait() { asm volatile("griddepcontrol.wait;" ::: "memory"); }
+__device__ __forceinline__ void pdl_trigger() { asm volatile("griddepcontrol.launch_dependents;" ::: "memory"); }
+
+template <typename... KArgs, typename... Args>
+static inline cudaError_t launch_pdl(void (*kernel)(KArgs...), dim3 grid, dim3 block, size_t smem, cudaStream_t st, Args &&...args) {
+    cudaLaunchAttribute attr[1];
+    attr[0].id = cudaLaunchAttributeProgrammaticStreamSerialization;
+    attr[0].val.programmaticStreamSerializationAllowed = 1;
+    cudaLaunchConfig_t cfg = {};
+    cfg.gridDim = grid;
+    cfg.blockDim = block;
+    cfg.dynamicSmemBytes = smem;
+    cfg.stream = st;
+    cfg.attrs = attr;
+    cfg.numAttrs = 1;
+    return cudaLaunchKernelEx(&cfg, kernel, std::forward<Args>(args)...);
+}
 
 struct DevBuf {
     void *p = nullptr;
@@ -119,7 +138,7 @@
     int64_t seg_S = 0;
     bool has_seg = false;
     snpm::DevBuf d_flags, d_flag_counts;
-    snpm::DevBuf d_match_row, d_tile_cnt, d_tile_off, d_prefix, d_pair_db, d_pair_s, d_pair_w;
+    snpm::DevBuf d_match_row, d_tile_cnt, d_tile_off, d_tile_state, d_prefix, d_pair_db, d_pair_s, d_pair_w;
     snpm::DevBuf d_mstart, d_seg_off;
     snpm::DevBuf d_part_score, d_part_ninfo, d_red, d_matches, d_ninfo64, d_prob, d_L, d_LR, d_status;
     int32_t n_windows = 0;
diff --git a/snpmatch_b200/csrc/group_sort.cuh b/snpmatch_b200/csrc/group_sort.cuh
--- a/snpmatch_b200/csrc/group_sort.cuh
+++ b/snpmatch_b200/csrc/group_sort.cuh
@@ -48,37 +48,62 @@
 constexpr int SC_THREADS = 256;
 constexpr int SC_PER = JOIN_TILE / SC_THREADS;
 constexpr int SC_SLOTS = 1024;
+constexpr unsigned long long JS_AGG = 1ull << 32, JS_INCL = 2ull << 32;
+
+__device__ __forceinline__ unsigned long long ld_relaxed_u64(const unsigned long long *p) {
+    unsigned long long v;
+    asm volatile("ld.relaxed.gpu.global.u64 %0, [%1];" : "=l"(v) : "l"(p) : "memory");
+    return v;
+}
+__device__ __forceinline__ void st_relaxed_u64(unsigned long long *p, unsigned long long v) {
+    asm volatile("st.relaxed.gpu.global.u64 [%0], %1;" ::"l"(p), "l"(v) : "memory");
+}
+
 template <typename KeyT>
-__global__ void __launch_bounds__(SC_THREADS) k_scatter_pairs_coded(
-        const int32_t *__restrict__ match_row, int64_t n, const int32_t *__restrict__ tile_off, const uint16_t *__restrict__ codes,
-        const double *__restrict__ wtable, int32_t n_table, int32_t code_bits, int32_t *__restrict__ prefix,
-        int32_t *__restrict__ pair_db, int32_t *__restrict__ pair_s, KeyT *__restrict__ key, int *status,
-        const int64_t *__restrict__ off, int64_t S, unsigned long long *__restrict__ hash, int *__restrict__ overflow,
-        const uint32_t *__restrict__ codes32) {
+__global__ void __launch_bounds__(SC_THREADS) k_join_scatter_coded(
+        const uint32_t *__restrict__ packed_cp, int64_t n, const int64_t *__restrict__ off, int64_t S, const JoinIndex x,
+        const uint16_t *__restrict__ codes, const uint32_t *__restrict__ codes32, const double *__restrict__ wtable, int32_t n_table,
+        int32_t code_bits, int32_t *__restrict__ match_row, int32_t *__restrict__ prefix, int32_t *__restrict__ pair_db,
+        int32_t *__restrict__ pair_s, KeyT *__restrict__ key, unsigned long long *__restrict__ hash, int *__restrict__ overflow,
+        int *status, unsigned long long *tile_state, int32_t chunk, int32_t *__restrict__ mstart, int32_t *__restrict__ seg_off) {
     constexpr int NW = SC_THREADS / 32;
     __shared__ int s_cnt[SC_PER][NW];
-    __shared__ int64_t s_first_sm, s_first_end;
+    __shared__ int64_t s_tile, s_first_sm, s_first_end, s_start;
+    __shared__ int32_t s_excl;
+    __shared__ int s_last;
+    __shared__ int s_warp[33];
+    __shared__ int32_t s_pref[JOIN_TILE];
     __shared__ unsigned long long s_seen[SC_SLOTS];
     const int lane = threadIdx.x & 31, warp = threadIdx.x >> 5;
-    const int64_t i0 = int64_t(blockIdx.x) * JOIN_TILE;
-    int32_t row[SC_PER];
-    uint32_t cw[SC_PER];
+    if (threadIdx.x == 0) s_tile = int64_t(atomicAdd(reinterpret_cast<unsigned int *>(tile_state), 1u));
+#pragma unroll
+    for (int j = 0; j < SC_SLOTS / SC_THREADS; ++j) s_seen[j * SC_THREADS + threadIdx.x] = 0ull;
+    __syncthreads();
+    pdl_trigger();
+    const int64_t tile = s_tile, n_tiles = gridDim.x;
+    const int64_t i0 = tile * JOIN_TILE;
+    uint32_t v[SC_PER], cw[SC_PER];
 #pragma unroll
     for (int j = 0; j < SC_PER; ++j) {
         const int64_t i = i0 + j * SC_THREADS + threadIdx.x;
-        row[j] = i < n ? match_row[i] : -1;
+        v[j] = i < n ? packed_cp[i] : 0xffffffffu;
     }
 #pragma unroll
     for (int j = 0; j < SC_PER; ++j) {
         const int64_t i = i0 + j * SC_THREADS + threadIdx.x;
         cw[j] = (codes32 != nullptr && i < n) ? codes32[i] : 0u;
     }
-    const int32_t base0 = tile_off[blockIdx.x];
-#pragma unroll
-    for (int j = 0; j < SC_SLOTS / SC_THREADS; ++j) s_seen[j * SC_THREADS + threadIdx.x] = 0ull;
+    int32_t row[SC_PER];
     uint32_t bal[SC_PER];
 #pragma unroll
     for (int j = 0; j < SC_PER; ++j) {
+        const int64_t i = i0 + j * SC_THREADS + threadIdx.x;
+        row[j] = -1;
+        if (i < n) {
+            check_order_packed(packed_cp, v[j], off, S, i, status);
+            row[j] = join_lookup(x, (v[j] >> 27) == 31u ? -1 : int32_t(v[j] >> 27), int32_t(v[j] & 0x7ffffffu));
+            match_row[i] = row[j];
+        }
         bal[j] = __ballot_sync(0xffffffffu, row[j] >= 0);
         if (lane == 0) s_cnt[j][warp] = __popc(bal[j]);
     }
@@ -91,9 +116,45 @@
         s_first_sm = lo;
         s_first_end = off[lo + 1];
     }
+    if (threadIdx.x == 32) {
+        int64_t lo = 0, hi = S + 1;
+        while (lo < hi) {
+            const int64_t mid = (lo + hi) >> 1;
+            if (off[mid] < i0) lo = mid + 1; else hi = mid;
+        }
+        s_start = lo;
+    }
+    __syncthreads();
+    if (warp == 0) {
+        int agg = 0;
+#pragma unroll
+        for (int j = 0; j < SC_PER; ++j)
+#pragma unroll
+            for (int w = 0; w < NW; ++w) agg += s_cnt[j][w];
+        unsigned long long *ts = tile_state + 2;
+        if (lane == 0) st_relaxed_u64(ts + tile, (tile == 0 ? JS_INCL : JS_AGG) | uint32_t(agg));
+        int excl = 0;
+        for (int64_t look = tile - 1; look >= 0; look -= 32) {
+            const int64_t k = look - lane;
+            unsigned long long sw = JS_INCL;
+            if (k >= 0)
+                do { sw = ld_relaxed_u64(ts + k); } while ((sw >> 32) == 0ull);
+            const uint32_t incl = __ballot_sync(0xffffffffu, (sw >> 32) == 2ull);
+            const int stop = incl ? __ffs(incl) - 1 : 31;
+            int c = lane <= stop ? int(uint32_t(sw)) : 0;
+#pragma unroll
+            for (int d = 16; d > 0; d >>= 1) c += __shfl_xor_sync(0xffffffffu, c, d);
+            excl += c;
+            if (incl) break;
+        }
+        if (lane == 0) {
+            if (tile > 0) st_relaxed_u64(ts + tile, JS_INCL | uint32_t(excl + agg));
+            s_excl = excl;
+        }
+    }
     __syncthreads();
     const int64_t s_first = s_first_sm, first_end = s_first_end;
-    int32_t base = base0;
+    int32_t base = s_excl;
 #pragma unroll
     for (int j = 0; j < SC_PER; ++j) {
         const int64_t i = i0 + j * SC_THREADS + threadIdx.x;
@@ -106,6 +167,7 @@
         }
         const int32_t p = base + before + __popc(bal[j] & ((1u << lane) - 1u));
         base += total;
+        s_pref[j * SC_THREADS + threadIdx.x] = p;
         unsigned long long ins = ~0ull, fold = 0ull;
         bool solo = false;
         int64_t smp = 0;
@@ -116,8 +178,8 @@
                 pair_s[p] = int32_t(i);
                 uint32_t cd[3];
                 if (codes32 != nullptr) {
-                    const uint32_t v = cw[j];
-                    cd[0] = v & 1023u; cd[2] = (v >> 10) & 1023u; cd[1] = (v >> 20) & 1023u;
+                    const uint32_t u = cw[j];
+                    cd[0] = u & 1023u; cd[2] = (u >> 10) & 1023u; cd[1] = (u >> 20) & 1023u;
                 } else {
                     cd[0] = codes[3 * i]; cd[2] = codes[3 * i + 1]; cd[1] = codes[3 * i + 2];
                 }
@@ -131,7 +193,9 @@
                 if (w0 == 1.0) c = 0; else if (w1 == 1.0) c = 1; else if (w2 == 1.0) c = 2;
                 else { c = 0; if (w1 > w0) c = 1; if (w2 > (c ? w1 : w0)) c = 2; }
                 const int b = code_bits;
-                const KeyT kk = (KeyT(c) << (3 * b)) | (KeyT(cd[c]) << (2 * b)) | (KeyT(cd[gs_slow_class(c)]) << b) | KeyT(cd[gs_fast_class(c)]);
+                const uint32_t c_called = c == 0 ? cd[0] : (c == 1 ? cd[1] : cd[2]);
+                const uint32_t c_slow = c == 2 ? cd[0] : cd[2], c_fast = c == 1 ? cd[0] : cd[1];
+                const KeyT kk = (KeyT(c) << (3 * b)) | (KeyT(c_called) << (2 * b)) | (KeyT(c_slow) << b) | KeyT(c_fast);
                 key[p] = kk;
                 int64_t lo = s_first;
                 if (i >= first_end) {
@@ -160,27 +224,50 @@
             if (fresh) gh_insert(hash + size_t(smp) * GH_SLOTS, ins, overflow + smp);
         }
     }
-}
-
-__global__ void __launch_bounds__(256) k_tile_ranges(const int32_t *__restrict__ mstart, const int32_t *__restrict__ tile_sample,
-                                                     const int32_t *__restrict__ tile_first, int32_t n_tiles, int2 *__restrict__ range) {
-    const int t = blockIdx.x * blockDim.x + threadIdx.x;
-    if (t >= n_tiles) return;
-    const int s = tile_sample[t];
-    const int lt = t - tile_first[s];
-    const int b0 = mstart[s], b1 = mstart[s + 1];
-    const int begin = min(b1, b0 + lt * RS_TILE);
-    range[t] = make_int2(begin, min(b1, begin + RS_TILE));
-}
-
+    __syncthreads();
+    const int64_t i1 = min(n, i0 + JOIN_TILE);
+    for (int64_t s = s_start + threadIdx.x; s < S && off[s] < i1; s += SC_THREADS) mstart[s] = s_pref[off[s] - i0];
+    if (tile == n_tiles - 1) {
+        const int32_t total = base;
+        if (threadIdx.x == 0) prefix[n] = total;
+        for (int64_t s = s_start + threadIdx.x; s <= S; s += SC_THREADS)
+            if (off[s] >= n) mstart[s] = total;
+    }
+    __threadfence();
+    __syncthreads();
+    if (threadIdx.x == 0) s_last = atomicAdd(reinterpret_cast<unsigned int *>(tile_state + 1), 1u) == unsigned(n_tiles - 1);
+    __syncthreads();
+    if (!s_last) return;
+    __threadfence();
+    int carry = 0;
+    for (int64_t sb = 0; sb < S; sb += SC_THREADS) {
+        const int64_t s = sb + threadIdx.x;
+        const int v = s < S ? (__ldcg(mstart + s + 1) - __ldcg(mstart + s) + chunk - 1) / chunk : 0;
+        int tot;
+        const int ex = block_excl_scan(v, &tot, s_warp);
+        if (s < S) seg_off[s] = carry + ex;
+        carry += tot;
+    }
+    if (threadIdx.x == 0) seg_off[S] = carry;
+}
 
 template <typename KeyT>
 __global__ void __launch_bounds__(1024) k_group_rank(const unsigned long long *__restrict__ hash, const double *__restrict__ wtable, int32_t code_bits,
                                                      uint16_t *__restrict__ slot_gid, int32_t *__restrict__ ngroups, KeyT *__restrict__ gkeys,
-                                                     double4 *__restrict__ gw, int *__restrict__ overflow) {
+                                                     double4 *__restrict__ gw, int *__restrict__ overflow, const int32_t *__restrict__ mstart,
+                                                     const int32_t *__restrict__ tile_first, int2 *__restrict__ range) {
     __shared__ unsigned long long sm[GH_SLOTS];
     __shared__ int s_warp[33];
     const int s = blockIdx.x;
+    pdl_wait();
+    pdl_trigger();
+    if (range != nullptr) {
+        const int b0 = mstart[s], b1 = mstart[s + 1], t0 = tile_first[s], t1 = tile_first[s + 1];
+        for (int t = t0 + threadIdx.x; t < t1; t += blockDim.x) {
+            const int begin = min(b1, b0 + (t - t0) * RS_TILE);
+            range[t] = make_int2(begin, min(b1, begin + RS_TILE));
+        }
+    }
     const unsigned long long *tab = hash + size_t(s) * GH_SLOTS;
     unsigned long long v[4];
     int cnt = 0;
@@ -241,6 +328,8 @@
                                                          uint16_t *__restrict__ gid, uint32_t *__restrict__ tile_hist) {
     __shared__ uint32_t h[GH_MAX_GROUPS];
     const int t = blockIdx.x;
+    pdl_wait();
+    pdl_trigger();
     const int2 rg = range[t];
     const int begin = rg.x, end = rg.y;
     const int s = tile_sample[t];
@@ -278,6 +367,8 @@
                                                      const int32_t *__restrict__ ngroups, int32_t *__restrict__ goff) {
     __shared__ int s_warp[33];
     const int s = blockIdx.x;
+    pdl_wait();
+    pdl_trigger();
     const int ng = ngroups[s];
     const int t0 = tile_first[s], t1 = tile_first[s + 1];
     constexpr int PITCH = GH_MAX_GROUPS, U = 8;
@@ -316,6 +407,8 @@
                                                               const uint32_t *__restrict__ tile_hist, const int32_t *__restrict__ ngroups,
                                                               const int32_t *__restrict__ goff, unsigned int *__restrict__ work_counter) {
     extern __shared__ uint32_t rs_sm[];
+    pdl_wait();
+    pdl_trigger();
     if (blockIdx.x == 0 && threadIdx.x == 0) *work_counter = 0u;
     constexpr int NW = RS_THREADS / 32;
     constexpr int PITCH = GH_MAX_GROUPS;
@@ -454,6 +547,8 @@
                                                       int32_t jcap, int32_t *__restrict__ bucket_cnt, int2 *__restrict__ seg_br) {
     __shared__ int32_t s_off[GH_MAX_GROUPS + 1];
     const int s = blockIdx.x;
+    pdl_wait();
+    pdl_trigger();
     const int ng = ngroups[s];
     for (int g = threadIdx.x; g <= ng; g += blockDim.x) s_off[g] = goff[size_t(s) * (GH_MAX_GROUPS + 1) + g];
     __syncthreads();
@@ -477,6 +572,8 @@
     uint16_t *whist = reinterpret_cast<uint16_t *>(gp_smem);
     uint32_t *whist32 = reinterpret_cast<uint32_t *>(gp_smem);
     int32_t *s_off = reinterpret_cast<int32_t *>(gp_smem + size_t(GP_WARPS) * GH_MAX_GROUPS * 2);
+    pdl_wait();
+    pdl_trigger();
     if (blockIdx.x == 0 && threadIdx.x == 0) *work_counter = 0u;
     const int s = blockIdx.x;
     const int ng = ngroups[s];
@@ -581,6 +678,8 @@
     __shared__ int scan[SO_BUCKETS];
     __shared__ int warp_sum[8];
     const int s = blockIdx.x, t = threadIdx.x;
+    pdl_wait();
+    pdl_trigger();
     const int seg0 = seg_off[s], nseg_s = seg_off[s + 1] - seg0;
     if (nseg_s <= 0) return;
     constexpr int PT = SO_BUCKETS / 256;
diff --git a/snpmatch_b200/csrc/grouped.cuh b/snpmatch_b200/csrc/grouped.cuh
--- a/snpmatch_b200/csrc/grouped.cuh
+++ b/snpmatch_b200/csrc/grouped.cuh
@@ -420,6 +420,8 @@
     const int s = blockIdx.y;
     const int x = threadIdx.x & 31, y = threadIdx.x >> 5;
     const int p = blockIdx.x * 32 + x;
+    pdl_wait();
+    pdl_trigger();
     const int j0 = seg_off[s], j1 = seg_off[s + 1];
     const int per = (j1 - j0 + CG_PARTS - 1) / CG_PARTS;
     const int ja = min(j1, j0 + y * per), jb = min(j1, ja + per);
diff --git a/snpmatch_b200/csrc/grouped2.cuh b/snpmatch_b200/csrc/grouped2.cuh
--- a/snpmatch_b200/csrc/grouped2.cuh
+++ b/snpmatch_b200/csrc/grouped2.cuh
@@ -134,6 +134,8 @@
     unsigned char *team = g2_smem + size_t(in_team ? q : 0) * team_bytes;
     uint64_t *ring = reinterpret_cast<uint64_t *>(team);
     unsigned char *stage0 = team + size_t(RING) * wx * 8;
+    pdl_wait();
+    pdl_trigger();
     const int n_items = __ldg(a.seg_off + a.S) * a.n_slices;
     auto decode = [&](int i) {
         G2Item it;
diff --git a/snpmatch_b200/csrc/join.cuh b/snpmatch_b200/csrc/join.cuh
--- a/snpmatch_b200/csrc/join.cuh
+++ b/snpmatch_b200/csrc/join.cuh
@@ -74,14 +74,64 @@
     first_row[w] = p0 > 0x7fffffffll ? int32_t(re) : int32_t(lower_bound_i32(db_pos, rs, re, int32_t(p0)));
 }
 
+__device__ __forceinline__ void check_order_packed(const uint32_t *__restrict__ packed_cp, uint32_t v, const int64_t *__restrict__ off,
+                                                   int64_t S, int64_t i, int *status) {
+    if (i == 0 || (v >> 27) == 31u) return;
+    const uint32_t v0 = packed_cp[i - 1];
+    if ((v0 >> 27) == 31u || v > v0) return;
+    int64_t lo = 0, hi = S + 1;
+    while (lo < hi) {
+        const int64_t mid = (lo + hi) >> 1;
+        if (off[mid] < i) lo = mid + 1; else hi = mid;
+    }
+    if (!(lo <= S && off[lo] == i)) atomicAdd(status, 1);
+}
+
+struct JoinIndex {
+    const int32_t *db_pos;
+    int32_t n_chr;
+    const int32_t *bucket, *bucket_off;
+    int shift;
+    const int64_t *filter;
+    int64_t n_filter, row0_global;
+    const unsigned long long *bitmap;
+    const int32_t *first_row;
+    const int64_t *bm_off;
+};
+
+__device__ __forceinline__ int32_t join_lookup(const JoinIndex &x, int32_t c, int32_t p) {
+    int32_t row = -1;
+    if (c >= 0 && c < x.n_chr) {
+        const int32_t b0 = x.bucket_off[c], nb = x.bucket_off[c + 1] - b0 - 1;
+        const int32_t b = p >> x.shift;
+        if (x.bitmap != nullptr) {
+            const int64_t bit = x.bm_off[c] + p;
+            if (p >= 0 && bit < x.bm_off[c + 1]) {
+                const int64_t w = bit >> 6;
+                const unsigned long long word = __ldg(x.bitmap + w);
+                const int32_t base = __ldg(x.first_row + w);
+                const unsigned long long m = 1ull << (bit & 63);
+                if (word & m) {
+                    row = base + __popcll(word & (m - 1ull));
+                    if (x.filter && !contains_i64(x.filter, x.n_filter, int64_t(row) + x.row0_global)) row = -1;
+                }
+            }
+        } else if (p >= 0 && b < nb) {
+            const int64_t rs = __ldg(x.bucket + b0 + b), re = __ldg(x.bucket + b0 + b + 1);
+            const int64_t j = lower_bound_i32(x.db_pos, rs, re, p);
+            if (j < re && __ldg(x.db_pos + j) == p) {
+                row = int32_t(j);
+                if (x.filter && !contains_i64(x.filter, x.n_filter, j + x.row0_global)) row = -1;
+            }
+        }
+    }
+    return row;
+}
+
 __global__ void __launch_bounds__(JOIN_TILE) k_join_search(
         const int32_t *__restrict__ chrom, const int32_t *__restrict__ pos, int64_t n,
-        const int64_t *__restrict__ off, int64_t S,
-        const int32_t *__restrict__ db_pos, const int64_t *__restrict__ chr_regions, int32_t n_chr,
-        const int32_t *__restrict__ bucket, const int32_t *__restrict__ bucket_off, int shift,
-        const int64_t *__restrict__ filter, int64_t n_filter, int64_t row0_global,
+        const int64_t *__restrict__ off, int64_t S, const JoinIndex x,
         int32_t *__restrict__ match_row, int32_t *__restrict__ tile_cnt, int *status, int check,
-        const unsigned long long *__restrict__ bitmap, const int32_t *__restrict__ first_row, const int64_t *__restrict__ bm_off,
         const uint32_t *__restrict__ packed_cp) {
     const int64_t i = int64_t(blockIdx.x) * JOIN_TILE + threadIdx.x;
     int32_t row = -1;
@@ -91,46 +141,13 @@
             const uint32_t v = packed_cp[i];
             c = (v >> 27) == 31u ? -1 : int32_t(v >> 27);
             p = int32_t(v & 0x7ffffffu);
-            if (check && i > 0 && c >= 0) {
-                const uint32_t v0 = packed_cp[i - 1];
-                if ((v0 >> 27) != 31u && v <= v0) {
-                    int64_t lo = 0, hi = S + 1;
-                    while (lo < hi) {
-                        const int64_t mid = (lo + hi) >> 1;
-                        if (off[mid] < i) lo = mid + 1; else hi = mid;
-                    }
-                    if (!(lo <= S && off[lo] == i)) atomicAdd(status, 1);
-                }
-            }
+            if (check) check_order_packed(packed_cp, v, off, S, i, status);
         } else {
             if (check) check_order(chrom, pos, off, S, i, status);
             c = chrom[i];
             p = pos[i];
         }
-        if (c >= 0 && c < n_chr) {
-            const int32_t b0 = bucket_off[c], nb = bucket_off[c + 1] - b0 - 1;
-            const int32_t b = p >> shift;
-            if (bitmap != nullptr) {
-                const int64_t bit = bm_off[c] + p;
-                if (p >= 0 && bit < bm_off[c + 1]) {
-                    const int64_t w = bit >> 6;
-                    const unsigned long long word = __ldg(bitmap + w);
-                    const int32_t base = __ldg(first_row + w);
-                    const unsigned long long m = 1ull << (bit & 63);
-                    if (word & m) {
-                        row = base + __popcll(word & (m - 1ull));
-                        if (filter && !contains_i64(filter, n_filter, int64_t(row) + row0_global)) row = -1;
-                    }
-                }
-            } else if (p >= 0 && b < nb) {
-                const int64_t rs = __ldg(bucket + b0 + b), re = __ldg(bucket + b0 + b + 1);
-                const int64_t j = lower_bound_i32(db_pos, rs, re, p);
-                if (j < re && __ldg(db_pos + j) == p) {
-                    row = int32_t(j);
-                    if (filter && !contains_i64(filter, n_filter, j + row0_global)) row = -1;
-                }
-            }
-        }
+        row = join_lookup(x, c, p);
         match_row[i] = row;
     }
     const int cnt = __syncthreads_count(row >= 0);
```

New measurement: 6150 billion, median of 6. 1.5% lower.
